# ESMWG/NoahMP

Hardware: AMD Instinct MI355X
Metric: column-steps/sec (higher is better)
Workload: dtype f32

## Files before the change

### __graft_entry__.py

```python
import os
import subprocess
import sys

ROOT = os.path.dirname(os.path.abspath(__file__))
sys.path.insert(0, ROOT)
os.environ.setdefault("GPU_PINNED_MIN_XFER_SIZE", "1048576")


def build():
    from noahmp_amd import build as b
    b.build(verbose=True)
    b.build(extra_flags=["-DNMP_EXACT_LIBM=0"], lib=os.path.join(b.CSRC, "variants", "lib_ocml.so"), jobs=4)
    b.build(extra_flags=["-DNOAHMP_NSOIL=6"], lib=os.path.join(b.CSRC, "variants", "lib_nsoil6.so"), jobs=4)
    subprocess.check_call(["make", "-s", "-C", os.path.join(ROOT, "oracle"), "port"])
    if os.path.isdir("/root/reference"):
        subprocess.check_call(["make", "-s", "-C", os.path.join(ROOT, "oracle"), "ref"])
    sys.path.insert(0, os.path.join(ROOT, "tests"))
    from host_emul import emullib
    emullib.build()
    for ns in (6, 8):
        emullib.build(ns)
    import test_libm
    test_libm.build()
    import test_divrc
    test_divrc.build()
    from fortran import build_shim
    if build_shim.available():
        build_shim.build()
    import noahmp_amd
    from noahmp_amd import abi
    abi.load_library()
    from noahmp_amd import jit_warm
    n, bad = jit_warm.warm()
    if bad:
        raise RuntimeError("jit_warm: %d of %d option sets failed to compile" % (bad, n))
    print("build ok:", b.LIB)


def smoke():
    import torch
    import numpy as np
    from noahmp_amd import synth
    from noahmp_amd.tables import load_tables
    from noahmp_amd.driver import Engine
    from oracle.portlib import PortLib
    from tools.compare import parity_check, exact_check

    T, tb = load_tables("usgs")
    s = synth.mixed_small(tb, ni=64, nj=4)
    synth.first_step_fixups(s)
    synth.diurnal_forcing(s, 12, t_offset=s.t_offset)
    port = PortLib(autobuild=not os.path.exists(os.path.join(ROOT, "oracle", "_build", "libnoahmp_oracle.so")))
    port.set_tables(T)
    eng = Engine(T, device=0)
    so, sd = s.copy(), s.to_device("cuda:0")
    port.noahmplsm(so, 1, 2000, 180.0)
    st = eng.noahmplsm(sd, 1, 2000, 180.0)
    ok, lines = exact_check(so, sd.to_host()) if eng.exact_libm else parity_check(so, sd.to_host(), steps=1)
    print("smoke: land=%d glacier=%d skipped=%d kernel_ms=%.3f" % (st.n_land, st.n_glacier, st.n_skipped, st.kernel_ms))
    if st.code or not ok:
        raise AssertionError("HIP vs oracle mismatch (code %d):\n%s" % (st.code, "\n".join(lines)))
    print("smoke ok")


if __name__ == "__main__":
    build()
    if len(sys.argv) > 1 and sys.argv[1] == "smoke":
        smoke()
```

### include/noahmp_hip.h

```cpp
#ifndef NOAHMP_HIP_H
#define NOAHMP_HIP_H
#ifndef __HIPCC_RTC__
#include <stdint.h>
#include <stddef.h>
#endif
#ifdef __cplusplus
extern "C" {
#endif

#define NOAHMP_HIP_ABI_VERSION 1
#define NOAHMP_NSNOW 3
#ifndef NOAHMP_NSOIL
#define NOAHMP_NSOIL 4
#endif

typedef struct noahmp_step_args {
  int32_t         itimestep;
  int32_t         yr;
  float           julian;
  const float*    coszin;
  const float*    xlatin;
  const float*    dz8w;
  float           dt;
  const float*    dzs;
  int32_t         nsoil;
  float           dx;
  const int32_t*  ivgtyp;
  const int32_t*  isltyp;
  const float*    vegfra;
  const float*    vegmax;
  const float*    tmn;
  const float*    xland;
  const float*    xice;
  float           xice_thres;
  int32_t         isice;
  int32_t         isurban;
  int32_t         idveg;
  int32_t         iopt_crs;
  int32_t         iopt_btr;
  int32_t         iopt_run;
  int32_t         iopt_sfc;
  int32_t         iopt_frz;
  int32_t         iopt_inf;
  int32_t         iopt_rad;
  int32_t         iopt_alb;
  int32_t         iopt_snf;
  int32_t         iopt_tbot;
  int32_t         iopt_stc;
  int32_t         iz0tlnd;
  const float*    t3d;
  const float*    qv3d;
  const float*    u_phy;
  const float*    v_phy;
  const float*    swdown;
  const float*    glw;
  const float*    p8w3d;
  const float*    rainbl;
  float*          tsk;
  float*          hfx;
  float*          qfx;
  float*          lh;
  float*          grdflx;
  float*          smstav;
  float*          smstot;
  float*          sfcrunoff;
  float*          udrunoff;
  float*          albedo;
  float*          snowc;
  float*          smois;
  float*          sh2o;
  float*          tslb;
  float*          snow;
  float*          snowh;
  float*          canwat;
  float*          acsnom;
  float*          acsnow;
  float*          emiss;
  float*          qsfc;
  int32_t*        isnowxy;
  float*          tvxy;
  float*          tgxy;
  float*          canicexy;
  float*          canliqxy;
  float*          eahxy;
  float*          tahxy;
  float*          cmxy;
  float*          chxy;
  float*          fwetxy;
  float*          sneqvoxy;
  float*          alboldxy;
  float*          qsnowxy;
  float*          wslakexy;
  float*          zwtxy;
// ... 373 lines not shown
```

### noahmp_amd/csrc/nmp_dev_common.hpp

```cpp
#pragma once
#ifndef __HIPCC_RTC__
#include <hip/hip_runtime.h>
#include <stdint.h>
#endif
#include "noahmp_hip.h"

namespace nmp {

#define NMP_DEV __host__ __device__ __forceinline__
#define L(i) ((i) + 2)
#if defined(__HIP_DEVICE_COMPILE__)
#define NMP_ASSUME(c) __builtin_assume(c)
#else
#define NMP_ASSUME(c) ((void)0)
#endif
constexpr int NSOIL = NOAHMP_NSOIL;
constexpr int NSNOW = NOAHMP_NSNOW;
constexpr int NL = NSNOW + NSOIL;
static_assert(NSNOW == 3 && NSOIL >= 2 && NSOIL <= 12, "layer slots: three snow layers, 2..12 soil layers");

constexpr float GRAV = 9.80616f, SB = 5.67E-08f, VKC = 0.40f, TFRZ = 273.16f, HSUB = 2.8440E06f,
                HVAP = 2.5104E06f, HFUS = 0.3336E06f, CWAT = 4.188E06f, CICE = 2.094E06f,
                CPAIR = 1004.64f, TKWAT = 0.6f, TKICE = 2.2f, RAIR = 287.04f, RW = 461.269f,
                DENH2O = 1000.f, DENICE = 917.f;
// ... 7 lines not shown
};

NMP_DEV float fmin2(float a, float b) { return (a < b) ? a : b; }
NMP_DEV float fmax2(float a, float b) { return (a > b) ? a : b; }

NMP_DEV float powi2(float a) { return a * a; }
NMP_DEV float powi3(float a) { return a * (a * a); }
NMP_DEV float powi4(float a) { float b = a * a; return b * b; }
NMP_DEV float powi5(float a) { float b = a * a; return a * (b * b); }

#ifndef NMP_EXACT_LIBM
#define NMP_EXACT_LIBM 1
#endif
}
#include "nmp_libm.hpp"
namespace nmp {
#if defined(NMP_LIBM_COUNT) && !defined(__HIP_DEVICE_COMPILE__)
extern "C" long nmp_libm_calls[8];
#define NMP_CNT(i) (nmp_libm_calls[i]++)
#else
#define NMP_CNT(i) ((void)0)
#endif
NMP_DEV float nmp_max(float a, float b) { return a > b ? a : b; }
NMP_DEV float nmp_min(float a, float b) { return a < b ? a : b; }

#if NMP_EXACT_LIBM
NMP_DEV float nmp_expf(float x) { NMP_CNT(0); return libm::expf_(x); }
NMP_DEV float nmp_expf_const(float x) { NMP_CNT(0); return libm::expf_k_(x); }
NMP_DEV float nmp_logf(float x) { NMP_CNT(1); return libm::logf_(x); }
template <int N> NMP_DEV void nmp_logfN(const float* x, float* out) { for (int n = 0; n < N; n++) NMP_CNT(1); libm::logfN_<N>(x, out); }
template <int N> NMP_DEV void nmp_expfN(const float* x, float* out) { for (int n = 0; n < N; n++) NMP_CNT(0); libm::expfN_<N>(x, out); }
template <int N> NMP_DEV void nmp_powfN(const float* x, const float* y, float* out) { for (int n = 0; n < N; n++) NMP_CNT(2); libm::powfN_<N>(x, y, out); }
#define NMP_LOG2K(base) libm::powf_log2_k(libm::asuint(base))
template <int N> NMP_DEV void nmp_powf_constbaseN(const float* base, const double* log2base, const float* y, float* out) {
  for (int n = 0; n < N; n++) NMP_CNT(2);
  libm::powf_constbaseN_<N>(base, log2base, y, out);
}
template <int N> NMP_DEV void nmp_powf_pairN(const float* x, float y1, float y2, float* o1, float* o2) {
  for (int n = 0; n < 2 * N; n++) NMP_CNT(2);
  libm::powf_pairN_<N>(x, y1, y2, o1, o2);
}
NMP_DEV float nmp_powf(float x, float y) { NMP_CNT(2); return libm::powf_(x, y); }
NMP_DEV float nmp_log10f(float x) { NMP_CNT(3); return libm::log10f_(x); }
NMP_DEV float nmp_atanf(float x) { NMP_CNT(4); return libm::atanf_(x); }
NMP_DEV float nmp_atanf_ge1(float x) { NMP_CNT(4); return libm::atanf_ge1_(x); }
NMP_DEV float nmp_tanhf(float x) { NMP_CNT(5); return libm::tanhf_(x); }
NMP_DEV float nmp_tanf(float x) { return libm::tanf_(x); }
NMP_DEV float nmp_acosf(float x) { return libm::acosf_(x); }
NMP_DEV float nmp_cosf(float x) { return libm::cosf_(x); }
NMP_DEV float pow_quarter(float x) { NMP_CNT(6); return libm::powf_(x, 0.25f); }
NMP_DEV void pow_quarter2(float x1, float x2, float& r1, float& r2) {
  NMP_CNT(6); NMP_CNT(6);
  const float x[2] = {x1, x2}, y[2] = {0.25f, 0.25f}; float o[2];
  libm::powfN_<2>(x, y, o);
  r1 = o[0]; r2 = o[1];
}
NMP_DEV float pow_half(float x) { NMP_CNT(6); return libm::powf_(x, 0.5f); }
NMP_DEV float pow_two(float x) { NMP_CNT(6); return libm::powf_(x, 2.0f); }
NMP_DEV float pow_neg_quarter(float x) { NMP_CNT(6); return libm::powf_(x, -0.25f); }
#else
NMP_DEV float nmp_expf(float x) { return expf(x); }
NMP_DEV float nmp_expf_const(float x) { return expf(x); }
NMP_DEV float nmp_logf(float x) { return logf(x); }
template <int N> NMP_DEV void nmp_logfN(const float* x, float* out) { for (int n = 0; n < N; n++) out[n] = logf(x[n]); }
template <int N> NMP_DEV void nmp_expfN(const float* x, float* out) { for (int n = 0; n < N; n++) out[n] = expf(x[n]); }
template <int N> NMP_DEV void nmp_powfN(const float* x, const float* y, float* out) { for (int n = 0; n < N; n++) out[n] = powf(x[n], y[n]); }
#define NMP_LOG2K(base) 0.0
template <int N> NMP_DEV void nmp_powf_constbaseN(const float* base, const double*, const float* y, float* out) { for (int n = 0; n < N; n++) out[n] = powf(base[n], y[n]); }
template <int N> NMP_DEV void nmp_powf_pairN(const float* x, float y1, float y2, float* o1, float* o2) { for (int n = 0; n < N; n++) { o1[n] = powf(x[n], y1); o2[n] = powf(x[n], y2); } }
NMP_DEV float nmp_powf(float x, float y) { return powf(x, y); }
NMP_DEV float nmp_log10f(float x) { return log10f(x); }
NMP_DEV float nmp_atanf(float x) { return atanf(x); }
NMP_DEV float nmp_atanf_ge1(float x) { return atanf(x); }
NMP_DEV float nmp_tanhf(float x) { return tanhf(x); }
NMP_DEV float nmp_tanf(float x) { return tanf(x); }
NMP_DEV float nmp_acosf(float x) { return acosf(x); }
NMP_DEV float nmp_cosf(float x) { return cosf(x); }
NMP_DEV float pow_quarter(float x) { return sqrtf(sqrtf(x)); }
NMP_DEV void pow_quarter2(float x1, float x2, float& r1, float& r2) { r1 = sqrtf(sqrtf(x1)); r2 = sqrtf(sqrtf(x2)); }
NMP_DEV float pow_half(float x) { return sqrtf(x); }
NMP_DEV float pow_two(float x) { return x * x; }
NMP_DEV float pow_neg_quarter(float x) { return 1.0f / sqrtf(sqrtf(x)); }
#endif

#if defined(NMP_PHASE_TIMERS)
constexpr int NMP_NPHASE = 32;
static __device__ unsigned long long g_nmp_prof[NMP_NPHASE * 256];
#endif
#if defined(NMP_PHASE_TIMERS) && defined(__HIP_DEVICE_COMPILE__)
static __shared__ long long s_nmp_last[8];
#define NMP_TIC(ph) do { if ((int)(threadIdx.x & 63) == __ffsll((long long)__ballot(1)) - 1) { const long long now_ = clock64(); \
    const int w_ = threadIdx.x >> 6; \
    atomicAdd(&g_nmp_prof[(ph) * 256 + (blockIdx.x & 255)], (unsigned long long)(now_ - s_nmp_last[w_])); \
    s_nmp_last[w_] = now_; } } while (0)
#define NMP_TIC0() do { if ((threadIdx.x & 63) == 0) s_nmp_last[threadIdx.x >> 6] = clock64(); } while (0)
#else
#define NMP_TIC(ph) ((void)0)
#define NMP_TIC0() ((void)0)
#endif

#ifdef NMP_FIXED_DVEG
#ifndef NMP_FIXED_RUN
#define NMP_FIXED_RUN 1
#endif
#ifndef NMP_FIXED_CRS
#define NMP_FIXED_CRS 1
#define NMP_FIXED_BTR 1
#define NMP_FIXED_SFC 1
#define NMP_FIXED_FRZ 1
#define NMP_FIXED_INF 1
#define NMP_FIXED_RAD 3
#define NMP_FIXED_ALB 2
#define NMP_FIXED_SNF 1
#define NMP_FIXED_TBOT 2
#define NMP_FIXED_STC 1
#endif
struct Opt {
  static constexpr int dveg = NMP_FIXED_DVEG, crs = NMP_FIXED_CRS, btr = NMP_FIXED_BTR, run = NMP_FIXED_RUN, sfc = NMP_FIXED_SFC,
                       frz = NMP_FIXED_FRZ, inf = NMP_FIXED_INF, rad = NMP_FIXED_RAD, alb = NMP_FIXED_ALB, snf = NMP_FIXED_SNF,
                       tbot = NMP_FIXED_TBOT, stc = NMP_FIXED_STC;
};
#else
struct Opt {
  int dveg, crs, btr, run, sfc, frz, inf, rad, alb, snf, tbot, stc;
};
#endif

constexpr int NSLT = 30, NVEGT = 27;
struct Derived {
  float thks_pow[2][NSLT], thkdry[2][NSLT], d_rsurf[2][NSLT], frzx[2][NSLT];
  float kdt[NSLT];
  float chil[NVEGT], phi1[NVEGT], phi2[NVEGT], avmu[NVEGT];
};

struct TablesDev { noahmp_tables t; Derived d; };
NMP_DEV const Derived* derived_of(const noahmp_tables* T) { return &reinterpret_cast<const TablesDev*>(T)->d; }

struct Parm {
  int nroot;
  int st, u;
  float rgl, rsmin, hs, rsmax, topt;
  float bexp, smcmax, smcref, psisat, dksat, dwsat, smcwlt, quartz;
  float slope, csoil, zbot, czil, kdt, frzx;
  float thks_pow, thkdry, d_rsurf, chil, phi1, phi2, avmu;
  float lai1, lai2, sai1, sai2, hvt, hvb, tmin, z0mvt, cwpvt, dleaf;
  float ph_wt1;
  float ch2op;
};

NMP_DEV float div_rc(float x, double r) { return (float)((double)x * r); }
#define NMP_RCC(c) (1.0 / (double)(c))
NMP_DEV double rc64(float y) {
#if defined(__HIP_DEVICE_COMPILE__)
  const double yd = (double)y;
  const double r0 = __builtin_amdgcn_rcp(yd);
  const double e = __builtin_fma(-yd, r0, 1.0);
  const double t = __builtin_fma(e, e, e);
  return __builtin_amdgcn_div_fixup(__builtin_fma(r0, t, r0), yd, 1.0);
#else
  return 1.0 / (double)y;
#endif
}

struct Urc {
  double dt;
  double dt_hfus;
  double dz[NL];
  double dz2[NL];
  double dzmm[NL];
  double zs[NL];
  double one_m_ea4;
};

struct TabScalars {
  int iswater, isbarren, issnow, eblforest, lucats, slcats;
  float csoil, zbot, czil, topt, rsmax, slope0;
  float albsat4[2], albdry4[2], omegas[2], betads, betais, eg1;
};
constexpr int NMP_TS_INTS = 6, NMP_TS_FLOATS = 15;
NMP_DEV TabScalars tab_scalars(const noahmp_tables& t) {
  TabScalars r;
  r.iswater = t.iswater; r.isbarren = t.isbarren; r.issnow = t.issnow; r.eblforest = t.eblforest; r.lucats = t.lucats; r.slcats = t.slcats;
  r.csoil = t.csoil_data; r.zbot = t.zbot_data; r.czil = t.czil_data; r.topt = t.topt_data; r.rsmax = t.rsmax_data; r.slope0 = t.slope_data[0];
  for (int ib = 0; ib < 2; ib++) { r.albsat4[ib] = t.albsat[ib][3]; r.albdry4[ib] = t.albdry[ib][3]; r.omegas[ib] = t.omegas[ib]; }
  r.betads = t.betads; r.betais = t.betais; r.eg1 = t.eg[0];
  return r;
}
NMP_DEV void tab_scalars_pack(const TabScalars& r, int* i, float* f) {
  i[0] = r.iswater; i[1] = r.isbarren; i[2] = r.issnow; i[3] = r.eblforest; i[4] = r.lucats; i[5] = r.slcats;
  f[0] = r.csoil; f[1] = r.zbot; f[2] = r.czil; f[3] = r.topt; f[4] = r.rsmax; f[5] = r.slope0;
  f[6] = r.albsat4[0]; f[7] = r.albsat4[1]; f[8] = r.albdry4[0]; f[9] = r.albdry4[1]; f[10] = r.omegas[0]; f[11] = r.omegas[1];
  f[12] = r.betads; f[13] = r.betais; f[14] = r.eg1;
}
NMP_DEV TabScalars tab_scalars_unpack(const int* i, const float* f) {
  TabScalars r;
  r.iswater = i[0]; r.isbarren = i[1]; r.issnow = i[2]; r.eblforest = i[3]; r.lucats = i[4]; r.slcats = i[5];
  r.csoil = f[0]; r.zbot = f[1]; r.czil = f[2]; r.topt = f[3]; r.rsmax = f[4]; r.slope0 = f[5];
  r.albsat4[0] = f[6]; r.albsat4[1] = f[7]; r.albdry4[0] = f[8]; r.albdry4[1] = f[9]; r.omegas[0] = f[10]; r.omegas[1] = f[11];
  r.betads = f[12]; r.betais = f[13]; r.eg1 = f[14];
  return r;
}

struct Ctx {
  const noahmp_tables* __restrict__ T;
  const Derived* __restrict__ D;
  Opt O;
  float dt;
  float zsoil[NL];
  int isurban;
  TabScalars ts;
  Urc u;
  unsigned char* cost;
};
NMP_DEV void record_cost(const Ctx& c, int which, int n) {
#if defined(__HIP_DEVICE_COMPILE__) && defined(NMP_COST_RECORD)
  if (c.cost) c.cost[2 * (size_t)(blockIdx.x * blockDim.x + threadIdx.x) + which] = (unsigned char)n;
#else
  (void)c; (void)which; (void)n;
#endif
}

#if defined(__HIP_DEVICE_COMPILE__)
NMP_DEV float uniform_value(float x) { int i; memcpy(&i, &x, 4); i = __builtin_amdgcn_readfirstlane(i); memcpy(&x, &i, 4); return x; }
NMP_DEV double uniform_value(double x) {
  int i[2]; memcpy(i, &x, 8);
  i[0] = __builtin_amdgcn_readfirstlane(i[0]); i[1] = __builtin_amdgcn_readfirstlane(i[1]);
  memcpy(&x, i, 8); return x;
}
#else
NMP_DEV float uniform_value(float x) { return x; }
NMP_DEV double uniform_value(double x) { return x; }
#endif
template <class T> NMP_DEV T pick_layer(const T* a, int k) {
  T r = uniform_value(a[L(0)]);
#pragma unroll
  for (int j = 1; j < NSOIL; j++) { const T vj = uniform_value(a[L(j)]); r = (k == j) ? vj : r; }
  const T vn = uniform_value(a[L(NSOIL)]);
  r = (k >= NSOIL) ? vn : r;
  return r;
}

template <int J, class A> NMP_DEV float pick_soil_from(const A& a, int k) {
  if constexpr (J >= NSOIL) return a[L(NSOIL)];
  else return (k == J) ? a[L(J)] : pick_soil_from<J + 1>(a, k);
}
template <class A> NMP_DEV float pick_soil(const A& a, int k) { return pick_soil_from<1>(a, k); }
template <int J, class A> NMP_DEV float pick_soil_below_from(const A& a, int k) {
  if constexpr (J >= NSOIL - 2) return a[L(NSOIL - 1)];
  else return (k == J) ? a[L(J + 1)] : pick_soil_below_from<J + 1>(a, k);
}
template <class A> NMP_DEV float pick_soil_below(const A& a, int k) { return pick_soil_below_from<1>(a, k); }
template <class A, class P> NMP_DEV bool any_of_layers_1_to_4(const A& a, P pred) {
  bool r = false;
#pragma unroll
  for (int j = 1; j <= (NSOIL < 4 ? NSOIL : 4); j++) r = r || pred(a[L(j)]);
  return r;
}

NMP_DEV float dz_soil(const Ctx& c, int k) { return k == 1 ? -c.zsoil[L(1)] : (c.zsoil[L(k - 1)] - c.zsoil[L(k)]); }

NMP_DEV void ctx_fill_uniform(Ctx& c) {
  c.u.dt = 1.0 / (double)c.dt;
  c.u.dt_hfus = 1.0 / (double)(c.dt * HFUS);
  for (int k = 1; k <= NSOIL; k++) {
    const float dz = dz_soil(c, k);
    c.u.dz[L(k)] = 1.0 / (double)dz;
    c.u.dzmm[L(k)] = 1.0 / (double)(dz * 1000.f);
    c.u.zs[L(k)] = 1.0 / (double)(-c.zsoil[L(k)]);
    if (k < NSOIL) c.u.dz2[L(k)] = 1.0 / (double)(k == 1 ? -c.zsoil[L(2)] : (c.zsoil[L(k - 1)] - c.zsoil[L(k + 1)]));
  }
  c.u.one_m_ea4 = 1.0 / (double)(1.0f - nmp_expf(-4.0f));
}

struct Col {
  float lat, julian, cosz, shdfac, shdmax, sfctmp, sfcprs, psfc, uu, vv, q2, soldn, lwdn, prcp,
        tbot, co2air, o2air, foln, zlvl;
  int yearlen, ice, ist, isc, vegtyp;
  float albold, sneqvo, tah, eah, fwet, canliq, canice, tv, tg, qsfc, qsnow;
  int isnow;
  float snowh, sneqv, zwt, wa, wt, wslake, lfmass, rtmass, stmass, wood, stblcp, fastcp, lai, sai,
        cm, ch, tauss, smcwtd, deeprech, rech;
  float acc_sfcrunoff, acc_udrunoff, acc_acsnow, acc_acsnom, acc_rech, acc_deeprech;
  float fsa, fsr, fira, fsh, ssoil, fcev, fgev, fctr, ecan, etran, edir, trad, tgb, tgv, t2mv, t2mb,
        q2v, q2b, runsrf, runsub, apar, psn, sav, sag, fsno, nee, gpp, npp, fveg, albedo, qsnbot,
        ponding, ponding1, ponding2, rssun, rssha, bgap, wgap, chv, chb, emissi, shg, shc, shb, evg,
        evb, ghv, ghb, irg, irc, irb, tr, evc, chleaf, chuc, chv2, chb2, fpice;
  float thair, qair, eair, rhoair, qprecc, qprecl, solad0, solad1, solai0, solai1, swdown;
  float elai, esai, htop, igs, btran, latheav, latheag, qmelt, fsrv, fsrg;
  int frozen_canopy, frozen_ground;
  int err;
};

template <class A>
struct Lay {
  A stc, zsnso, dzsnso;
// ... 9 lines not shown
```

### noahmp_amd/csrc/nmp_dev_energy.hpp

```cpp
#pragma once
#include "nmp_dev_common.hpp"

namespace nmp {

NMP_DEV void esat_sel(float t, float& es, float& des) {
  if (t > 0.f) {
    es = 100.f * (6.107799961f + t * (4.436518521E-01f + t * (1.428945805E-02f + t * (2.650648471E-04f +
         t * (3.031240396E-06f + t * (2.034080948E-08f + t * 6.136820929E-11f))))));
    des = 100.f * (4.438099984E-01f + t * (2.857002636E-02f + t * (7.938054040E-04f + t * (1.215215065E-05f +
          t * (1.036561403E-07f + t * (3.532421810e-10f + t * -7.090244804E-13f))))));
  } else {
    es = 100.f * (6.109177956f + t * (5.034698970E-01f + t * (1.886013408E-02f + t * (4.176223716E-04f +
         t * (5.824720280E-06f + t * (4.838803174E-08f + t * 1.838826904E-10f))))));
    des = 100.f * (5.030305237E-01f + t * (3.773255020E-02f + t * (1.267995369E-03f + t * (2.477563108E-05f +
          t * (3.005693132E-07f + t * (2.158542548E-09f + t * 7.131097725E-12f))))));
  }
}
NMP_DEV float tdc(float t) { return nmp_min(50.f, nmp_max(-50.f, (t - TFRZ))); }

NMP_DEV float tdfcnd_thks_pow(const Parm& P) {
  float thks = nmp_powf(7.7f, P.quartz) * nmp_powf(2.0f, 1.f - P.quartz);
  return nmp_powf(thks, 1.f - P.smcmax);
}
NMP_DEV float tdfcnd_thkdry(const Parm& P) {
// ... 209 lines not shown
    float fage;
    snow_age(c.dt, s.tg, s.sneqvo, s.sneqv, s.tauss, fage);
    if (c.O.alb == 1) {
      float sl = 2.0f, sl1 = 1.f / sl, sl2 = 2.f * sl;
      float cf1 = ((1.f + sl1) / (1.f + sl2 * s.cosz) - sl1);
      float fzen = nmp_max(cf1, 0.f);
      albsni[0] = 0.95f * (1.f - 0.2f * fage);
      albsni[1] = 0.65f * (1.f - 0.5f * fage);
      albsnd[0] = albsni[0] + 0.4f * fzen * (1.f - albsni[0]);
      albsnd[1] = albsni[1] + 0.4f * fzen * (1.f - albsni[1]);
    } else {
      float alb = 0.55f + (s.albold - 0.55f) * nmp_expf(-0.01f * c.dt / 3600.f);
      if (s.qsnow > 0.f) alb = alb + nmp_min(s.qsnow * c.dt, SWEMX) * (0.84f - alb) / (SWEMX);
      albsni[0] = albsni[1] = albsnd[0] = albsnd[1] = alb;
      s.albold = alb;
    }
#pragma unroll
    for (int ib = 0; ib < 2; ib++) {
      float inc = nmp_max(0.11f - 0.40f * smc1, 0.f);
      float albsod = nmp_min(c.ts.albsat4[ib] + inc, c.ts.albdry4[ib]);
      float albsoi = albsod;
      if (s.isc == 9) { albsod += 0.10f; albsoi += 0.10f; }
      albgrd[ib] = albsod * (1.f - s.fsno) + albsnd[ib] * s.fsno;
      albgri[ib] = albsoi * (1.f - s.fsno) + albsni[ib] * s.fsno;
    }
    float gdir = 0.f;
#pragma unroll 1
    for (int ib = 0; ib < 2; ib++) {
#pragma unroll
      for (int ic = 0; ic < 2; ic++) {
        TwoStreamOut o = twostream(c, P, ic, v, s.cosz, vai, s.fwet, s.tv, albgrd[ib], albgri[ib],
                                   rho[ib], tau[ib], c.ts.omegas[ib], s.fveg, gdir, s.bgap, s.wgap);
        if (ic == 0) { fabd[ib] = o.fab; albd[ib] = o.fre; ftdd[ib] = o.ftd; ftid[ib] = o.fti;
                       frevd[ib] = o.frev; fregd[ib] = o.freg; }
        else { fabi[ib] = o.fab; albi[ib] = o.fre; ftii[ib] = o.fti; frevi[ib] = o.frev;
               fregi[ib] = o.freg; }
      }
    }
    float ext = gdir / s.cosz * sqrtf(1.f - rho[0] - tau[0]);
    fsun = (1.f - nmp_expf(-ext * vai)) / nmp_max(ext * vai, MPE);
    if (fsun < 0.01f) fsun = 0.f;
  }
  RadOut r;
  r.fsun = fsun;
  float fsha = 1.f - fsun;
  r.laisun = s.elai * fsun;
  r.laisha = s.elai * fsha;
  const float solad[2] = {s.solad0, s.solad1}, solai[2] = {s.solai0, s.solai1};
  float cad[2], cai[2];
  s.sag = 0.f; s.sav = 0.f; s.fsa = 0.f;
#pragma unroll
  for (int ib = 0; ib < 2; ib++) {
    cad[ib] = solad[ib] * fabd[ib];
    cai[ib] = solai[ib] * fabi[ib];
    s.sav = s.sav + cad[ib] + cai[ib];
    s.fsa = s.fsa + cad[ib] + cai[ib];
    float trd = solad[ib] * ftdd[ib];
    float tri = solad[ib] * ftid[ib] + solai[ib] * ftii[ib];
    float abs_ = trd * (1.f - albgrd[ib]) + tri * (1.f - albgri[ib]);
    s.sag = s.sag + abs_;
    s.fsa = s.fsa + abs_;
  }
  float laifra = s.elai / nmp_max(vai, MPE);
  if (fsun > 0.f) {
    r.parsun = (cad[0] + fsun * cai[0]) * laifra / nmp_max(r.laisun, MPE);
    r.parsha = (fsha * cai[0]) * laifra / nmp_max(r.laisha, MPE);
  } else {
    r.parsun = 0.f;
    r.parsha = (cad[0] + cai[0]) * laifra / nmp_max(r.laisha, MPE);
  }
  float rvis = albd[0] * solad[0] + albi[0] * solai[0];
  float rnir = albd[1] * solad[1] + albi[1] * solai[1];
  s.fsr = rvis + rnir;
  s.fsrv = frevd[0] * solad[0] + frevi[0] * solai[0] + frevd[1] * solad[1] + frevi[1] * solai[1];
  s.fsrg = fregd[0] * solad[0] + fregi[0] * solai[0] + fregd[1] * solad[1] + fregi[1] * solai[1];
  return r;
}

struct MoState {
  float moz, fm, fh, fh2, fv; int mozsgn;
  float tmpcm, tmpcm2;
};

NMP_DEV void sfcdif1(int& err, int iter, float sfctmp, double r_rhocp, float h, float qair, float zlvl,
                     float zpd, float z0m, float ur, float mpe, MoState& m, float& cm,
                     float& ch) {
  const float z0h = z0m;
  float mozold = m.moz;
  float moz2, fmnew, fhnew, fh2new;
  if (zlvl <= zpd) { if (!err) err = NOAHMP_ERR_STABILITY_STOP; }
  if (iter == 1) {
    m.tmpcm = nmp_logf((zlvl - zpd) / z0m);
    m.tmpcm2 = nmp_logf((2.0f + z0m) / z0m);
  }
  const float tmpcm = m.tmpcm, tmpch = m.tmpcm, tmpch2 = m.tmpcm2;
  if (iter == 1) {
    m.fv = 0.0f; m.moz = 0.0f; moz2 = 0.0f;
  } else {
    float tvir = (1.f + 0.61f * qair) * sfctmp;
    float tmp1 = div_rc(VKC * (GRAV / tvir) * h, r_rhocp);
    if (fabsf(tmp1) <= mpe) tmp1 = mpe;
    float mol = -1.f * powi3(m.fv) / tmp1;
    const double r_mol = rc64(mol);
    m.moz = nmp_min(div_rc(zlvl - zpd, r_mol), 1.f);
    moz2 = nmp_min(div_rc(2.0f + z0h, r_mol), 1.f);
  }
  if (mozold * m.moz < 0.f) m.mozsgn = m.mozsgn + 1;
  if (m.mozsgn >= 2) { m.moz = 0.f; m.fm = 0.f; m.fh = 0.f; moz2 = 0.f; m.fh2 = 0.f; }
  if (m.moz < 0.f) {
    float tmp1, tmp12;
    pow_quarter2(1.f - 16.f * m.moz, 1.f - 16.f * moz2, tmp1, tmp12);
    const float la[3] = {(1.f + tmp1 * tmp1) / 2.f, (1.f + tmp1) / 2.f, (1.f + tmp12 * tmp12) / 2.f};
    float lg[3];
    nmp_logfN<3>(la, lg);
    const float tmp2 = lg[0], tmp3 = lg[1];
    fmnew = 2.f * tmp3 + tmp2 - 2.f * nmp_atanf_ge1(tmp1) + 1.5707963f;
    fhnew = 2 * tmp2;
    const float tmp22 = lg[2];
    fh2new = 2 * tmp22;
  } else {
    fmnew = -5.f * m.moz; fhnew = fmnew;
    fh2new = -5.f * moz2;
  }
  if (iter == 1) {
    m.fm = fmnew; m.fh = fhnew; m.fh2 = fh2new;
  } else {
    m.fm = 0.5f * (m.fm + fmnew);
    m.fh = 0.5f * (m.fh + fhnew);
    m.fh2 = 0.5f * (m.fh2 + fh2new);
  }
  m.fh = nmp_min(m.fh, 0.9f * tmpch);
  m.fm = nmp_min(m.fm, 0.9f * tmpcm);
  m.fh2 = nmp_min(m.fh2, 0.9f * tmpch2);
  float cmfm = tmpcm - m.fm, chfh = tmpch - m.fh;
  if (fabsf(cmfm) <= mpe) cmfm = mpe;
  if (fabsf(chfh) <= mpe) chfh = mpe;
  cm = VKC * VKC / (cmfm * cmfm);
  ch = VKC * VKC / (cmfm * chfh);
  m.fv = ur * sqrtf(cm);
}

NMP_DEV float pspmu(float xx) {
  return -2.f * nmp_logf((xx + 1.f) * 0.5f) - nmp_logf((xx * xx + 1.f) * 0.5f) + 2.f * nmp_atanf(xx) -
         (3.14159265f / 2.f);
}
NMP_DEV float psphu(float xx) { return -2.f * nmp_logf((xx * xx + 1.f) * 0.5f); }

NMP_DEV float sfcdif2_rlogu(float z0, float zlm) { return nmp_logf((zlm + z0) / z0); }
NMP_DEV void sfcdif2(int iter, float z0, float thz0, float thlm, float sfcspd, float czil, float zlm,
                     float& akms, float& akhs, float& rlmo, float& wstar2, float& ustar, const float rlogu_in) {
  const float WWST2 = 1.2f * 1.2f, VKRM = 0.40f, EXCM = 0.001f, BTG = (1.0f / 270.0f) * GRAV,
              ELFC = VKRM * BTG, WOLD = 0.15f, WNEW = 1.0f - WOLD, EPSU2 = 1.E-4f, EPSUST = 0.07f,
              ZTMIN = -5.0f, ZTMAX = 1.0f, HPBL = 1000.0f, SQVISC = 258.2f;
  float zilfc = -czil * VKRM * SQVISC;
  float zu = z0;
  float rdz = 1.f / zlm;
  float cxch = EXCM * rdz;
  float dthv = thlm - thz0;
  float du2 = nmp_max(sfcspd * sfcspd, EPSU2);
  float btgh = BTG * HPBL;
  if (iter == 1) {
    if (btgh * akhs * dthv != 0.0f) wstar2 = WWST2 * nmp_powf(fabsf(btgh * akhs * dthv), 2.f / 3.f);
    else wstar2 = 0.0f;
    ustar = nmp_max(sqrtf(akms * sqrtf(du2 + wstar2)), EPSUST);
    rlmo = ELFC * akhs * dthv / powi3(ustar);
  }
  float zt = nmp_max(1.E-6f, nmp_expf(zilfc * sqrtf(ustar * z0)) * z0);
  float zslu = zlm + zu;
  float zslt = zlm + zt;
  const float rlt_arg = zslt / zt;
  const float rlogu = rlogu_in;
  float rlogt;
  float zetalt = nmp_max(zslt * rlmo, ZTMIN);
  rlmo = zetalt / zslt;
  float zetalu = zslu * rlmo;
  float zetau = zu * rlmo;
  float zetat = zt * rlmo;
  float psmz, simm, pshz, simh;
  if (rlmo < 0.f) {
    float xlu = sqrtf(sqrtf(1.f - 16.f * zetalu)), xlt = sqrtf(sqrtf(1.f - 16.f * zetalt)),
          xu = sqrtf(sqrtf(1.f - 16.f * zetau)), xt = sqrtf(sqrtf(1.f - 16.f * zetat));
    const float la[7] = {(xu + 1.f) * 0.5f, (xu * xu + 1.f) * 0.5f, (xlu + 1.f) * 0.5f, (xlu * xlu + 1.f) * 0.5f,
                         (xt * xt + 1.f) * 0.5f, (xlt * xlt + 1.f) * 0.5f, rlt_arg};
    float lg[7];
    nmp_logfN<7>(la, lg);
    rlogt = lg[6];
    psmz = -2.f * lg[0] - lg[1] + 2.f * nmp_atanf(xu) - (3.14159265f / 2.f);
    const float pspmu_xlu = -2.f * lg[2] - lg[3] + 2.f * nmp_atanf(xlu) - (3.14159265f / 2.f);
    simm = pspmu_xlu - psmz + rlogu;
    pshz = -2.f * lg[4];
    simh = -2.f * lg[5] - pshz + rlogt;
  } else {
    rlogt = nmp_logf(rlt_arg);
    zetalu = nmp_min(zetalu, ZTMAX);
    zetalt = nmp_min(zetalt, ZTMAX);
    psmz = 5.f * zetau;
    simm = 5.f * zetalu - psmz + rlogu;
    pshz = 5.f * zetat;
    simh = 5.f * zetalt - pshz + rlogt;
  }
  ustar = nmp_max(sqrtf(akms * sqrtf(du2 + wstar2)), EPSUST);
  float ustark = ustar * VKRM;
  akms = nmp_max(ustark / simm, cxch);
  akhs = nmp_max(ustark / simh, cxch);
  if (btgh * akhs * dthv != 0.0f) wstar2 = WWST2 * nmp_powf(fabsf(btgh * akhs * dthv), 2.f / 3.f);
  else wstar2 = 0.0f;
  float rlmn = ELFC * akhs * dthv / powi3(ustar);
  rlmo = rlmo * WOLD + rlmn * WNEW;
}

struct StomataT { float awc, cp, vcmx_t; };
struct StomataP { float bp, c3psn, mp, folnmx, qe25, vcmx25, kc25, akc, ko25, ako, avcmx; };
NMP_DEV StomataP stomata_rows(const noahmp_tables* T, int v) {
  return StomataP{T->bp[v], T->c3psn[v], T->mp[v], T->folnmx[v], T->qe25[v], T->vcmx25[v], T->kc25[v], T->akc[v], T->ko25[v], T->ako[v], T->avcmx[v]};
}
NMP_DEV StomataT stomata_temperature(const StomataP& T, float tv, float o2) {
  StomataT r;
  float tc = tv - TFRZ;
  const float ex = div_rc(tc - 25.0f, NMP_RCC(10.0f));
  float pk[2];
  { const float pb[2] = {T.akc, T.ako}, py[2] = {ex, ex}; nmp_powfN<2>(pb, py, pk); }
  float kc = T.kc25 * pk[0];
// ... 12 lines not shown
  rs = 1.0f / bpv * cf;
  psn = 0.0f;
  if (apar <= 0.0f) return;
  const float c3 = T.c3psn, mpv = T.mp;
  float fnf = nmp_min(foln / nmp_max(mpe, T.folnmx), 1.0f);
  float ppf = 4.6f * apar;
  float j = ppf * T.qe25;
  const float awc = st.awc, cp = st.cp;
  float vcmx = T.vcmx25 / (1.0f + st.vcmx_t) * fnf * btran * avcmx_pow;
  float rlb = rb / cf;
  float cihi = 1.5f * co2, cilow = 0.0f;
  const double r_sfcprs = rc64(sfcprs);
#pragma unroll 1
  for (int iter = 1; iter <= 20; iter++) {
    float ci = 0.5f * (cihi + cilow);
    float wj = nmp_max(ci - cp, 0.0f) * j / (ci + 2.0f * cp) * c3 + j * (1.f - c3);
    float wc = nmp_max(ci - cp, 0.0f) * vcmx / (ci + awc) * c3 + vcmx * (1.f - c3);
    float we = 0.5f * vcmx * c3 + div_rc(4000.0f * vcmx * ci, r_sfcprs) * (1.f - c3);
    psn = nmp_min(nmp_min(wj, wc), we) * igs;
    float cs = nmp_max(co2 - 1.37f * rlb * sfcprs * psn, mpe);
    float a = mpv * psn * sfcprs * ea / (cs * ei) + bpv;
    float b = (mpv * psn * sfcprs / cs + bpv) * rlb - 1.f;
    float cq = -rlb;
    float q;
    if (b >= 0.0f) q = -0.5f * (b + sqrtf(b * b - 4.0f * a * cq));
    else q = -0.5f * (b - sqrtf(b * b - 4.0f * a * cq));
    float r1 = q / a, r2 = cq / q;
    rs = nmp_max(r1, r2);
    float fci = nmp_max(cs - psn * sfcprs * 1.65f * rs, 0.0f);
    steps++;
    if (((cihi - cilow) <= 5e-2f) || fabsf(fci - ci) <= mpe) break;
    else if (fci > ci) cilow = ci;
    else cihi = ci;
  }
  rs = rs * cf;
}

NMP_DEV void canres(const Parm& P, float par, float sfctmp, float rcsoil, float eah, float sfcprs,
                    float& rc, float& psn) {
  float q2 = 0.622f * eah / (sfcprs - 0.378f * eah);
  q2 = q2 / (1.0f + q2);
  float es = 0.611f * nmp_expf(2.501E6f / 461.0f * (1.f / 273.15f - 1.f / sfctmp));
  float sfcprsx = sfcprs * 1.E-3f;
  float q2sat = 0.622f * es / (sfcprsx - es);
  q2sat = q2sat * 1.E3f;
  q2sat = q2sat / 1.E3f;
  float ff = 2.0f * par / P.rgl;
  float rcs = (ff + P.rsmin / P.rsmax) / (1.0f + ff);
  rcs = nmp_max(rcs, 0.0001f);
  float dt_ = P.topt - sfctmp;
  float rct = 1.0f - 0.0016f * pow_two(dt_);
  rct = nmp_max(rct, 0.0001f);
  float rcq = 1.0f / (1.0f + P.hs * nmp_max(0.f, q2sat - q2));
  rcq = nmp_max(rcq, 0.01f);
  rc = P.rsmin / (rcs * rct * rcq * rcsoil);
  psn = -999.99f;
}

struct VegIn {
  float ur, vai, gammav, gammag, laisun, laisha, cwp, zlvl, zpd, z0m, z0mg, emv, emg, rsurf, rhsur,
        parsun, parsha, df_top, dz_top, stc_top;
  double r_rhocp, r_gammav, r_gammag;
};

struct VegLoop {
  float sfctmp, rhoair, qair, zlvl, zpd, z0m, ur, z0mg, hcan, cwp, vaie, sqrt_dleaf_uc, fveg, tg, laisune,
        laishae, rssun, rssha, rsurf, eair, estg, gammav, air, cir, canliq, canice, latheav, sav, fwet, sfcprs,
        thair, czil, rlogu;
  double r_rhocp, r_hcan, r_gammav;
  double r_ur;
  MoState mo;
  float cm, ch, tv, tah, eah, h, hg, fhg, dtv, rahc, rahg, rb, cah, cvh, estv, destv, irc, shc, evc, tr, wstar,
        tv_in, csh, cev, ctr;
  int liter, err, iter, done;
};
constexpr int VEGLOOP_WORDS = sizeof(VegLoop) / 4;

struct VegFirst {
  const Parm* P; int v; float parsun, parsha, foln, o2air, co2air, igs, btran; float psnsun, psnsha;
  StomataP sp;
  int bisections;
};

template <bool FIRST>
NMP_DEV void vege_iter(const Ctx& c, VegLoop& L, const int iter, VegFirst* f) {
  const float MPE = 1E-6f;
  const float sfctmp = L.sfctmp, rhoair = L.rhoair, ur = L.ur, fveg = L.fveg, tg = L.tg;
  const float z0h = L.z0m, z0hg = L.z0mg, hcan = L.hcan;
  if (c.O.sfc == 1) {
    sfcdif1(L.err, iter, sfctmp, L.r_rhocp, L.h, L.qair, L.zlvl, L.zpd, L.z0m, ur, MPE, L.mo, L.cm, L.ch);
  } else {
    sfcdif2(iter, L.z0m, L.tah, L.thair, ur, L.czil, L.zlvl, L.cm, L.ch, L.mo.moz, L.wstar, L.mo.fv, L.rlogu);
    L.ch = div_rc(L.ch, L.r_ur);
    L.cm = div_rc(L.cm, L.r_ur);
  }
  NMP_TIC(16);
  L.rahc = nmp_max(1.f, 1.f / (L.ch * ur));
  const float rawc = L.rahc;
  {
    float mozg = 0.f, fhgnew;
    if (!FIRST) {
      float tmp1 = div_rc(VKC * (GRAV / L.tah) * L.hg, L.r_rhocp);
      if (fabsf(tmp1) <= MPE) tmp1 = MPE;
      float molg = -1.f * powi3(L.mo.fv) / tmp1;
      mozg = nmp_min((L.zpd - L.z0mg) / molg, 1.f);
    }
    if (mozg < 0.f) fhgnew = pow_neg_quarter(1.f - 15.f * mozg);
    else fhgnew = 1.f + 4.7f * mozg;
    if (FIRST) L.fhg = fhgnew;
    else L.fhg = 0.5f * (L.fhg + fhgnew);
    float cwpc = pow_half(L.cwp * L.vaie * hcan * L.fhg);
    const float ea[4] = {div_rc(-cwpc * z0hg, L.r_hcan), div_rc(-cwpc * (z0h + L.zpd), L.r_hcan), cwpc, -cwpc / 2.f};
    float ex[4];
    nmp_expfN<4>(ea, ex);
    float tmp1 = ex[0];
    float tmp2 = ex[1];
    float tmprah2 = hcan * ex[2] / cwpc * (tmp1 - tmp2);
    float kh = nmp_max(VKC * L.mo.fv * (hcan - L.zpd), MPE);
    L.rahg = tmprah2 / kh;
    float tmprb = cwpc * 50.f / (1.f - ex[3]);
    L.rb = tmprb * L.sqrt_dleaf_uc;
  }
  const float rawg = L.rahg, rb = L.rb;
  NMP_TIC(17);
  float t = tdc(L.tv);
  esat_sel(t, L.estv, L.destv);
  const float estv = L.estv, destv = L.destv;
  NMP_TIC(18);
  if (FIRST) {
    StomataT st = {0.f, 0.f, 0.f};
    float avcmx_pow = 0.f;
    if (c.O.crs == 1 && (!(f->parsun <= 0.0f) || !(f->parsha <= 0.0f))) {
      st = stomata_temperature(f->sp, L.tv, f->o2air);
      avcmx_pow = nmp_powf(f->sp.avcmx, div_rc((L.tv - TFRZ) - 25.0f, NMP_RCC(10.0f)));
    }
#pragma unroll 1
    for (int leaf = 0; leaf < 2; leaf++) {
      float par = leaf ? f->parsha : f->parsun, rs_, psn_;
      if (c.O.crs == 1)
        stomata(f->sp, MPE, par, f->foln, L.tv, estv, L.eah, sfctmp, L.sfcprs, f->o2air, f->co2air, f->igs,
                f->btran, rb, st, avcmx_pow, rs_, psn_, f->bisections);
      else
        canres(*f->P, par, L.tv, f->btran, L.eah, L.sfcprs, rs_, psn_);
      if (leaf) { L.rssha = rs_; f->psnsha = psn_; } else { L.rssun = rs_; f->psnsun = psn_; }
    }
  }
  NMP_TIC(19);
  const double r_rahc = rc64(L.rahc), r_rb = rc64(rb), r_rahg = rc64(L.rahg);
  L.cah = div_rc(1.f, r_rahc);
  L.cvh = div_rc(2.f * L.vaie, r_rb);
  const float cah = L.cah, cvh = L.cvh;
  float cgh = div_rc(1.f, r_rahg);
  float cond = cah + cvh + cgh;
  const double r_cond = rc64(cond);
  float ata = div_rc(sfctmp * cah + tg * cgh, r_cond);
  float bta = div_rc(cvh, r_cond);
  float csh = (1.f - bta) * rhoair * CPAIR * cvh;
  float caw = cah;
  float cew = div_rc(L.fwet * L.vaie, r_rb);
  float ctw = (1.f - L.fwet) * (L.laisune / (rb + L.rssun) + L.laishae / (rb + L.rssha));
  float cgw = 1.f / (rawg + L.rsurf);
  cond = caw + cew + ctw + cgw;
  const double r_cond2 = rc64(cond);
  float aea = div_rc(L.eair * caw + L.estg * cgw, r_cond2);
  float bea = div_rc(cew + ctw, r_cond2);
  float cev = div_rc((1.f - bea) * cew * rhoair * CPAIR, L.r_gammav);
  float ctr = div_rc((1.f - bea) * ctw * rhoair * CPAIR, L.r_gammav);
  L.tah = ata + bta * L.tv;
  L.eah = aea + bea * estv;
  L.irc = fveg * (L.air + L.cir * powi4(L.tv));
  L.shc = fveg * rhoair * CPAIR * cvh * (L.tv - L.tah);
  L.evc = div_rc(fveg * rhoair * CPAIR * cew * (estv - L.eah), L.r_gammav);
  L.tr = div_rc(fveg * rhoair * CPAIR * ctw * (estv - L.eah), L.r_gammav);
  if (L.tv > TFRZ) L.evc = nmp_min(div_rc(L.canliq * L.latheav, c.u.dt), L.evc);
  else L.evc = nmp_min(div_rc(L.canice * L.latheav, c.u.dt), L.evc);
  float b = L.sav - L.irc - L.shc - L.evc - L.tr;
  float a = fveg * (4.f * L.cir * powi3(L.tv) + csh + (cev + ctr) * destv);
  L.dtv = b / a;
  L.tv_in = L.tv; L.csh = csh; L.cev = cev; L.ctr = ctr;
  L.tv = L.tv + L.dtv;
  L.h = div_rc(rhoair * CPAIR * (L.tah - sfctmp), r_rahc);
  L.hg = div_rc(rhoair * CPAIR * (tg - L.tah), r_rahg);
  NMP_TIC(20);
  NMP_CNT(7);
  if (L.liter == 1) L.done = 1;
  else if (iter >= 5 && fabsf(L.dtv) <= 0.01f && L.liter == 0) L.liter = 1;
  L.iter = iter + 1;
  if (L.iter > 20) L.done = 1;
}

NMP_DEV void vege_run_until(const Ctx& c, VegLoop& L, int last) {
#pragma unroll 1
  while (!L.done && L.iter <= last) vege_iter<false>(c, L, L.iter, nullptr);
}

struct SimpleLoop {
  NMP_DEV void run(const Ctx& c, VegLoop& L, bool active) const {
    if (active) vege_run_until(c, L, 20);
  }
};

template <class Runner>
NMP_DEV void vege_flux(const Ctx& c, const Parm& P, Col& s, const VegIn& q, float& cmv, float& psnsun,
                       float& psnsha, const bool canopy, Runner& runner) {
  const noahmp_tables* T = c.T;
  const float MPE = 1E-6f;
  VegLoop L = {};
  L.done = 1;
  if (canopy) {
    const int v = s.vegtyp - 1;
    VegFirst f = {};
    f.P = &P; f.v = v;
    if (c.O.crs == 1) f.sp = stomata_rows(T, v);
    const float fveg = s.fveg, ur = q.ur;
    L.sfctmp = s.sfctmp; L.rhoair = s.rhoair; L.qair = s.qair; L.zlvl = q.zlvl; L.zpd = q.zpd; L.z0m = q.z0m;
    L.ur = ur; L.z0mg = q.z0mg; L.cwp = q.cwp; L.fveg = fveg; L.rsurf = q.rsurf; L.eair = s.eair;
    L.gammav = q.gammav; L.canliq = s.canliq; L.canice = s.canice; L.latheav = s.latheav; L.sav = s.sav;
    L.fwet = s.fwet; L.sfcprs = s.sfcprs; L.thair = s.thair; L.czil = P.czil;
    L.mo = MoState{0.f, 0.f, 0.f, 0.f, 0.1f, 0, 0.f, 0.f};
    L.tv = s.tv; L.tg = s.tgv; L.tah = s.tah; L.eah = s.eah; L.ch = s.chv; L.cm = cmv;
    L.r_rhocp = q.r_rhocp; L.r_gammav = q.r_gammav;
    if (c.O.sfc != 1) { L.r_ur = rc64(ur); L.rlogu = sfcdif2_rlogu(L.z0m, L.zlvl); }
    const double r_fveg = rc64(fveg);
    L.vaie = nmp_min(6.f, div_rc(q.vai, r_fveg));
    L.laisune = nmp_min(6.f, div_rc(q.laisun, r_fveg));
    L.laishae = nmp_min(6.f, div_rc(q.laisha, r_fveg));
    float t = tdc(L.tg), destg_unused;
    esat_sel(t, L.estg, destg_unused);
    L.hcan = s.htop;
    L.r_hcan = rc64(L.hcan);
    float uc = ur * nmp_logf(L.hcan / q.z0m) / nmp_logf(q.zlvl / q.z0m);
    if ((L.hcan - q.zpd) <= 0.f) raise(s, NOAHMP_ERR_HCAN_LE_ZPD);
    L.air = -q.emv * (1.f + (1.f - q.emv) * (1.f - q.emg)) * s.lwdn - q.emv * q.emg * SB * powi4(L.tg);
    L.cir = (2.f - q.emv * (1.f - q.emg)) * q.emv * SB;
    L.sqrt_dleaf_uc = sqrtf(P.dleaf / uc);
    L.irc = s.irc; L.shc = s.shc; L.evc = s.evc; L.tr = s.tr;
    L.done = 0; L.iter = 1;
    f.parsun = q.parsun; f.parsha = q.parsha; f.foln = s.foln; f.o2air = s.o2air; f.co2air = s.co2air; f.igs = s.igs; f.btran = s.btran;
    vege_iter<true>(c, L, 1, &f);
    psnsun = f.psnsun; psnsha = f.psnsha;
    record_cost(c, 1, f.bisections);
  } else {
    record_cost(c, 1, 0);
  }
  runner.run(c, L, canopy);
  record_cost(c, 0, canopy ? L.iter - 1 : 0);
  NMP_TIC(21);
  if (!canopy) return;
  if (L.err) raise(s, L.err);
  {
    const float fveg = L.fveg, destv = L.destv;
    L.irc = L.irc + fveg * 4.f * L.cir * powi3(L.tv_in) * L.dtv;
    L.shc = L.shc + fveg * L.csh * L.dtv;
    L.evc = L.evc + fveg * L.cev * destv * L.dtv;
    L.tr = L.tr + fveg * L.ctr * destv * L.dtv;
  }
  float& tv = s.tv; float& tg = s.tgv; float& tah = s.tah; float& eah = s.eah;
  const float rhoair = s.rhoair;
  tv = L.tv; tah = L.tah; eah = L.eah; cmv = L.cm;
  s.rssun = L.rssun; s.rssha = L.rssha;
  s.irc = L.irc; s.shc = L.shc; s.evc = L.evc; s.tr = L.tr;
  s.qsfc = (0.622f * L.eah) / (L.sfcprs - 0.378f * L.eah);
  const float rahg = L.rahg, rawg = L.rahg, cah = L.cah, cvh = L.cvh, z0h = q.z0m, fveg = s.fveg;
  float t, estg = L.estg, destg = 0.f;
  float air = -q.emg * (1.f - q.emv) * s.lwdn - q.emg * q.emv * SB * powi4(tv);
  float cir = q.emg * SB;
  float csh = rhoair * CPAIR / rahg;
  float cev = rhoair * CPAIR / (q.gammag * (rawg + q.rsurf));
  float cgh = 2.f * q.df_top / q.dz_top;
#pragma unroll 1
  for (int iter = 1; iter <= 5; iter++) {
    t = tdc(tg);
    esat_sel(t, estg, destg);
    s.irg = cir * powi4(tg) + air;
    s.shg = csh * (tg - tah);
    s.evg = cev * (estg * q.rhsur - eah);
    s.ghv = cgh * (tg - q.stc_top);
    float b = s.sag - s.irg - s.shg - s.evg - s.ghv;
    float a = 4.f * cir * powi3(tg) + csh + cev * destg + cgh;
    float dtg = b / a;
    s.irg = s.irg + 4.f * cir * powi3(tg) * dtg;
    s.shg = s.shg + csh * dtg;
    s.evg = s.evg + cev * destg * dtg;
    s.ghv = s.ghv + cgh * dtg;
    tg = tg + dtg;
  }
  if (c.O.stc == 1) {
    if (s.snowh > 0.05f && tg > TFRZ) {
      tg = TFRZ;
      s.irg = cir * powi4(tg) - q.emg * (1.f - q.emv) * s.lwdn - q.emg * q.emv * SB * powi4(tv);
      s.shg = csh * (tg - tah);
      s.evg = cev * (estg * q.rhsur - eah);
      s.ghv = s.sag - (s.irg + s.shg + s.evg);
    }
  }
  float cah2 = L.mo.fv * VKC / ((c.O.sfc == 1 ? L.mo.tmpcm2 : nmp_logf((2.f + z0h) / z0h)) - L.mo.fh2);
  s.chv2 = cah2;
  if (cah2 < 1.E-5f) {
    s.t2mv = tah;
    s.q2v = s.qsfc;
  } else {
    const double r_fveg = rc64(fveg), r_cah2 = rc64(cah2);
    s.t2mv = tah - div_rc(div_rc(s.shg + div_rc(s.shc, r_fveg), q.r_rhocp) * 1.f, r_cah2);
    s.q2v = s.qsfc - div_rc(((div_rc(s.evc + s.tr, r_fveg) + s.evg) / (s.latheav * rhoair)) * 1.f, r_cah2);
  }
  s.chv = cah;
  s.chleaf = cvh;
  s.chuc = 1.f / rahg;
}

NMP_DEV void bare_flux(const Ctx& c, const Parm& P, Col& s, const VegIn& q, float zpdg, float& cmb) {
  const float MPE = 1E-6f;
  const float rhoair = s.rhoair, sfctmp = s.sfctmp, ur = q.ur, z0m = q.z0mg;
  MoState mo = {0.f, 0.f, 0.f, 0.f, 0.1f, 0, 0.f, 0.f};
  float h = 0.f, wstar = 0.f;
  float t, estg = 0.f, destg, csh = 0.f, cev = 0.f, ehb = 0.f;
  float& tgb = s.tgb; float& ch = s.chb; float& cm = cmb;
  const float z0h = z0m;
  const float cir = q.emg * SB;
  const float cgh = 2.f * q.df_top / q.dz_top;
  const float gamma = q.gammag, lathea = s.latheag;
  t = tdc(tgb);
  esat_sel(t, estg, destg);
  const double r_ur = (c.O.sfc != 1) ? rc64(ur) : 0.0;
  const float rlogu2 = (c.O.sfc != 1) ? sfcdif2_rlogu(z0m, q.zlvl) : 0.f;
#pragma unroll 1
  for (int iter = 1; iter <= 5; iter++) {
    if (c.O.sfc == 1) {
      sfcdif1(s.err, iter, sfctmp, q.r_rhocp, h, s.qair, q.zlvl, zpdg, z0m, ur, MPE, mo, cm, ch);
    } else {
      sfcdif2(iter, z0m, tgb, s.thair, ur, P.czil, q.zlvl, cm, ch, mo.moz, wstar, mo.fv, rlogu2);
      ch = div_rc(ch, r_ur);
      cm = div_rc(cm, r_ur);
      if (s.snowh > 0.f) { cm = nmp_min(0.01f, cm); ch = nmp_min(0.01f, ch); }
    }
    float rahb = nmp_max(1.f, 1.f / (ch * ur));
    float rawb = rahb;
    const double r_rahb = rc64(rahb);
    ehb = div_rc(1.f, r_rahb);
    csh = div_rc(rhoair * CPAIR, r_rahb);
    cev = div_rc(rhoair * CPAIR, q.r_gammag) / (q.rsurf + rawb);
    s.irb = cir * powi4(tgb) - q.emg * s.lwdn;
    s.shb = csh * (tgb - sfctmp);
    s.evb = cev * (estg * q.rhsur - s.eair);
    s.ghb = cgh * (tgb - q.stc_top);
    float b = s.sag - s.irb - s.shb - s.evb - s.ghb;
    float a = 4.f * cir * powi3(tgb) + csh + cev * destg + cgh;
    float dtg = b / a;
    if (iter == 5) {
      s.irb = s.irb + 4.f * cir * powi3(tgb) * dtg;
      s.shb = s.shb + csh * dtg;
      s.evb = s.evb + cev * destg * dtg;
      s.ghb = s.ghb + cgh * dtg;
    }
    tgb = tgb + dtg;
    h = csh * (tgb - sfctmp);
    t = tdc(tgb);
    esat_sel(t, estg, destg);
    if (iter == 5) s.qsfc = 0.622f * (estg * q.rhsur) / (s.psfc - 0.378f * (estg * q.rhsur));
  }
  if (c.O.stc == 1) {
    if (s.snowh > 0.05f && tgb > TFRZ) {
      tgb = TFRZ;
      s.irb = cir * powi4(tgb) - q.emg * s.lwdn;
      s.shb = csh * (tgb - sfctmp);
      s.evb = cev * (estg * q.rhsur - s.eair);
      s.ghb = s.sag - (s.irb + s.shb + s.evb);
    }
  }
  float ehb2 = mo.fv * VKC / ((c.O.sfc == 1 ? mo.tmpcm2 : nmp_logf((2.f + z0h) / z0h)) - mo.fh2);
  s.chb2 = ehb2;
  if (ehb2 < 1.E-5f) {
    s.t2mb = tgb;
    s.q2b = s.qsfc;
  } else {
    s.t2mb = tgb - div_rc(s.shb, q.r_rhocp) * 1.f / ehb2;
    s.q2b = s.qsfc - s.evb / (lathea * rhoair) * (1.f / ehb2 + q.rsurf);
  }
  if (s.vegtyp == c.isurban) s.q2b = s.qsfc;
  ch = ehb;
}

template <class A>
NMP_DEV void tsnosoi(const Ctx& c, const Parm& P, const Col& s, const Lay<A>& y, const float* df,
                     const float* hcpct) {
  const int isnow = s.isnow, ntop = isnow + 1;
  const float dt = c.dt;
  const float zbotsno = P.zbot - s.snowh;
  float ai[NL], bi[NL], ci[NL], rhsts[NL], ddz[NL], dtsdz[NL], zs[NL], tt[NL];
#pragma unroll
  for (int k = -2; k <= NSOIL; k++) { zs[L(k)] = y.zsnso[L(k)]; tt[L(k)] = y.stc[L(k)]; }
#pragma unroll
  for (int k = -2; k <= NSOIL; k++) {
    const int km = (k > -2) ? k - 1 : -2;
    const int kp = (k < NSOIL) ? k + 1 : NSOIL;
    ai[L(k)] = 0.f; bi[L(k)] = 1.f; ci[L(k)] = 0.f; rhsts[L(k)] = 0.f; ddz[L(k)] = 0.f; dtsdz[L(k)] = 0.f;
    if (k >= ntop) {
      float denom, eflux;
      if (k == ntop) {
        denom = -zs[L(k)] * hcpct[L(k)];
        float temp1 = -zs[L(kp)];
        const double r_temp1 = rc64(temp1);
        ddz[L(k)] = div_rc(2.0f, r_temp1);
        dtsdz[L(k)] = div_rc(2.0f * (tt[L(k)] - tt[L(kp)]), r_temp1);
        eflux = df[L(k)] * dtsdz[L(k)] - s.ssoil - 0.f;
      } else if (k < NSOIL) {
        denom = (zs[L(km)] - zs[L(k)]) * hcpct[L(k)];
        float temp1 = zs[L(km)] - zs[L(kp)];
        const double r_temp1 = rc64(temp1);
        ddz[L(k)] = div_rc(2.0f, r_temp1);
        dtsdz[L(k)] = div_rc(2.0f * (tt[L(k)] - tt[L(kp)]), r_temp1);
        eflux = (df[L(k)] * dtsdz[L(k)] - df[L(km)] * dtsdz[L(km)]) - 0.f;
      } else {
        denom = (zs[L(km)] - zs[L(k)]) * hcpct[L(k)];
        float botflx = 0.f;
        if (c.O.tbot == 2) {
          dtsdz[L(k)] = (tt[L(k)] - s.tbot) / (0.5f * (zs[L(km)] + zs[L(k)]) - zbotsno);
          botflx = -df[L(k)] * dtsdz[L(k)];
        }
        eflux = (-botflx - df[L(km)] * dtsdz[L(km)]) - 0.f;
      }
      const double r_denom = rc64(denom);
      if (k == ntop) {
        ai[L(k)] = 0.0f;
        ci[L(k)] = div_rc(-df[L(k)] * ddz[L(k)], r_denom);
        if (c.O.stc == 1) bi[L(k)] = -ci[L(k)];
        else bi[L(k)] = -ci[L(k)] + df[L(k)] / (0.5f * zs[L(k)] * zs[L(k)] * hcpct[L(k)]);
      } else if (k < NSOIL) {
        ai[L(k)] = div_rc(-df[L(km)] * ddz[L(km)], r_denom);
        ci[L(k)] = div_rc(-df[L(k)] * ddz[L(k)], r_denom);
        bi[L(k)] = -(ai[L(k)] + ci[L(k)]);
      } else {
        ai[L(k)] = div_rc(-df[L(km)] * ddz[L(km)], r_denom);
        ci[L(k)] = 0.0f;
        bi[L(k)] = -(ai[L(k)] + ci[L(k)]);
      }
      rhsts[L(k)] = div_rc(eflux, -r_denom);
      rhsts[L(k)] = rhsts[L(k)] * dt;
      ai[L(k)] = ai[L(k)] * dt;
      bi[L(k)] = 1.f + bi[L(k)] * dt;
      ci[L(k)] = ci[L(k)] * dt;
    }
  }
// ... 351 lines not shown
```

### noahmp_amd/csrc/nmp_dev_water.hpp

```cpp
#pragma once
#include "nmp_dev_common.hpp"

namespace nmp {

NMP_DEV void canwater(const Ctx& c, const Parm& P, Col& s, float& qrain, float& snowhin) {
  const float dt = c.dt, sfctmp = s.sfctmp, fveg = s.fveg;
  const double rdt = c.u.dt;
  float fp = 0.0f, qintr, qdripr, qthror, qints, qdrips, qthros, qevac, qdewc, qsubc, qfroc;
  float fpice = 0.f;
  if (c.O.snf == 1) {
    if (sfctmp > TFRZ + 2.5f) fpice = 0.f;
    else if (sfctmp <= TFRZ + 0.5f) fpice = 1.0f;
    else if (sfctmp <= TFRZ + 2.f) fpice = 1.f - (-54.632f + 0.2f * sfctmp);
    else fpice = 0.6f;
  } else if (c.O.snf == 2) {
    fpice = (sfctmp >= TFRZ + 2.2f) ? 0.f : 1.0f;
  } else {
    fpice = (sfctmp >= TFRZ) ? 0.f : 1.0f;
  }
  s.fpice = fpice;
  float bdfall = nmp_min(120.f, 67.92f + 51.25f * nmp_expf(div_rc(sfctmp - TFRZ, NMP_RCC(2.59f))));
  float rain = (s.qprecc + s.qprecl) * (1.f - fpice);
  float snow = (s.qprecc + s.qprecl) * fpice;
  if (s.qprecc + s.qprecl > 0.f) fp = (s.qprecc + s.qprecl) / (10.f * s.qprecc + s.qprecl);
  const float vai = s.elai + s.esai;
  float maxliq = P.ch2op * vai;
  if (vai > 0.f) {
    qintr = fveg * rain * fp;
    qintr = nmp_min(qintr, div_rc(maxliq - s.canliq, rdt) * (1.f - nmp_expf(-rain * dt / maxliq)));
    qintr = nmp_max(qintr, 0.f);
    qdripr = fveg * rain - qintr;
    qthror = (1.f - fveg) * rain;
  } else {
    qintr = 0.f; qdripr = 0.f; qthror = rain;
  }
  if (!s.frozen_canopy) {
    const float fcev_hvap = div_rc(s.fcev, NMP_RCC(HVAP));
    s.etran = nmp_max(div_rc(s.fctr, NMP_RCC(HVAP)), 0.f);
    qevac = nmp_max(fcev_hvap, 0.f);
    qdewc = fabsf(nmp_min(fcev_hvap, 0.f));
    qsubc = 0.f; qfroc = 0.f;
  } else {
    const float fcev_hsub = div_rc(s.fcev, NMP_RCC(HSUB));
    s.etran = nmp_max(div_rc(s.fctr, NMP_RCC(HSUB)), 0.f);
    qevac = 0.f; qdewc = 0.f;
    qsubc = nmp_max(fcev_hsub, 0.f);
    qfroc = fabsf(nmp_min(fcev_hsub, 0.f));
  }
  qevac = nmp_min(div_rc(s.canliq, rdt), qevac);
  s.canliq = nmp_max(0.f, s.canliq + (qintr + qdewc - qevac) * dt);
  if (s.canliq <= 1.E-06f) s.canliq = 0.0f;
  float maxsno = 6.6f * (0.27f + 46.f / bdfall) * vai;
  if (vai > 0.f) {
    qints = fveg * snow * fp;
    qints = nmp_min(qints, div_rc(maxsno - s.canice, rdt) * (1.f - nmp_expf(-snow * dt / maxsno)));
    qints = nmp_max(qints, 0.f);
    float ft = nmp_max(0.0f, div_rc(s.tv - 270.15f, NMP_RCC(1.87E5f)));
    float fv = div_rc(sqrtf(s.uu * s.uu + s.vv * s.vv), NMP_RCC(1.56E5f));
    qdrips = nmp_max(0.f, s.canice) * (fv + ft);
    qthros = (1.0f - fveg) * snow + (fveg * snow - qints);
  } else {
    qints = 0.f; qdrips = 0.f; qthros = snow;
  }
  qsubc = nmp_min(div_rc(s.canice, rdt), qsubc);
  s.canice = nmp_max(0.f, s.canice + (qints - qdrips) * dt + (qfroc - qsubc) * dt);
  if (s.canice <= 1.E-6f) s.canice = 0.f;
  if (s.canice > 0.f) s.fwet = nmp_max(0.f, s.canice) / nmp_max(maxsno, 1.E-06f);
  else s.fwet = nmp_max(0.f, s.canliq) / nmp_max(maxliq, 1.E-06f);
  s.fwet = nmp_powf(nmp_min(s.fwet, 1.f), 0.667f);
  if (s.canice > 1.E-6f && s.tv > TFRZ) {
    float qmeltc = nmp_min(div_rc(s.canice, rdt), div_rc(div_rc((s.tv - TFRZ) * CICE * s.canice, NMP_RCC(DENICE)), c.u.dt_hfus));
    s.canice = nmp_max(0.f, s.canice - qmeltc * dt);
    s.canliq = nmp_max(0.f, s.canliq + qmeltc * dt);
    s.tv = s.fwet * TFRZ + (1.f - s.fwet) * s.tv;
  }
  if (s.canliq > 1.E-6f && s.tv < TFRZ) {
    float qfrzc = nmp_min(div_rc(s.canliq, rdt), div_rc(div_rc((TFRZ - s.tv) * CWAT * s.canliq, NMP_RCC(DENH2O)), c.u.dt_hfus));
    s.canliq = nmp_max(0.f, s.canliq - qfrzc * dt);
    s.canice = nmp_max(0.f, s.canice + qfrzc * dt);
    s.tv = s.fwet * TFRZ + (1.f - s.fwet) * s.tv;
  }
  s.ecan = qevac + qsubc - qdewc - qfroc;
  qrain = qdripr + qthror;
  s.qsnow = qdrips + qthros;
  snowhin = s.qsnow / bdfall;
}

NMP_DEV void combo(float& dz, float& wliq, float& wice, float& t, float dz2, float wliq2, float wice2,
                   float t2) {
  float dzc = dz + dz2;
  float wicec = (wice + wice2);
  float wliqc = (wliq + wliq2);
  float h = (CICE * wice + CWAT * wliq) * (t - TFRZ) + HFUS * wliq;
  float h2 = (CICE * wice2 + CWAT * wliq2) * (t2 - TFRZ) + HFUS * wliq2;
  float hc = h + h2, tc;
  if (hc < 0.f) tc = TFRZ + hc / (CICE * wicec + CWAT * wliqc);
  else if (hc <= HFUS * wliqc) tc = TFRZ;
  else tc = TFRZ + (hc - HFUS * wliqc) / (CICE * wicec + CWAT * wliqc);
  dz = dzc; wice = wicec; wliq = wliqc; t = tc;
}

template <bool GLAC, class A>
NMP_DEV void combine(Col& s, const Lay<A>& y) {
  int& isnow = s.isnow;
  int isnow_old = isnow;
#pragma unroll 1
  for (int j = isnow_old + 1; j <= 0; j++) {
    if (y.snice[L(j)] <= .1f) {
      if (j != 0) {
        y.snliq[L(j + 1)] = y.snliq[L(j + 1)] + y.snliq[L(j)];
        y.snice[L(j + 1)] = y.snice[L(j + 1)] + y.snice[L(j)];
      } else {
        if (isnow_old < -1) {
          y.snliq[L(j - 1)] = y.snliq[L(j - 1)] + y.snliq[L(j)];
          y.snice[L(j - 1)] = y.snice[L(j - 1)] + y.snice[L(j)];
        } else {
          if (GLAC) {
            s.ponding1 = s.ponding1 + y.snliq[L(j)];
            s.sneqv = y.snice[L(j)];
            s.snowh = y.dzsnso[L(j)];
          } else if (y.snice[L(j)] >= 0.f) {
            s.ponding1 = y.snliq[L(j)];
            s.sneqv = y.snice[L(j)];
            s.snowh = y.dzsnso[L(j)];
          } else {
            s.ponding1 = y.snliq[L(j)] + y.snice[L(j)];
            if (s.ponding1 < 0.f) {
              y.sice[L(1)] = nmp_max(0.0f, y.sice[L(1)] + s.ponding1 / (y.dzsnso[L(1)] * 1000.f));
              s.ponding1 = 0.0f;
            }
            s.sneqv = 0.0f;
            s.snowh = 0.0f;
          }
          y.snliq[L(j)] = 0.0f; y.snice[L(j)] = 0.0f; y.dzsnso[L(j)] = 0.0f;
        }
      }
      if (j > isnow + 1 && isnow < -1) {
#pragma unroll 1
        for (int i = j; i >= isnow + 2; i--) {
          y.stc[L(i)] = y.stc[L(i - 1)];
          y.snliq[L(i)] = y.snliq[L(i - 1)];
          y.snice[L(i)] = y.snice[L(i - 1)];
          y.dzsnso[L(i)] = y.dzsnso[L(i - 1)];
        }
      }
      isnow = isnow + 1;
    }
  }
  if (y.sice[L(1)] < 0.f) { y.sh2o[L(1)] = y.sh2o[L(1)] + y.sice[L(1)]; y.sice[L(1)] = 0.f; }
  if (isnow == 0) return;
  s.sneqv = 0.f; s.snowh = 0.f;
  float zwice = 0.f, zwliq = 0.f;
// ... 206 lines not shown
    }
  }
  s.qsnbot = div_rc(qout, c.u.dt);
}

template <class A>
NMP_DEV void rebuild_layers(const Ctx& c, const Col& s, const Lay<A>& y) {
  float run = 0.f;
#pragma unroll
  for (int iz = -2; iz <= NSOIL; iz++) {
    if (iz > s.isnow) {
      float d;
      if (iz <= 0) d = -y.dzsnso[L(iz)];
      else if (iz == 1) d = c.zsoil[L(1)];
      else d = (c.zsoil[L(iz)] - c.zsoil[L(iz > 1 ? iz - 1 : 1)]);
      run = (iz == s.isnow + 1) ? d : (run + d);
      y.zsnso[L(iz)] = run;
      y.dzsnso[L(iz)] = -d;
    }
  }
}

template <class A>
NMP_DEV void snowwater(const Ctx& c, Col& s, const Lay<A>& y, float snowhin, float qsnfro,
                       float qsnsub, float qrain, float& snoflow) {
  const float dt = c.dt;
  snoflow = 0.0f; s.ponding1 = 0.0f; s.ponding2 = 0.0f;
  {
    int newnode = 0;
    if (s.isnow == 0 && s.qsnow > 0.f) {
      s.snowh = s.snowh + snowhin * dt;
      s.sneqv = s.sneqv + s.qsnow * dt;
    }
    if (s.isnow == 0 && s.qsnow > 0.f && s.snowh >= 0.025f) {
      s.isnow = -1;
      newnode = 1;
      y.dzsnso[L(0)] = s.snowh;
      s.snowh = 0.f;
      y.stc[L(0)] = nmp_min(273.16f, s.sfctmp);
      y.snice[L(0)] = s.sneqv;
      y.snliq[L(0)] = 0.f;
    }
    if (s.isnow < 0 && newnode == 0 && s.qsnow > 0.f) {
      y.snice[L(s.isnow + 1)] = y.snice[L(s.isnow + 1)] + s.qsnow * dt;
      y.dzsnso[L(s.isnow + 1)] = y.dzsnso[L(s.isnow + 1)] + snowhin * dt;
    }
  }
  if (s.isnow < 0) compact(c, s, y);
  if (s.isnow < 0) combine<false>(s, y);
  if (s.isnow < 0) divide<false>(s, y);
  snowh2o<false>(c, s, y, qsnfro, qsnsub, qrain);
  NMP_ASSUME(s.isnow >= -NSNOW && s.isnow <= 0);
#pragma unroll
  for (int iz = -2; iz <= 0; iz++) {
    if (iz <= s.isnow) {
      y.snice[L(iz)] = 0.f; y.snliq[L(iz)] = 0.f; y.stc[L(iz)] = 0.f; y.dzsnso[L(iz)] = 0.f;
      y.zsnso[L(iz)] = 0.f;
    }
  }
  if (s.sneqv > 2000.f) {
    float bdsnow = y.snice[L(0)] / y.dzsnso[L(0)];
    snoflow = (s.sneqv - 2000.f);
    y.snice[L(0)] = y.snice[L(0)] - snoflow;
    y.dzsnso[L(0)] = y.dzsnso[L(0)] - snoflow / bdsnow;
    snoflow = div_rc(snoflow, c.u.dt);
  }
  if (s.isnow < 0) {
    float sw = 0.f;
#pragma unroll
    for (int iz = -2; iz <= 0; iz++)
      if (iz > s.isnow) sw = sw + y.snice[L(iz)] + y.snliq[L(iz)];
    s.sneqv = sw;
  }
  rebuild_layers(c, s, y);
}

NMP_DEV void wdfcnd1(const Parm& P, double r_smcmax, float& wdf, float& wcnd, float smc, float fcr) {
  float factr = nmp_max(0.01f, div_rc(smc, r_smcmax));
  wdf = P.dwsat * nmp_powf(factr, P.bexp + 2.0f);
  wdf = wdf * (1.0f - fcr);
  wcnd = P.dksat * nmp_powf(factr, 2.0f * P.bexp + 3.0f);
  wcnd = wcnd * (1.0f - fcr);
}
NMP_DEV void wdfcnd2(const Parm& P, double r_smcmax, float& wdf, float& wcnd, float smc, float sice) {
  float factr = nmp_max(0.01f, div_rc(smc, r_smcmax));
  float expon = P.bexp + 2.0f;
  wdf = P.dwsat * nmp_powf(factr, expon);
  if (sice > 0.0f) {
    float x = 500.f * sice;
    float vkwgt = 1.f / (1.f + nmp_powf(x, 3.f));
    wdf = vkwgt * wdf + (1.f - vkwgt) * P.dwsat * nmp_powf(div_rc(0.2f, r_smcmax), expon);
  }
  wcnd = P.dksat * nmp_powf(factr, 2.0f * P.bexp + 3.0f);
}

template <class A>
NMP_DEV void soilwater(const Ctx& c, const Parm& P, Col& s, const Lay<A>& y, float qinsur, float qseva,
                       const float* etrani, float& qdrain, float* wcnd, float& fcrmax) {
  const float dt = c.dt;
  const double r_smcmax = rc64(P.smcmax);
  float sh2o[NL], smc[NL], sice[NL], dz[NL], fcr[NL];
  float pddum = 0.0f, rsat = 0.0f, sicemax = 0.0f;
  s.runsrf = 0.0f;
  fcrmax = 0.0f;
#pragma unroll
  for (int k = 1; k <= NSOIL; k++) {
    sh2o[L(k)] = y.sh2o[L(k)]; smc[L(k)] = y.smc[L(k)]; sice[L(k)] = y.sice[L(k)];
    dz[L(k)] = dz_soil(c, k);
  }
#pragma unroll
  for (int k = 1; k <= NSOIL; k++) {
    float epore = nmp_max(1.E-4f, (P.smcmax - sice[L(k)]));
    rsat = rsat + nmp_max(0.f, sh2o[L(k)] - epore) * dz[L(k)];
    sh2o[L(k)] = nmp_min(epore, sh2o[L(k)]);
  }
  const float ea4 = nmp_expf_const(-4.0f);
  float fcr_arg[NSOIL], fcr_exp[NSOIL];
#pragma unroll
  for (int k = 1; k <= NSOIL; k++) fcr_arg[k - 1] = -4.0f * (1.f - nmp_min(1.0f, div_rc(sice[L(k)], r_smcmax)));
  nmp_expfN<NSOIL>(fcr_arg, fcr_exp);
#pragma unroll
  for (int k = 1; k <= NSOIL; k++) {
    fcr[L(k)] = div_rc(nmp_max(0.0f, fcr_exp[k - 1] - ea4), c.u.one_m_ea4);
    if (sice[L(k)] > sicemax) sicemax = sice[L(k)];
    if (fcr[L(k)] > fcrmax) fcrmax = fcr[L(k)];
  }
  if (c.O.run == 2) {
    float wd1 = 0.f, wd2 = 0.f;
#pragma unroll
    for (int k = 1; k <= NSOIL; k++) wd1 = wd1 + (P.smcmax - sh2o[L(k)]) * dz[L(k)];
    float dzfine = 3.0f * (-c.zsoil[L(NSOIL)]) / 100;
    s.zwt = -3.f * c.zsoil[L(NSOIL)] - 0.001f;
    const float zwt0 = s.zwt;
#pragma unroll 1
    for (int k = 1; k <= 100; k++) {
      float zfine = (float)k * dzfine;
      float temp = 1.f + (zwt0 - zfine) / P.psisat;
      wd2 = wd2 + P.smcmax * (1.f - nmp_powf(temp, -1.f / P.bexp)) * dzfine;
      if (fabsf(wd2 - wd1) <= 0.01f) { s.zwt = zfine; break; }
    }
    s.runsub = (1.0f - fcrmax) * 4.0f * nmp_expf_const(-TIMEAN) * nmp_expf(-2.0f * s.zwt);
  }
  if (s.vegtyp == c.isurban) fcr[L(1)] = 0.95f;
  if (c.O.run == 1 || c.O.run == 2 || c.O.run == 4 || c.O.run == 5) {
    float fsat;
    if (c.O.run == 1) fsat = FSATMX * nmp_expf(-0.5f * 6.0f * (s.zwt - 2.0f));
    else if (c.O.run == 5) fsat = FSATMX * nmp_expf(-0.5f * 6.0f * nmp_max(-2.0f - s.zwt, 0.f));
    else if (c.O.run == 2) fsat = FSATMX * nmp_expf(-0.5f * 2.0f * s.zwt);
    else {
      float smctot = 0.f, dztot = 0.f;
      bool done = false;
#pragma unroll
      for (int k = 1; k <= NSOIL; k++) {
        if (!done) {
          dztot = dztot + dz[L(k)];
          smctot = smctot + smc[L(k)] * dz[L(k)];
          if (dztot >= 2.0f) done = true;
        }
      }
      smctot = smctot / dztot;
      fsat = nmp_powf(nmp_max(0.01f, smctot / P.smcmax), 4.f);
    }
    if (qinsur > 0.f) {
      s.runsrf = qinsur * ((1.0f - fcr[L(1)]) * fsat + fcr[L(1)]);
      pddum = qinsur - s.runsrf;
    }
  }
  if (c.O.run == 3) {
    if (qinsur > 0.0f) {
      float dt1 = dt / 86400.f;
      float smcav = P.smcmax - P.smcwlt;
      float dmax = -c.zsoil[L(1)] * smcav;
      float dice = -c.zsoil[L(1)] * sice[L(1)];
      dmax = dmax * (1.0f - (sh2o[L(1)] + sice[L(1)] - P.smcwlt) / smcav);
      float dd = dmax;
#pragma unroll
      for (int k = 2; k <= NSOIL; k++) {
        float th = (c.zsoil[L(k - 1)] - c.zsoil[L(k)]);
        dice = dice + th * sice[L(k)];
        dmax = th * smcav;
        dmax = dmax * (1.0f - (sh2o[L(k)] + sice[L(k)] - P.smcwlt) / smcav);
        dd = dd + dmax;
      }
      float val = (1.f - nmp_expf(-P.kdt * dt1));
      float ddt = dd * val;
      float px = nmp_max(0.f, qinsur * dt);
      float infmax = (px * (ddt / (px + ddt))) / dt;
      float fcr_ = 1.f;
      if (dice > 1.E-2f) {
        float acrt = 3 * P.frzx / dice;
        float sum = 1.f;
        sum = sum + (acrt * acrt) / 2.f;
        sum = sum + acrt / 1.f;
        fcr_ = 1.f - nmp_expf(-acrt) * sum;
      }
      infmax = infmax * fcr_;
      float wdf_, wcnd_;
      wdfcnd2(P, r_smcmax, wdf_, wcnd_, sh2o[L(1)], sicemax);
      infmax = nmp_max(infmax, wcnd_);
      infmax = nmp_min(infmax, px);
      s.runsrf = nmp_max(0.f, qinsur - infmax);
      pddum = qinsur - s.runsrf;
    }
  }
  int niter = 1;
  if (c.O.inf == 1) {
    niter = 3;
    if (pddum * dt > dz[L(1)] * P.smcmax) niter = niter * 2;
  }
  const float dtf = dt / niter;
  float qdrain_save = 0.0f;
  qdrain = 0.f;
#pragma unroll 1
  for (int iter = 1; iter <= niter; iter++) {
    float wdf[NL], smx[NL], ddz[NL], dsmdz[NL], ai[NL], bi[NL], ci[NL], rhstt[NL];
    float smxwtd = 0.f;
    if (c.O.inf == 1) {
      float factr[NSOIL], pw1[NSOIL], pw2[NSOIL];
#pragma unroll
      for (int k = 1; k <= NSOIL; k++) factr[k - 1] = nmp_max(0.01f, div_rc(smc[L(k)], r_smcmax));
      nmp_powf_pairN<NSOIL>(factr, P.bexp + 2.0f, 2.0f * P.bexp + 3.0f, pw1, pw2);
#pragma unroll
      for (int k = 1; k <= NSOIL; k++) {
        wdf[L(k)] = P.dwsat * pw1[k - 1];
        wdf[L(k)] = wdf[L(k)] * (1.0f - fcr[L(k)]);
        wcnd[L(k)] = P.dksat * pw2[k - 1];
        wcnd[L(k)] = wcnd[L(k)] * (1.0f - fcr[L(k)]);
        smx[L(k)] = smc[L(k)];
      }
    } else {
#pragma unroll
      for (int k = 1; k <= NSOIL; k++) { wdfcnd2(P, r_smcmax, wdf[L(k)], wcnd[L(k)], sh2o[L(k)], sicemax); smx[L(k)] = sh2o[L(k)]; }
    }
    if (c.O.run == 5) smxwtd = (c.O.inf == 1) ? s.smcwtd : s.smcwtd * sh2o[L(NSOIL)] / smc[L(NSOIL)];
#pragma unroll
    for (int k = 1; k <= NSOIL; k++) {
      float denom, wflux;
      if (k == 1) {
        denom = -c.zsoil[L(k)];
        ddz[L(k)] = div_rc(2.0f, c.u.dz2[L(k)]);
        dsmdz[L(k)] = div_rc(2.0f * (smx[L(k)] - smx[L(k + 1)]), c.u.dz2[L(k)]);
        wflux = wdf[L(k)] * dsmdz[L(k)] + wcnd[L(k)] - pddum + etrani[L(k)] + qseva;
      } else if (k < NSOIL) {
        denom = (c.zsoil[L(k - 1)] - c.zsoil[L(k)]);
        ddz[L(k)] = div_rc(2.0f, c.u.dz2[L(k)]);
        dsmdz[L(k)] = div_rc(2.0f * (smx[L(k)] - smx[L(k + 1)]), c.u.dz2[L(k)]);
        wflux = wdf[L(k)] * dsmdz[L(k)] + wcnd[L(k)] - wdf[L(k - 1)] * dsmdz[L(k - 1)] - wcnd[L(k - 1)] +
                etrani[L(k)];
      } else {
        denom = (c.zsoil[L(k - 1)] - c.zsoil[L(k)]);
        if (c.O.run == 1 || c.O.run == 2) qdrain = 0.f;
        if (c.O.run == 3) qdrain = P.slope * wcnd[L(k)];
        if (c.O.run == 4) qdrain = (1.0f - fcrmax) * wcnd[L(k)];
        if (c.O.run == 5) {
          float smxbot;
          if (s.zwt < c.zsoil[L(NSOIL)] - denom)
            smxbot = smx[L(k)] - (smx[L(k)] - smxwtd) * denom * 2.f / (denom + c.zsoil[L(k)] - s.zwt);
          else
            smxbot = smxwtd;
          dsmdz[L(k)] = div_rc(2.0f * (smx[L(k)] - smxbot), 0.5 * c.u.dz[L(k)]);
          qdrain = wdf[L(k)] * dsmdz[L(k)] + wcnd[L(k)];
        }
        wflux = -(wdf[L(k - 1)] * dsmdz[L(k - 1)]) - wcnd[L(k - 1)] + etrani[L(k)] + qdrain;
      }
      if (k == 1) {
        ai[L(k)] = 0.0f;
        bi[L(k)] = div_rc(wdf[L(k)] * ddz[L(k)], c.u.dz[L(k)]);
        ci[L(k)] = -bi[L(k)];
      } else if (k < NSOIL) {
        ai[L(k)] = div_rc(-wdf[L(k - 1)] * ddz[L(k - 1)], c.u.dz[L(k)]);
        ci[L(k)] = div_rc(-wdf[L(k)] * ddz[L(k)], c.u.dz[L(k)]);
        bi[L(k)] = -(ai[L(k)] + ci[L(k)]);
      } else {
        ai[L(k)] = div_rc(-wdf[L(k - 1)] * ddz[L(k - 1)], c.u.dz[L(k)]);
        ci[L(k)] = 0.0f;
        bi[L(k)] = -(ai[L(k)] + ci[L(k)]);
      }
      rhstt[L(k)] = div_rc(wflux, -c.u.dz[L(k)]);
    }
    float wplus = 0.0f;
#pragma unroll
    for (int k = 1; k <= NSOIL; k++) {
      rhstt[L(k)] = rhstt[L(k)] * dtf;
      ai[L(k)] = ai[L(k)] * dtf;
      bi[L(k)] = 1.f + bi[L(k)] * dtf;
      ci[L(k)] = ci[L(k)] * dtf;
    }
    {
      float p[NL], dl[NL];
      ci[L(NSOIL)] = 0.0f;
      p[L(1)] = -ci[L(1)] / bi[L(1)];
      dl[L(1)] = rhstt[L(1)] / bi[L(1)];
#pragma unroll
      for (int k = 2; k <= NSOIL; k++) {
        float inv = 1.0f / (bi[L(k)] + ai[L(k)] * p[L(k - 1)]);
        p[L(k)] = -ci[L(k)] * inv;
        dl[L(k)] = (rhstt[L(k)] - ai[L(k)] * dl[L(k - 1)]) * inv;
      }
      p[L(NSOIL)] = dl[L(NSOIL)];
#pragma unroll
      for (int kk = NSOIL - 1; kk >= 1; kk--) p[L(kk)] = p[L(kk)] * p[L(kk + 1)] + dl[L(kk)];
#pragma unroll
      for (int k = 1; k <= NSOIL; k++) sh2o[L(k)] = sh2o[L(k)] + p[L(k)];
    }
    if (c.O.run == 5) {
      if (s.zwt < c.zsoil[L(NSOIL)] - dz[L(NSOIL)]) {
        s.deeprech = s.deeprech + dtf * qdrain;
      } else {
        s.smcwtd = s.smcwtd + div_rc(dtf * qdrain, c.u.dz[L(NSOIL)]);
        wplus = nmp_max((s.smcwtd - P.smcmax), 0.0f) * dz[L(NSOIL)];
        float wminus = nmp_max((1.E-4f - s.smcwtd), 0.0f) * dz[L(NSOIL)];
        s.smcwtd = nmp_max(nmp_min(s.smcwtd, P.smcmax), 1.E-4f);
        sh2o[L(NSOIL)] = sh2o[L(NSOIL)] + div_rc(wplus, c.u.dz[L(NSOIL)]);
        qdrain = qdrain - wplus / dtf;
        s.deeprech = s.deeprech - wminus;
      }
    }
#pragma unroll
    for (int k = NSOIL; k >= 2; k--) {
      float epore = nmp_max(1.E-4f, (P.smcmax - sice[L(k)]));
      wplus = nmp_max((sh2o[L(k)] - epore), 0.0f) * dz[L(k)];
      sh2o[L(k)] = nmp_min(epore, sh2o[L(k)]);
      sh2o[L(k - 1)] = sh2o[L(k - 1)] + div_rc(wplus, c.u.dz[L(k - 1)]);
    }
    {
      float epore = nmp_max(1.E-4f, (P.smcmax - sice[L(1)]));
      wplus = nmp_max((sh2o[L(1)] - epore), 0.0f) * dz[L(1)];
      sh2o[L(1)] = nmp_min(epore, sh2o[L(1)]);
    }
#pragma unroll
    for (int k = 1; k <= NSOIL; k++) smc[L(k)] = sh2o[L(k)] + sice[L(k)];
    rsat = rsat + wplus;
    qdrain_save = qdrain_save + qdrain;
  }
  qdrain = (niter == 3) ? div_rc(qdrain_save, NMP_RCC(3.f)) : (niter == 6) ? div_rc(qdrain_save, NMP_RCC(6.f)) : qdrain_save;
  s.runsrf = s.runsrf * 1000.f + div_rc(rsat * 1000.f, c.u.dt);
  qdrain = qdrain * 1000.f;
  if (c.O.run == 2) {
    float wtsub = 0.f;
#pragma unroll
    for (int k = 1; k <= NSOIL; k++) wtsub = wtsub + wcnd[L(k)] * dz[L(k)];
#pragma unroll
    for (int k = 1; k <= NSOIL; k++) {
      float mh2o = s.runsub * dt * (wcnd[L(k)] * dz[L(k)]) / wtsub;
      sh2o[L(k)] = sh2o[L(k)] - div_rc(mh2o, c.u.dzmm[L(k)]);
    }
  }
  if (c.O.run != 1) {
    float mliq[NL], xs;
    const float watmin = 0.01f;
#pragma unroll
    for (int iz = 1; iz <= NSOIL; iz++) mliq[L(iz)] = sh2o[L(iz)] * dz[L(iz)] * 1000.f;
#pragma unroll
    for (int iz = 1; iz <= NSOIL - 1; iz++) {
      xs = (mliq[L(iz)] < 0.f) ? (watmin - mliq[L(iz)]) : 0.f;
      mliq[L(iz)] = mliq[L(iz)] + xs;
      mliq[L(iz + 1)] = mliq[L(iz + 1)] - xs;
    }
    xs = (mliq[L(NSOIL)] < watmin) ? (watmin - mliq[L(NSOIL)]) : 0.f;
    mliq[L(NSOIL)] = mliq[L(NSOIL)] + xs;
    s.runsub = s.runsub - div_rc(xs, c.u.dt);
    if (c.O.run == 5) s.deeprech = s.deeprech - xs * 1.E-3f;
#pragma unroll
    for (int iz = 1; iz <= NSOIL; iz++) sh2o[L(iz)] = div_rc(mliq[L(iz)], c.u.dzmm[L(iz)]);
  }
#pragma unroll
  for (int k = 1; k <= NSOIL; k++) { y.sh2o[L(k)] = sh2o[L(k)]; y.smc[L(k)] = smc[L(k)]; }
}

template <class A>
NMP_DEV void groundwater(const Ctx& c, const Parm& P, Col& s, const Lay<A>& y, const float* wcnd,
                         float fcrmax, float& qdis) {
  const float ROUS = 0.2f, CMIC = 0.20f, dt = c.dt;
  float dzmm[NL], znode[NL], mliq[NL], epore[NL], hk[NL], smc[NL];
  dzmm[L(1)] = -c.zsoil[L(1)] * 1.E3f;
  znode[L(1)] = -c.zsoil[L(1)] / 2.f;
#pragma unroll
  for (int iz = 2; iz <= NSOIL; iz++) {
    dzmm[L(iz)] = 1.E3f * (c.zsoil[L(iz - 1)] - c.zsoil[L(iz)]);
    znode[L(iz)] = -c.zsoil[L(iz - 1)] + 0.5f * (c.zsoil[L(iz - 1)] - c.zsoil[L(iz)]);
  }
#pragma unroll
  for (int iz = 1; iz <= NSOIL; iz++) {
    float sh = y.sh2o[L(iz)], si = y.sice[L(iz)];
    smc[L(iz)] = sh + si;
    mliq[L(iz)] = sh * dzmm[L(iz)];
    epore[L(iz)] = nmp_max(0.01f, P.smcmax - si);
    hk[L(iz)] = 1.E3f * wcnd[L(iz)];
  }
  int iwt = NSOIL;
  {
    bool found = false;
#pragma unroll
    for (int iz = 2; iz <= NSOIL; iz++)
      if (!found && s.zwt <= -c.zsoil[L(iz)]) { iwt = iz - 1; found = true; }
  }
  qdis = (1.0f - fcrmax) * 5.0f * nmp_expf_const(-TIMEAN) * nmp_expf(-6.0f * (s.zwt - 2.0f));
  float smc_iwt = pick_soil(smc, iwt), hk_iwt = pick_soil(hk, iwt), zn_iwt = pick_soil(znode, iwt);
  double s_node = nmp_min(1.0f, smc_iwt / P.smcmax);
  s_node = (s_node > (double)0.01f) ? s_node : (double)0.01f;
  float smpfz = (float)(-((double)(P.psisat * 1000.f) * pow(s_node, (double)(-P.bexp))));
  smpfz = nmp_max(-120000.0f, CMIC * smpfz);
  float wh_zwt = -s.zwt * 1.E3f;
  float wh = smpfz - zn_iwt * 1.E3f;
  float qin = -hk_iwt * (wh_zwt - wh) / ((s.zwt - zn_iwt) * 1.E3f);
  qin = nmp_max(div_rc(-10.0f, c.u.dt), nmp_min(div_rc(10.f, c.u.dt), qin));
  s.wt = s.wt + (qin - qdis) * dt;
  if (iwt == NSOIL) {
    s.wa = s.wa + (qin - qdis) * dt;
    s.wt = s.wa;
    s.zwt = (-c.zsoil[L(NSOIL)] + 25.f) - div_rc(div_rc(s.wa, NMP_RCC(1000.f)), NMP_RCC(ROUS));
    mliq[L(NSOIL)] = mliq[L(NSOIL)] - qin * dt;
    mliq[L(NSOIL)] = mliq[L(NSOIL)] + nmp_max(0.f, (s.wa - 5000.f));
    s.wa = nmp_min(s.wa, 5000.f);
  } else {
    if (iwt == NSOIL - 1) {
      s.zwt = -c.zsoil[L(NSOIL)] - div_rc((s.wt - ROUS * 1000 * 25.f) / (epore[L(NSOIL)]), NMP_RCC(1000.f));
    } else {
      float ws = 0.f;
#pragma unroll
      for (int iz = 3; iz <= NSOIL; iz++)
        if (iz >= iwt + 2) ws = ws + epore[L(iz)] * dzmm[L(iz)];
      const float ep = pick_soil_below(epore, iwt), zs = pick_soil_below(c.zsoil, iwt);
      s.zwt = -zs - div_rc((s.wt - ROUS * 1000.f * 25.f - ws) / (ep), NMP_RCC(1000.f));
    }
    float wtsub = 0.f;
#pragma unroll
    for (int iz = 1; iz <= NSOIL; iz++) wtsub = wtsub + hk[L(iz)] * dzmm[L(iz)];
    const double r_wtsub = rc64(wtsub);
#pragma unroll
    for (int iz = 1; iz <= NSOIL; iz++) mliq[L(iz)] = mliq[L(iz)] - div_rc(qdis * dt * hk[L(iz)] * dzmm[L(iz)], r_wtsub);
  }
  s.zwt = nmp_max(1.5f, s.zwt);
  float xs;
  const float watmin = 0.01f;
#pragma unroll
  for (int iz = 1; iz <= NSOIL - 1; iz++) {
    xs = (mliq[L(iz)] < 0.f) ? (watmin - mliq[L(iz)]) : 0.f;
    mliq[L(iz)] = mliq[L(iz)] + xs;
    mliq[L(iz + 1)] = mliq[L(iz + 1)] - xs;
  }
  xs = (mliq[L(NSOIL)] < watmin) ? (watmin - mliq[L(NSOIL)]) : 0.f;
  mliq[L(NSOIL)] = mliq[L(NSOIL)] + xs;
  s.wa = s.wa - xs;
  s.wt = s.wt - xs;
#pragma unroll
  for (int iz = 1; iz <= NSOIL; iz++) y.sh2o[L(iz)] = div_rc(mliq[L(iz)], c.u.dzmm[L(iz)]);
}
// ... 132 lines not shown
```

### noahmp_amd/csrc/nmp_engine_fixed.inc

```
#define NMP_CAT2(a, b) a##b
#define NMP_CAT(a, b) NMP_CAT2(a, b)
#define NMP_FIXED_TAG NMP_CAT(NMP_CAT(d, NMP_FIXED_DVEG), NMP_CAT(_r, NMP_FIXED_RUN))
#define nmp NMP_CAT(nmp_fixed_, NMP_FIXED_TAG)
#include "nmp_kernel.hpp"

namespace nmp_host {

static void NMP_CAT(fill_fixed_, NMP_FIXED_TAG)(KArgs& k, const LaunchDesc& d) {
  memset(&k, 0, sizeof(k));
  k.a = d.a;
  k.c.T = d.tables; k.c.D = derived_of(d.tables); k.c.dt = d.dt; k.c.isurban = d.isurban;
  k.c.ts = tab_scalars_unpack(d.ts_i, d.ts_f);
  for (int l = 0; l < NL; l++) k.c.zsoil[l] = d.zsoil[l];
  ctx_fill_uniform(k.c);
  k.ni = d.ni; k.nka = d.nka; k.nti = d.nti; k.ntj = d.ntj; k.k1 = d.k1; k.kp_lo = d.kp_lo; k.kp_hi = d.kp_hi; k.yearlen = d.yearlen;
  k.c.cost = d.cost;
  k.r_land = d.r_land; k.r_ice = d.r_ice; k.r_skip = d.r_skip;
  k.err = d.err; k.counts = d.counts; k.err_base = d.err_base; k.t_offset = d.t_offset; k.t_first = d.t_first; k.t_count = d.t_count;
}

#ifdef NMP_FIXED_EXPORT_PACK
size_t pack_fixed_kargs(const LaunchDesc& d, void* buf, size_t cap) {
  if (cap < sizeof(KArgs)) return 0;
  NMP_CAT(fill_fixed_, NMP_FIXED_TAG)(*reinterpret_cast<KArgs*>(buf), d);
  return sizeof(KArgs);
}
#endif

void NMP_CAT(launch_fixed_, NMP_FIXED_TAG)(const LaunchDesc& d, int mode, hipStream_t s, hipEvent_t ev0, hipEvent_t ev1) {
  KArgs k;
  NMP_CAT(fill_fixed_, NMP_FIXED_TAG)(k, d);
#ifndef NMP_FIXED_USE_LDS
#define NMP_FIXED_USE_LDS true
#endif
  constexpr long B = NMP_FIXED_BLOCK;
  if (mode == 4) {
    const long nb = (k.r_ice + B - 1) / B + (k.r_land + B - 1) / B + (k.r_skip + B - 1) / B;
    if (nb <= 0) return;
    hipExtLaunchKernelGGL((noahmp_ranges_kernel<NMP_FIXED_BLOCK>), dim3((unsigned)nb), dim3(NMP_FIXED_BLOCK), 0, s, ev0, ev1, 0, k);
    return;
  }
  const long n = (long)k.nti * k.ntj;
  if (n <= 0) return;
  hipExtLaunchKernelGGL((noahmp_column_kernel<NMP_FIXED_BLOCK, NMP_FIXED_USE_LDS, 0>), dim3((unsigned)((n + B - 1) / B)), dim3(NMP_FIXED_BLOCK), 0, s, ev0, ev1, 0, k);
}

#ifdef NMP_PHASE_TIMERS
void NMP_CAT(prof_fixed_, NMP_FIXED_TAG)(unsigned long long* acc, int n) {
  std::vector<unsigned long long> h(nmp::NMP_NPHASE * 256);
  if (hipMemcpyFromSymbol(h.data(), HIP_SYMBOL(nmp::g_nmp_prof), h.size() * 8) != hipSuccess) return;
  for (int p = 0; p < n && p < nmp::NMP_NPHASE; p++)
    for (int s2 = 0; s2 < 256; s2++) acc[p] += h[p * 256 + s2];
  std::fill(h.begin(), h.end(), 0ull);
  (void)hipMemcpyToSymbol(HIP_SYMBOL(nmp::g_nmp_prof), h.data(), h.size() * 8);
}
#endif

}
```

### noahmp_amd/csrc/nmp_engine_host.hpp

```cpp
#pragma once
#include <hip/hip_runtime.h>
#include <hip/hip_ext.h>
#include <stdio.h>
#include <string>
#include <unordered_map>
#include <vector>
#include "noahmp_hip.h"

#ifndef NMP_FIXED_BLOCK
#define NMP_FIXED_BLOCK 64
#endif

namespace nmp_host {

constexpr int kCountSlots = 256;
constexpr int kCountStride = 16;

struct Engine {
  int device = -1;
  bool have_tables = false;
  noahmp_tables* d_tables = nullptr;
  int ts_i[6] = {0, 0, 0, 0, 0, 0}; float ts_f[15] = {};
  unsigned long long* d_err = nullptr;
  int* d_counts = nullptr;
  int* d_gw_counts = nullptr;
  unsigned long long* h_err = nullptr;
  int* h_counts = nullptr;
  hipEvent_t ev0 = nullptr, ev1 = nullptr;
  bool ev_timed = false;
  hipStream_t own_stream = nullptr;
  std::vector<void*> mirror;
  std::vector<size_t> mirror_bytes;
  std::vector<void*> gw_mirror;
  std::vector<size_t> gw_mirror_bytes;
  std::vector<void*> init_mirror;
  std::vector<size_t> init_mirror_bytes;
  float* gw_kcell = nullptr;
  float* gw_head = nullptr;
  size_t gw_plane_bytes = 0;
  int async_pending = 0;
  hipStream_t async_stream = nullptr;
  std::vector<hipStream_t> async_streams;
  std::vector<hipEvent_t> async_events;
  int async_nti = 1, async_its = 1, async_jts = 1;
  float sync_class_ms[3] = {0.f, 0.f, 0.f};
  int sync_steps = 0;
  std::vector<float> sync_step_ms;
  std::vector<signed char> async_kind;
  int last_launch_kind = 0;
  unsigned char* d_cost = nullptr; size_t d_cost_bytes = 0; long cost_cols = 0; int record_cost = 0;
  bool cost_fresh = false;
  long long last_counts[3] = {0, 0, 0};
  int deferred_code = 0;
  hipStream_t s_up = nullptr, s_dn = nullptr;
  std::vector<hipEvent_t> pipe_events;
  struct HostReg { size_t bytes; int seen; int state; };
  std::unordered_map<const void*, HostReg> host_regs;
  int host_chunks = 3;
  bool host_chunks_auto = true;
  int pin_host_arrays = 0;
  int trust_out_mirror = 0;
  bool out_mirror_valid = false;
  std::vector<const void*> pipe_host;
  int pipe_extents[9] = {0, 0, 0, 0, 0, 0, 0, 0, 0};
  int resident_state = 0, lazy_download = 0;
  int static_inputs = 0;
  int deferred_status = 0;
  bool deferred_pending = false;
  unsigned resident_calls = 0;
  std::vector<void*> mirror_b;
  std::vector<size_t> mirror_b_bytes;
  int resident_sorted = 0;
  std::vector<void*> smirror; std::vector<size_t> smirror_bytes;
  int* s_perm = nullptr; unsigned* s_keys = nullptr; unsigned short* s_order = nullptr; int* s_dpos = nullptr; size_t s_cols = 0;
  long s_land = -1, s_glacier = -1;
  bool sorted_ok = false;
  bool sorted_newer = false;
  bool last_step_sorted = false;
  unsigned calls_since_sort = 0;
  hipEvent_t ev_up = nullptr, ev_kdone = nullptr;
  bool resident_valid = false, resident_dirty = false;
  std::vector<const void*> mirror_host;
  noahmp_step_args resident_args;
  int jit_kernels = 1;
  int jit_compile_only = 0;
  int fixed_kernels = 1;
  long sorted_land = -1, sorted_glacier = -1;
  int block = 256;
  int use_lds = 1;
  std::string last_error;
};
extern Engine g;

struct LaunchDesc {
  noahmp_step_args a;
  const noahmp_tables* tables;
  int ts_i[6]; float ts_f[15];
  float dt, zsoil[NOAHMP_NSNOW + NOAHMP_NSOIL + 1];
  int isurban, ni, nka, nti, ntj, k1, kp_lo, kp_hi, yearlen;
  unsigned long long* err;
  int* counts;
  unsigned long long err_base;
  long t_offset, t_first, t_count;
  unsigned char* cost;
  long r_land, r_ice, r_skip;
};
void launch_fixed_d1_r1(const LaunchDesc& d, int mode, hipStream_t s, hipEvent_t ev0, hipEvent_t ev1);
#ifdef NMP_PHASE_TIMERS
void prof_fixed_d1_r1(unsigned long long*, int); void prof_fixed_d3_r1(unsigned long long*, int); void prof_fixed_d3_r5(unsigned long long*, int);
void prof_fixed_d4_r1(unsigned long long*, int); void prof_fixed_d4_r3(unsigned long long*, int);
#endif
void launch_fixed_d3_r1(const LaunchDesc& d, int mode, hipStream_t s, hipEvent_t ev0, hipEvent_t ev1);
void launch_fixed_d3_r5(const LaunchDesc& d, int mode, hipStream_t s, hipEvent_t ev0, hipEvent_t ev1);
void launch_fixed_d4_r1(const LaunchDesc& d, int mode, hipStream_t s, hipEvent_t ev0, hipEvent_t ev1);
void launch_fixed_d4_r3(const LaunchDesc& d, int mode, hipStream_t s, hipEvent_t ev0, hipEvent_t ev1);
bool launch_jit(const int* o, const LaunchDesc& d, int mode, hipStream_t s, hipEvent_t ev0, hipEvent_t ev1);
void jit_finalize();
void jit_stats(int* out);
std::string cache_dir_public();
unsigned long long source_hash_public();
void sort_finalize();

#define HIPCHK(x) do { hipError_t e_ = (x); if (e_ != hipSuccess) { \
  char b_[256]; snprintf(b_, sizeof b_, "%s failed: %s (%s:%d)", #x, hipGetErrorString(e_), __FILE__, __LINE__); \
  nmp_host::g.last_error = b_; return -100; } } while (0)

int ensure_init();
void sum_counts(long long* out);
void status_counts(noahmp_status* st);
int ensure_bytes(void** p, size_t* have, size_t need);

}
```

### noahmp_amd/csrc/nmp_libm.hpp

```cpp
#pragma once
#ifndef __HIPCC_RTC__
#include <hip/hip_runtime.h>
#include <stdint.h>
#include <string.h>
#endif

namespace nmp {
namespace libm {

#ifndef NMP_LIBM_DEV
#define NMP_LIBM_DEV __host__ __device__ __forceinline__
#endif
#ifndef NMP_LIBM_FN
#define NMP_LIBM_FN NMP_LIBM_DEV
#endif
#ifndef NMP_LIBM_FN_POW
#define NMP_LIBM_FN_POW NMP_LIBM_FN
#endif

#if defined(__HIP_DEVICE_COMPILE__)
#define NMP_LIBM_TABLE static __device__ const
#else
#define NMP_LIBM_TABLE static const
#endif
#include "nmp_libm_tables.inc"
#ifndef NMP_LIBM_LDS
#define NMP_LIBM_LDS 1
#endif
#if defined(__HIP_DEVICE_COMPILE__) && NMP_LIBM_LDS
static __shared__ uint64_t sExp2fTab[32];
static __shared__ double sLogfTab[32];
static __shared__ double sPowfLog2Tab[32];
#define NMP_T_EXP2F sExp2fTab
#define NMP_T_LOGF sLogfTab
#define NMP_T_POWLOG2 sPowfLog2Tab
__device__ __forceinline__ void libm_stage_tables() {
  const int t = threadIdx.y * blockDim.x + threadIdx.x;
  if (t < 32) {
    sExp2fTab[t] = kExp2fTab[t];
    sLogfTab[t] = kLogfTab[t];
    sPowfLog2Tab[t] = kPowfLog2Tab[t];
  }
  __syncthreads();
}
#else
#define NMP_T_EXP2F kExp2fTab
#define NMP_T_LOGF kLogfTab
#define NMP_T_POWLOG2 kPowfLog2Tab
__host__ __device__ __forceinline__ void libm_stage_tables() {}
#endif

NMP_LIBM_DEV double mad(double a, double b, double c) { return __builtin_fma(a, b, c); }

NMP_LIBM_DEV uint32_t asuint(float f) { uint32_t u; memcpy(&u, &f, 4); return u; }
NMP_LIBM_DEV float asfloat(uint32_t u) { float f; memcpy(&f, &u, 4); return f; }
NMP_LIBM_DEV uint64_t asuint64(double f) { uint64_t u; memcpy(&u, &f, 8); return u; }
NMP_LIBM_DEV double asdouble(uint64_t u) { double f; memcpy(&f, &u, 8); return f; }
NMP_LIBM_DEV uint64_t exp2_tab_scale_(uint64_t tab, uint64_t k) {
#if defined(__HIP_DEVICE_COMPILE__)
  if (!__builtin_constant_p(k)) {
    typedef uint32_t u32x2 __attribute__((ext_vector_type(2)));
    u32x2 w = __builtin_bit_cast(u32x2, tab);
    w.y += (uint32_t)k << (52 - 5 - 32);
    return __builtin_bit_cast(uint64_t, w);
  }
#endif
  return tab + (k << (52 - 5));
}

NMP_LIBM_DEV bool expf_is_special_(float x) { return !(__builtin_fabsf(x) <= 88.0f); }
NMP_LIBM_DEV float expf_special_(float x, float res) {
  res = (x > 0x1.62e42ep6f) ? asfloat(0x7f800000u) : res;
  res = (x < -0x1.9fe368p6f) ? 0.0f : res;
  res = (x != x) ? x + x : res;
  return res;
}
NMP_LIBM_FN float expf_(float x) {
  const double xd = (double)x;
  double z = kExpfInvLn2Scaled * xd;
  double kd = z + kExp2fShift;
  const uint64_t ki = asuint64(kd);
  kd -= kExp2fShift;
  const double r = mad(kExpfInvLn2Scaled, xd, -kd);
  const uint64_t t = exp2_tab_scale_(NMP_T_EXP2F[ki % 32], ki);
  const double s = asdouble(t);
  z = mad(kExp2fPolyScaled[0], r, kExp2fPolyScaled[1]);
  const double r2 = r * r;
  double y = mad(kExp2fPolyScaled[2], r, 1.0);
  y = mad(z, r2, y);
  y = y * s;
  float res = (float)y;
  if (__builtin_expect(expf_is_special_(x), 0)) res = expf_special_(x, res);
  return res;
}

NMP_LIBM_DEV float expf_k_(float x) {
  const double xd = (double)x;
  double z = kExpfInvLn2Scaled * xd;
  double kd = z + kExp2fShift;
  const uint64_t ki = asuint64(kd);
  kd -= kExp2fShift;
  const double r = mad(kExpfInvLn2Scaled, xd, -kd);
  const uint64_t t = exp2_tab_scale_(kExp2fTab[ki % 32], ki);
  const double s = asdouble(t);
  z = mad(kExp2fPolyScaled[0], r, kExp2fPolyScaled[1]);
  const double r2 = r * r;
  double y = mad(kExp2fPolyScaled[2], r, 1.0);
  y = mad(z, r2, y);
  y = y * s;
  float res = (float)y;
  res = (x > 0x1.62e42ep6f) ? asfloat(0x7f800000u) : res;
  res = (x < -0x1.9fe368p6f) ? 0.0f : res;
  res = (x != x) ? x + x : res;
  return res;
}

NMP_LIBM_DEV bool logf_is_special_(uint32_t ix) { return ix - 0x00800000u >= 0x7f800000u - 0x00800000u; }
NMP_LIBM_DEV uint32_t logf_normalise_(float x, uint32_t ix) {
  return (ix - 1u < 0x007fffffu) ? asuint(x * 0x1p23f) - (23u << 23) : ix;
}
NMP_LIBM_DEV float logf_fix_special_(uint32_t ix0, float x, float res) {
  res = (ix0 == 0x7f800000u) ? x : res;
  res = ((ix0 & 0x80000000u) || ix0 * 2 > 0xff000000u) ? asfloat(0x7fc00000u) : res;
  res = (ix0 * 2 == 0) ? -asfloat(0x7f800000u) : res;
  return res;
}
NMP_LIBM_FN float logf_(float x) {
  const uint32_t ix0 = asuint(x);
  uint32_t ix = ix0;
  if (__builtin_expect(logf_is_special_(ix0), 0)) ix = logf_normalise_(x, ix0);
  const uint32_t tmp = ix - 0x3f330000u;
  const int i = (tmp >> (23 - 4)) % 16;
  const int k = (int32_t)tmp >> 23;
  const uint32_t iz = ix - (tmp & 0xff800000u);
  const double invc = NMP_T_LOGF[2 * i], logc = NMP_T_LOGF[2 * i + 1];
  const double z = (double)asfloat(iz);
  const double r = mad(z, invc, -1.0);
  const double y0 = mad((double)k, kLogfLn2, logc);
  const double r2 = r * r;
  double y = mad(kLogfPoly[1], r, kLogfPoly[2]);
  y = mad(kLogfPoly[0], r2, y);
  y = mad(y, r2, y0 + r);
  float res = (float)y;
  if (__builtin_expect(logf_is_special_(ix0), 0)) res = logf_fix_special_(ix0, x, res);
  return res;
}

#if defined(__HIP_DEVICE_COMPILE__)
#define NMP_LIBM_PIN() __builtin_amdgcn_sched_barrier(0)
#else
#define NMP_LIBM_PIN() ((void)0)
#endif
template <int N>
NMP_LIBM_DEV void logfN_(const float* x, float* out) {
  uint32_t ix0[N], ixn[N], iz[N]; int k[N]; double invc[N], logc[N];
  bool special = false;
#pragma unroll
  for (int n = 0; n < N; n++) {
    ix0[n] = asuint(x[n]);
    ixn[n] = ix0[n];
    special = special || logf_is_special_(ix0[n]);
  }
  if (__builtin_expect(special, 0)) {
#pragma unroll
    for (int n = 0; n < N; n++) ixn[n] = logf_normalise_(x[n], ix0[n]);
  }
#pragma unroll
  for (int n = 0; n < N; n++) {
    const uint32_t ix = ixn[n];
    const uint32_t tmp = ix - 0x3f330000u;
    const int i = (tmp >> (23 - 4)) % 16;
    k[n] = (int32_t)tmp >> 23;
    iz[n] = ix - (tmp & 0xff800000u);
    invc[n] = NMP_T_LOGF[2 * i]; logc[n] = NMP_T_LOGF[2 * i + 1];
  }
  NMP_LIBM_PIN();
#pragma unroll
  for (int n = 0; n < N; n++) {
    const double z = (double)asfloat(iz[n]);
    const double r = mad(z, invc[n], -1.0);
    const double y0 = mad((double)k[n], kLogfLn2, logc[n]);
    const double r2 = r * r;
    double y = mad(kLogfPoly[1], r, kLogfPoly[2]);
    y = mad(kLogfPoly[0], r2, y);
    y = mad(y, r2, y0 + r);
    out[n] = (float)y;
  }
  if (__builtin_expect(special, 0)) {
#pragma unroll
    for (int n = 0; n < N; n++) out[n] = logf_fix_special_(ix0[n], x[n], out[n]);
  }
}
template <int N>
NMP_LIBM_DEV void expfN_(const float* x, float* out) {
  double r[N]; uint64_t t[N];
#pragma unroll
  for (int n = 0; n < N; n++) {
    const double xd = (double)x[n];
    const double z = kExpfInvLn2Scaled * xd;
    double kd = z + kExp2fShift;
    const uint64_t ki = asuint64(kd);
    kd -= kExp2fShift;
    r[n] = mad(kExpfInvLn2Scaled, xd, -kd);
    t[n] = exp2_tab_scale_(NMP_T_EXP2F[ki % 32], ki);
  }
  NMP_LIBM_PIN();
  bool special = false;
#pragma unroll
  for (int n = 0; n < N; n++) {
    const double s = asdouble(t[n]);
    const double z = mad(kExp2fPolyScaled[0], r[n], kExp2fPolyScaled[1]);
    const double r2 = r[n] * r[n];
    double y = mad(kExp2fPolyScaled[2], r[n], 1.0);
    y = mad(z, r2, y);
    y = y * s;
    out[n] = (float)y;
    special = special || expf_is_special_(x[n]);
  }
  if (__builtin_expect(special, 0)) {
#pragma unroll
    for (int n = 0; n < N; n++) out[n] = expf_special_(x[n], out[n]);
  }
}

NMP_LIBM_DEV double powf_log2_inline(uint32_t ix) {
  const uint32_t tmp = ix - 0x3f330000u;
  const int i = (tmp >> (23 - 4)) % 16;
  const uint32_t top = tmp & 0xff800000u;
  const uint32_t iz = ix - top;
  const int k = (int32_t)top >> 23;
  const double invc = NMP_T_POWLOG2[2 * i], logc = NMP_T_POWLOG2[2 * i + 1];
  const double z = (double)asfloat(iz);
  const double r = mad(z, invc, -1.0);
  const double y0 = logc + (double)k;
  const double r2 = r * r;
  double y = mad(kPowfLog2Poly[0], r, kPowfLog2Poly[1]);
  const double p = mad(kPowfLog2Poly[2], r, kPowfLog2Poly[3]);
  const double r4 = r2 * r2;
  double q = mad(kPowfLog2Poly[4], r, y0);
  q = mad(p, r2, q);
  y = mad(y, r4, q);
  return y;
}

NMP_LIBM_DEV double powf_exp2_inline(double xd, uint32_t sign_bias) {
  double kd = xd + kExp2fShiftScaled;
  const uint64_t ki = asuint64(kd);
  kd -= kExp2fShiftScaled;
  const double r = xd - kd;
  const uint64_t t = exp2_tab_scale_(NMP_T_EXP2F[ki % 32], ki + sign_bias);
  const double s = asdouble(t);
  const double z = mad(kExp2fPoly[0], r, kExp2fPoly[1]);
  const double r2 = r * r;
  double y = mad(kExp2fPoly[2], r, 1.0);
  y = mad(z, r2, y);
  y = y * s;
  return y;
}

NMP_LIBM_DEV int powf_checkint(uint32_t iy) {
  const int e = iy >> 23 & 0xff;
  if (e < 0x7f) return 0;
  if (e > 0x7f + 23) return 2;
  if (iy & ((1u << (0x7f + 23 - e)) - 1)) return 0;
  if (iy & (1u << (0x7f + 23 - e))) return 1;
  return 2;
}
NMP_LIBM_DEV bool powf_zeroinfnan(uint32_t ix) { return 2 * ix - 1 >= 2u * 0x7f800000u - 1; }

NMP_LIBM_DEV bool powf_range_special_(double ylogx) { return !(__builtin_fabs(ylogx) < 126.0); }
NMP_LIBM_DEV bool powf_x_special_(uint32_t ix) { return ix - 0x00800000u >= 0x7f800000u - 0x00800000u; }
NMP_LIBM_DEV bool powf_is_special_(uint32_t ix, uint32_t iy) { return powf_x_special_(ix) || powf_zeroinfnan(iy); }
NMP_LIBM_DEV uint32_t powf_pre_special_(float x, uint32_t ix0) {
  uint32_t ix = ix0 & 0x7fffffffu;
  if (ix < 0x00800000u) ix = (asuint(x * 0x1p23f) & 0x7fffffffu) - (23u << 23);
  return ix;
}
NMP_LIBM_DEV float powf_post_special_(float x, float y, double ylogx, float res) {
  const uint32_t ix = asuint(x), iy = asuint(y);
  if (powf_zeroinfnan(iy)) {
    if (2 * iy == 0) return (2 * (ix ^ 0x00400000u) > 2u * 0x7fc00000u) ? x + y : 1.0f;
    if (ix == 0x3f800000u) return (2 * (iy ^ 0x00400000u) > 2u * 0x7fc00000u) ? x + y : 1.0f;
    if (2 * ix > 2u * 0x7f800000u || 2 * iy > 2u * 0x7f800000u) return x + y;
    if (2 * ix == 2 * 0x3f800000u) return 1.0f;
    if ((2 * ix < 2 * 0x3f800000u) == !(iy & 0x80000000u)) return 0.0f;
    return y * y;
  }
  if (powf_zeroinfnan(ix)) {
    float x2 = x * x;
    if ((ix & 0x80000000u) && powf_checkint(iy) == 1) x2 = -x2;
    return (iy & 0x80000000u) ? (1.0f / x2) : x2;
  }
  bool neg = false;
  if (ix & 0x80000000u) {
    const int yint = powf_checkint(iy);
    if (yint == 0) return asfloat(0x7fc00000u);
    neg = yint == 1;
  }
  res = (ylogx > 0x1.fffffffd1d571p+6) ? asfloat(0x7f800000u) : res;
  res = (ylogx <= -150.0) ? 0.0f : res;
  return neg ? -res : res;
}

NMP_LIBM_FN_POW float powf_(float x, float y) {
  const uint32_t ix0 = asuint(x), iy = asuint(y);
  const bool special = powf_is_special_(ix0, iy);
  uint32_t ix = ix0;
  if (__builtin_expect(special, 0)) ix = powf_pre_special_(x, ix0);
  const double logx = powf_log2_inline(ix);
  const double ylogx = (double)y * logx;
  float res = (float)powf_exp2_inline(ylogx, 0);
  if (__builtin_expect(special || powf_range_special_(ylogx), 0)) res = powf_post_special_(x, y, ylogx, res);
  return res;
}

template <int N>
NMP_LIBM_DEV void powfN_(const float* x, const float* y, float* out) {
  uint32_t ix[N]; double invc[N], logc[N];
  bool special = false;
#pragma unroll
  for (int n = 0; n < N; n++) {
    ix[n] = asuint(x[n]);
    special = special || powf_is_special_(ix[n], asuint(y[n]));
  }
  if (__builtin_expect(special, 0)) {
#pragma unroll
    for (int n = 0; n < N; n++) if (powf_x_special_(ix[n])) ix[n] = powf_pre_special_(x[n], ix[n]);
  }
#pragma unroll
  for (int n = 0; n < N; n++) {
    const int i = ((ix[n] - 0x3f330000u) >> (23 - 4)) % 16;
    invc[n] = NMP_T_POWLOG2[2 * i]; logc[n] = NMP_T_POWLOG2[2 * i + 1];
  }
  NMP_LIBM_PIN();
  double ylogx[N], r[N]; uint64_t t[N];
#pragma unroll
  for (int n = 0; n < N; n++) {
    const uint32_t tmp = ix[n] - 0x3f330000u;
    const uint32_t top = tmp & 0xff800000u;
    const int k = (int32_t)top >> 23;
    const double z = (double)asfloat(ix[n] - top);
    const double rr = mad(z, invc[n], -1.0);
    const double y0 = logc[n] + (double)k;
    const double r2 = rr * rr;
    double yy = mad(kPowfLog2Poly[0], rr, kPowfLog2Poly[1]);
    const double p = mad(kPowfLog2Poly[2], rr, kPowfLog2Poly[3]);
    const double r4 = r2 * r2;
    double q = mad(kPowfLog2Poly[4], rr, y0);
    q = mad(p, r2, q);
    yy = mad(yy, r4, q);
    ylogx[n] = (double)y[n] * yy;
    double kd = ylogx[n] + kExp2fShiftScaled;
    const uint64_t ki = asuint64(kd);
    kd -= kExp2fShiftScaled;
    r[n] = ylogx[n] - kd;
    t[n] = exp2_tab_scale_(NMP_T_EXP2F[ki % 32], ki);
  }
  NMP_LIBM_PIN();
#pragma unroll
  for (int n = 0; n < N; n++) {
    const double s = asdouble(t[n]);
    const double z = mad(kExp2fPoly[0], r[n], kExp2fPoly[1]);
    const double r2 = r[n] * r[n];
    double yy = mad(kExp2fPoly[2], r[n], 1.0);
    yy = mad(z, r2, yy);
    yy = yy * s;
    out[n] = (float)yy;
    special = special || powf_range_special_(ylogx[n]);
  }
  if (__builtin_expect(special, 0)) {
#pragma unroll
    for (int n = 0; n < N; n++)
      if (powf_is_special_(asuint(x[n]), asuint(y[n])) || powf_range_special_(ylogx[n])) out[n] = powf_post_special_(x[n], y[n], ylogx[n], out[n]);
  }
}

template <int N>
NMP_LIBM_DEV void powf_exp2N_(const double* ylogx, float* out) {
  double r[N]; uint64_t t[N];
#pragma unroll
  for (int n = 0; n < N; n++) {
    double kd = ylogx[n] + kExp2fShiftScaled;
    const uint64_t ki = asuint64(kd);
    kd -= kExp2fShiftScaled;
    r[n] = ylogx[n] - kd;
    t[n] = exp2_tab_scale_(NMP_T_EXP2F[ki % 32], ki);
  }
  NMP_LIBM_PIN();
#pragma unroll
  for (int n = 0; n < N; n++) {
    const double s = asdouble(t[n]);
    const double z = mad(kExp2fPoly[0], r[n], kExp2fPoly[1]);
    const double r2 = r[n] * r[n];
    double yy = mad(kExp2fPoly[2], r[n], 1.0);
    yy = mad(z, r2, yy);
    yy = yy * s;
    out[n] = (float)yy;
  }
}
NMP_LIBM_DEV double powf_log2_k(uint32_t ix) {
  const uint32_t tmp = ix - 0x3f330000u;
  const int i = (tmp >> (23 - 4)) % 16;
  const uint32_t top = tmp & 0xff800000u;
  const int k = (int32_t)top >> 23;
  const double invc = kPowfLog2Tab[2 * i], logc = kPowfLog2Tab[2 * i + 1];
  const double z = (double)asfloat(ix - top);
  const double r = mad(z, invc, -1.0);
  const double y0 = logc + (double)k;
  const double r2 = r * r;
  double y = mad(kPowfLog2Poly[0], r, kPowfLog2Poly[1]);
  const double p = mad(kPowfLog2Poly[2], r, kPowfLog2Poly[3]);
  const double r4 = r2 * r2;
  double q = mad(kPowfLog2Poly[4], r, y0);
  q = mad(p, r2, q);
  y = mad(y, r4, q);
  return y;
}
template <int N>
NMP_LIBM_DEV void powf_constbaseN_(const float* base, const double* log2base, const float* y, float* out) {
  double ylogx[N];
  bool special = false;
#pragma unroll
  for (int n = 0; n < N; n++) {
    ylogx[n] = (double)y[n] * log2base[n];
    special = special || powf_zeroinfnan(asuint(y[n])) || powf_range_special_(ylogx[n]);
  }
  powf_exp2N_<N>(ylogx, out);
  if (__builtin_expect(special, 0)) {
#pragma unroll
    for (int n = 0; n < N; n++)
      if (powf_zeroinfnan(asuint(y[n])) || powf_range_special_(ylogx[n])) out[n] = powf_post_special_(base[n], y[n], ylogx[n], out[n]);
  }
}
template <int N>
NMP_LIBM_DEV void powf_pairN_(const float* x, float y1, float y2, float* out1, float* out2) {
  uint32_t ix[N]; double invc[N], logc[N];
  bool special = powf_zeroinfnan(asuint(y1)) || powf_zeroinfnan(asuint(y2));
#pragma unroll
  for (int n = 0; n < N; n++) {
    ix[n] = asuint(x[n]);
    special = special || powf_x_special_(ix[n]);
  }
  if (__builtin_expect(special, 0)) {
#pragma unroll
    for (int n = 0; n < N; n++) if (powf_x_special_(ix[n])) ix[n] = powf_pre_special_(x[n], ix[n]);
  }
#pragma unroll
  for (int n = 0; n < N; n++) {
    const int i = ((ix[n] - 0x3f330000u) >> (23 - 4)) % 16;
    invc[n] = NMP_T_POWLOG2[2 * i]; logc[n] = NMP_T_POWLOG2[2 * i + 1];
  }
  NMP_LIBM_PIN();
  double ylogx[2 * N];
#pragma unroll
  for (int n = 0; n < N; n++) {
    const uint32_t tmp = ix[n] - 0x3f330000u;
    const uint32_t top = tmp & 0xff800000u;
    const int k = (int32_t)top >> 23;
    const double z = (double)asfloat(ix[n] - top);
    const double rr = mad(z, invc[n], -1.0);
    const double y0 = logc[n] + (double)k;
    const double r2 = rr * rr;
    double yy = mad(kPowfLog2Poly[0], rr, kPowfLog2Poly[1]);
    const double p = mad(kPowfLog2Poly[2], rr, kPowfLog2Poly[3]);
    const double r4 = r2 * r2;
    double q = mad(kPowfLog2Poly[4], rr, y0);
    q = mad(p, r2, q);
    yy = mad(yy, r4, q);
    ylogx[2 * n] = (double)y1 * yy;
    ylogx[2 * n + 1] = (double)y2 * yy;
    special = special || powf_range_special_(ylogx[2 * n]) || powf_range_special_(ylogx[2 * n + 1]);
  }
  float o[2 * N];
  powf_exp2N_<2 * N>(ylogx, o);
#pragma unroll
  for (int n = 0; n < N; n++) { out1[n] = o[2 * n]; out2[n] = o[2 * n + 1]; }
  if (__builtin_expect(special, 0)) {
#pragma unroll
    for (int n = 0; n < N; n++) {
      const uint32_t ixn = asuint(x[n]);
      if (powf_is_special_(ixn, asuint(y1)) || powf_range_special_(ylogx[2 * n])) out1[n] = powf_post_special_(x[n], y1, ylogx[2 * n], out1[n]);
      if (powf_is_special_(ixn, asuint(y2)) || powf_range_special_(ylogx[2 * n + 1])) out2[n] = powf_post_special_(x[n], y2, ylogx[2 * n + 1], out2[n]);
    }
  }
}

NMP_LIBM_FN float log10f_(float x) {
  const float two25 = 3.3554432000e+07f, ivln10 = 4.3429449201e-01f, log10_2hi = 3.0102920532e-01f,
              log10_2lo = 7.9034151668e-07f;
  int32_t hx = (int32_t)asuint(x);
  int32_t k = 0;
  if (hx < 0x00800000) {
    if ((hx & 0x7fffffff) == 0) return -asfloat(0x7f800000u);
    if (hx < 0) return asfloat(0x7fc00000u);
    k -= 25;
    x *= two25;
    hx = (int32_t)asuint(x);
  }
  if (hx >= 0x7f800000) return x + x;
  k += (hx >> 23) - 127;
  const int32_t i = (int32_t)(((uint32_t)k & 0x80000000u) >> 31);
  hx = (hx & 0x007fffff) | ((0x7f - i) << 23);
  const float y = (float)(k + i);
  x = asfloat((uint32_t)hx);
  const float z = y * log10_2lo + ivln10 * logf_(x);
  return z + y * log10_2hi;
}

NMP_LIBM_FN float atanf_(float x) {
  const float aT[11] = {3.3333334327e-01f, -2.0000000298e-01f, 1.4285714924e-01f, -1.1111110449e-01f,
                        9.0908870101e-02f, -7.6918758452e-02f, 6.6610731184e-02f, -5.8335702866e-02f,
                        4.9768779427e-02f, -3.6531571299e-02f, 1.6285819933e-02f};
  const int32_t hx = (int32_t)asuint(x);
  const int32_t ix = hx & 0x7fffffff;
  const float ax = fabsf(x);
  const bool small = ix < 0x3ee00000;
  const bool r0 = ix < 0x3f300000, r1 = ix < 0x3f980000, r2 = ix < 0x401c0000;
  const float num = small ? x : (r0 ? 2.0f * ax - 1.0f : (r1 ? ax - 1.0f : (r2 ? ax - 1.5f : -1.0f)));
  const float den = small ? 1.0f : (r0 ? 2.0f + ax : (r1 ? ax + 1.0f : (r2 ? 1.0f + 1.5f * ax : ax)));
  const float hi = r0 ? 4.6364760399e-01f : (r1 ? 7.8539812565e-01f : (r2 ? 9.8279368877e-01f : 1.5707962513e+00f));
  const float lo = r0 ? 5.0121582440e-09f : (r1 ? 3.7748947079e-08f : (r2 ? 3.4473217170e-08f : 7.5497894159e-08f));
  const float xr = num / den;
  float z = xr * xr;
  const float w = z * z;
  const float s1 = z * (aT[0] + w * (aT[2] + w * (aT[4] + w * (aT[6] + w * (aT[8] + w * aT[10])))));
  const float s2 = w * (aT[1] + w * (aT[3] + w * (aT[5] + w * (aT[7] + w * aT[9]))));
  const float red = hi - ((xr * (s1 + s2) - lo) - xr);
  float res = small ? xr - xr * (s1 + s2) : ((hx < 0) ? -red : red);
  res = (ix < 0x31000000) ? x : res;
  const float big = (hx > 0) ? 1.5707962513e+00f + 7.5497894159e-08f : -1.5707962513e+00f - 7.5497894159e-08f;
  res = (ix >= 0x4c000000) ? big : res;
  res = (ix > 0x7f800000) ? x + x : res;
  return res;
}

NMP_LIBM_FN float atanf_ge1_(float x) {
  if (__builtin_expect(!(x >= 1.0f), 0)) return atanf_(x);
  const float aT[11] = {3.3333334327e-01f, -2.0000000298e-01f, 1.4285714924e-01f, -1.1111110449e-01f,
                        9.0908870101e-02f, -7.6918758452e-02f, 6.6610731184e-02f, -5.8335702866e-02f,
                        4.9768779427e-02f, -3.6531571299e-02f, 1.6285819933e-02f};
  const int32_t ix = (int32_t)asuint(x);
  const bool r1 = ix < 0x3f980000, r2 = ix < 0x401c0000;
  const float num = r1 ? x - 1.0f : (r2 ? x - 1.5f : -1.0f);
  const float den = r1 ? x + 1.0f : (r2 ? 1.0f + 1.5f * x : x);
  const float hi = r1 ? 7.8539812565e-01f : (r2 ? 9.8279368877e-01f : 1.5707962513e+00f);
  const float lo = r1 ? 3.7748947079e-08f : (r2 ? 3.4473217170e-08f : 7.5497894159e-08f);
  const float xr = num / den;
  const float z = xr * xr;
  const float w = z * z;
  const float s1 = z * (aT[0] + w * (aT[2] + w * (aT[4] + w * (aT[6] + w * (aT[8] + w * aT[10])))));
  const float s2 = w * (aT[1] + w * (aT[3] + w * (aT[5] + w * (aT[7] + w * aT[9]))));
  const float red = hi - ((xr * (s1 + s2) - lo) - xr);
  return (ix >= 0x4c000000) ? 1.5707962513e+00f + 7.5497894159e-08f : red;
}

NMP_LIBM_FN float expm1f_(float x) {
  const float one = 1.0f, huge = 1.0e+30f, tiny = 1.0e-30f, o_threshold = 8.8721679688e+01f,
              ln2_hi = 6.9313812256e-01f, ln2_lo = 9.0580006145e-06f, invln2 = 1.4426950216e+00f,
              Q1 = -3.3333335072e-02f, Q2 = 1.5873016091e-03f, Q3 = -7.9365076090e-05f,
              Q4 = 4.0082177293e-06f, Q5 = -2.0109921195e-07f;
  float y, hi, lo, c = 0.f, t, e, hxs, hfx, r1;
  int32_t k;
  uint32_t hx = asuint(x);
  const uint32_t xsb = hx & 0x80000000u;
  hx &= 0x7fffffffu;
  if (hx >= 0x4195b844u) {
    if (hx >= 0x42b17218u) {
// ... 227 lines not shown
```

### noahmp_amd/csrc/noahmp_engine.hip

```cpp
#include <hip/hip_runtime.h>
#include <stdio.h>
#include <stdlib.h>
#include <string.h>
#include <string>
#include <vector>
#include "noahmp_hip.h"
#define NMP_WIDE_INDEX 1
#include "nmp_kernel.hpp"
#include "nmp_stage.hpp"

using namespace nmp;

namespace {

struct FieldDesc { const char* name; size_t off; int kind; int lev; int io; };
#define FD(n, kind, lev, io) {#n, offsetof(noahmp_step_args, n), kind, lev, io}
const FieldDesc kFields[] = {
#include "nmp_fields.inc"
};
constexpr int kNumFields = sizeof(kFields) / sizeof(kFields[0]);

}

namespace nmp_host {
// ... 80 lines not shown
int noahmp_hip_device_count(void) {
  int n = 0;
  if (hipGetDeviceCount(&n) != hipSuccess) return 0;
  return n;
}

int noahmp_hip_set_device(int device) {
  HIPCHK(hipSetDevice(device));
  g.device = device;
  return 0;
}

void* noahmp_hip_malloc(size_t bytes) {
  if (ensure_init()) return nullptr;
  void* p = nullptr;
  if (hipMalloc(&p, bytes ? bytes : 1) != hipSuccess) { g.last_error = "noahmp_hip_malloc: hipMalloc failed"; return nullptr; }
  return p;
}
int noahmp_hip_memcpy(void* dst, const void* src, size_t bytes, int kind) {
  int rc = ensure_init();
  if (rc) return rc;
  if (!bytes) return 0;
  if (kind == 2) { HIPCHK(hipMemcpy(dst, src, bytes, hipMemcpyDeviceToDevice)); return 0; }
  rc = kind == 0 ? nmp_host::copy_h2d(dst, src, bytes, g.own_stream) : nmp_host::copy_d2h(dst, src, bytes, g.own_stream);
  if (rc) return rc;
  HIPCHK(hipStreamSynchronize(g.own_stream));
  return 0;
}
void noahmp_hip_free(void* p) { if (p) hipFree(p); }

static void drop_host_regs();

int noahmp_hip_debug_live_host_registrations(void) {
  int n = 0;
  for (auto& kv : g.host_regs) n += kv.second.state == 1;
  return n;
}

int noahmp_hip_set_tables(const noahmp_tables* t) {
  int rc = ensure_init();
  if (rc) return rc;
  drop_host_regs();
  g.out_mirror_valid = false;
  static nmp::TablesDev img;
  img.t = *t;
  nmp::derive_tables(img.t, img.d);
  if (!g.d_tables) HIPCHK(hipMalloc((void**)&g.d_tables, sizeof(nmp::TablesDev)));
  HIPCHK(hipMemcpy(g.d_tables, &img, sizeof(nmp::TablesDev), hipMemcpyHostToDevice));
  nmp::tab_scalars_pack(nmp::tab_scalars(img.t), g.ts_i, g.ts_f);
  g.have_tables = true;
  return 0;
}

static void note_fetch(int rc) {
  if (rc > 0) {
    g.deferred_code = rc;
    g.last_error = std::string("a fatal column of the previous (deferred) step is pending: ") + noahmp_hip_error_string(rc);
  }
}

int noahmp_hip_set_option(const char* key, int value) {
  int prev = -1;
  if (!strcmp(key, "block")) { prev = g.block; if (value == 64 || value == 128 || value == 256) g.block = value; }
  else if (!strcmp(key, "lds")) { prev = g.use_lds; g.use_lds = value ? 1 : 0; }
  else if (!strcmp(key, "host_chunks")) {
    prev = g.host_chunks_auto ? -2 : g.host_chunks;
    if (value == -1 || value == -2) g.host_chunks_auto = true;
    else if (value >= 0 && value <= 32) { g.host_chunks = value; g.host_chunks_auto = false; }
  }
  else if (!strcmp(key, "pin_host_arrays")) {
    prev = g.pin_host_arrays;
    if (value == 0 || value == 1) {
      g.pin_host_arrays = value;
      if (!value) drop_host_regs();
    }
  }
  else if (!strcmp(key, "trust_out_mirror")) {
    prev = g.trust_out_mirror;
    if (value == 0 || value == 1) { g.trust_out_mirror = value; g.out_mirror_valid = false; }
  }
  else if (!strcmp(key, "jit_option_kernels")) { prev = g.jit_kernels; if (value == 0 || value == 1) g.jit_kernels = value; }
  else if (!strcmp(key, "jit_compile_only")) { prev = g.jit_compile_only; if (value == 0 || value == 1) g.jit_compile_only = value; }
  else if (!strcmp(key, "fixed_option_kernels")) { prev = g.fixed_kernels; if (value == 0 || value == 1) g.fixed_kernels = value; }
  else if (!strcmp(key, "sorted_land_columns")) { prev = (int)g.sorted_land; g.sorted_land = value; }
  else if (!strcmp(key, "sorted_glacier_columns")) { prev = (int)g.sorted_glacier; g.sorted_glacier = value; }
  else if (!strcmp(key, "resident_state")) {
    prev = g.resident_state;
    if (value == 0 || value == 1) {
      if (!value && (g.resident_dirty || g.deferred_pending)) note_fetch(noahmp_hip_fetch(nullptr));
      g.resident_state = value; g.resident_valid = false;
    }
  }
  else if (!strcmp(key, "resident_sorted")) {
    prev = g.resident_sorted;
    if (value == 0 || value == 1) {
      if (value != g.resident_sorted && (g.resident_dirty || g.deferred_pending)) note_fetch(noahmp_hip_fetch(nullptr));
      if (value != g.resident_sorted) { g.resident_sorted = value; g.sorted_ok = false; g.resident_valid = false; }
    }
  }
  else if (!strcmp(key, "lazy_download")) {
    prev = g.lazy_download;
    if (value == 0 || value == 1) {
      if (!value && (g.resident_dirty || g.deferred_pending)) note_fetch(noahmp_hip_fetch(nullptr));
      g.lazy_download = value;
    }
  }
  else if (!strcmp(key, "overlap_class_kernels")) prev = 1;
  else if (!strcmp(key, "static_inputs")) {
    prev = g.static_inputs;
    if ((value == 0 || value == 1) && value != g.static_inputs) {
      if (g.resident_dirty || g.deferred_pending) note_fetch(noahmp_hip_fetch(nullptr));
      g.static_inputs = value; g.sorted_ok = false; g.sorted_newer = false; g.resident_valid = false;
    }
  }
  else if (!strcmp(key, "deferred_status")) {
    prev = g.deferred_status;
    if (value == 0 || value == 1) {
      if (g.deferred_pending || g.resident_dirty) note_fetch(noahmp_hip_fetch(nullptr));
      g.deferred_status = value; g.resident_valid = false;
    }
  }
  else if (!strcmp(key, "record_cost")) {
#ifdef NMP_COST_RECORD
    prev = g.record_cost;
    if (value == 0 || value == 1) { g.record_cost = value; if (!value) g.cost_fresh = false; }
#endif
  }
  else if (!strcmp(key, "exact_libm")) prev = NMP_EXACT_LIBM;
  return prev;
}

}

static void fill_kargs(KArgs& k, const noahmp_step_args* a) {
  memset(&k, 0, sizeof(k));
  k.a = *a;
  k.ni = a->ime - a->ims + 1;
  k.nka = a->kme - a->kms + 1;
  k.nti = a->ite - a->its + 1;
  k.ntj = a->jte - a->jts + 1;
  k.k1 = 1 - a->kms;
  k.kp_lo = a->kts - a->kms;
  k.kp_hi = a->kts + 1 - a->kms;
  k.yearlen = 365;
  if (a->yr % 4 == 0) { k.yearlen = 366; if (a->yr % 100 == 0) { k.yearlen = 365; if (a->yr % 400 == 0) k.yearlen = 366; } }
  k.c.T = g.d_tables;
  k.c.D = derived_of(g.d_tables);
  k.c.O = Opt{a->idveg, a->iopt_crs, a->iopt_btr, a->iopt_run, a->iopt_sfc, a->iopt_frz, a->iopt_inf,
              a->iopt_rad, a->iopt_alb, a->iopt_snf, a->iopt_tbot, a->iopt_stc};
  k.c.dt = a->dt;
  k.c.isurban = a->isurban;
  k.c.ts = tab_scalars_unpack(g.ts_i, g.ts_f);
  k.c.zsoil[L(1)] = -a->dzs[0];
  for (int l = 2; l <= NOAHMP_NSOIL; l++) k.c.zsoil[L(l)] = -a->dzs[l - 1] + k.c.zsoil[L(l - 1)];
  ctx_fill_uniform(k.c);
  k.err = g.d_err;
  k.counts = g.d_counts;
  k.a.dzs = nullptr;
}

#ifndef NMP_NO_FIXED_KERNELS
struct FixedKernel { int dveg, run; void (*launch)(const nmp_host::LaunchDesc&, int, hipStream_t, hipEvent_t, hipEvent_t); };
static const FixedKernel kFixed[] = {{1, 1, nmp_host::launch_fixed_d1_r1}, {3, 1, nmp_host::launch_fixed_d3_r1},
                                     {3, 5, nmp_host::launch_fixed_d3_r5}, {4, 1, nmp_host::launch_fixed_d4_r1},
                                     {4, 3, nmp_host::launch_fixed_d4_r3}};
#endif
static int fixed_level(const KArgs& k) {
#ifdef NMP_NO_FIXED_KERNELS
  return 0;
#else
  const Opt& o = k.c.O;
  if (!g.fixed_kernels) return 0;
  if (noahmp_hip_index_width(k.ni, k.a.jme - k.a.jms + 1, k.nka) != 32) return 0;
  if (!(o.crs == 1 && o.btr == 1 && o.sfc == 1 && o.frz == 1 && o.inf == 1 && o.rad == 3 && o.alb == 2 &&
        o.snf == 1 && o.tbot == 2 && o.stc == 1)) return g.jit_kernels ? -1 : 0;
  for (int n = 0; n < (int)(sizeof(kFixed) / sizeof(kFixed[0])); n++)
    if (kFixed[n].dveg == o.dveg && kFixed[n].run == o.run) return n + 1;
  return g.jit_kernels ? -1 : 0;
#endif
}

static bool launch_fixed(const KArgs& k, int level, int mode, hipStream_t s, hipEvent_t ev0 = nullptr, hipEvent_t ev1 = nullptr) {
#ifdef NMP_NO_FIXED_KERNELS
  return false;
#else
  nmp_host::LaunchDesc d;
  memset(&d, 0, sizeof(d));
  d.a = k.a; d.tables = k.c.T; d.dt = k.c.dt; d.isurban = k.c.isurban;
  for (int n = 0; n < 6; n++) d.ts_i[n] = g.ts_i[n];
  for (int n = 0; n < 15; n++) d.ts_f[n] = g.ts_f[n];
  for (int l = 0; l < NL; l++) d.zsoil[l] = k.c.zsoil[l];
  d.ni = k.ni; d.nka = k.nka; d.nti = k.nti; d.ntj = k.ntj; d.k1 = k.k1; d.kp_lo = k.kp_lo; d.kp_hi = k.kp_hi; d.yearlen = k.yearlen;
  d.err = k.err; d.counts = k.counts; d.err_base = k.err_base; d.t_offset = k.t_offset; d.t_first = k.t_first; d.t_count = k.t_count;
  d.cost = k.c.cost;
  d.r_land = k.r_land; d.r_ice = k.r_ice; d.r_skip = k.r_skip;
  if (level > 0) { kFixed[level - 1].launch(d, mode, s, ev0, ev1); return true; }
  const Opt& o = k.c.O;
  const int opts[12] = {o.dveg, o.crs, o.btr, o.run, o.sfc, o.frz, o.inf, o.rad, o.alb, o.snf, o.tbot, o.stc};
  return nmp_host::launch_jit(opts, d, mode, s, ev0, ev1);
#endif
}

static void launch_ranges(KArgs k, long n_land, long n_ice, long n_skip, hipStream_t s, hipEvent_t ev0, hipEvent_t ev1) {
  constexpr long B = NMP_FIXED_BLOCK;
  k.r_land = n_land; k.r_ice = n_ice; k.r_skip = n_skip;
  k.t_first = 0; k.t_count = n_land + n_ice + n_skip;
  const long nb_ice = (n_ice + B - 1) / B, nb = nb_ice + (n_land + B - 1) / B + (n_skip + B - 1) / B;
  if (nb <= 0) return;
  if (k.c.cost) k.c.cost -= 2 * nb_ice * B;
  const int fx = fixed_level(k);
  if (fx && launch_fixed(k, fx, 4, s, ev0, ev1)) return;
  hipExtLaunchKernelGGL((noahmp_ranges_kernel<NMP_FIXED_BLOCK>), dim3((unsigned)nb), dim3(NMP_FIXED_BLOCK), 0, s, ev0, ev1, 0, k);
}

static void launch_any(const KArgs& k_in, hipStream_t s, bool class_ranges = false, hipEvent_t* ev = nullptr) {
  KArgs k = k_in;
  const long ncol = (long)k.nti * k.ntj;
  g.last_launch_kind = 0;
  if (ncol <= 0) { g.last_launch_kind = -1; return; }
  k.c.cost = nullptr;
  if (g.record_cost && class_ranges && k.t_offset == 0) {
    if (nmp_host::ensure_bytes((void**)&g.d_cost, &g.d_cost_bytes, (size_t)ncol * 2) == 0) {
      if (g.cost_cols != ncol) (void)hipMemsetAsync(g.d_cost, 0, (size_t)ncol * 2, s);
      k.c.cost = g.d_cost; g.cost_cols = ncol; g.cost_fresh = true;
    }
  }
  if (class_ranges && g.sorted_land >= 0 && g.sorted_glacier >= 0 && g.sorted_land + g.sorted_glacier <= ncol && k.t_offset == 0 &&
      g.block == 256 && g.use_lds) {
    g.last_launch_kind = 1;
    launch_ranges(k, g.sorted_land, g.sorted_glacier, ncol - g.sorted_land - g.sorted_glacier, s, ev ? ev[0] : nullptr, ev ? ev[1] : nullptr);
    return;
  }
  if (ev) hipEventRecord(ev[0], s);
  struct EndEvent { hipEvent_t* e; hipStream_t s; ~EndEvent() { if (e) hipEventRecord(e[1], s); } } at_end{ev, s};
  if (g.block == 256 && g.use_lds) {
    const int fx = fixed_level(k);
    if (fx) { k.t_first = 0; k.t_count = ncol; if (launch_fixed(k, fx, 0, s)) return; }
  }
  if (g.block == 256) launch<256>(k, ncol, g.use_lds, s);
  else if (g.block == 128) launch<128>(k, ncol, g.use_lds, s);
  else launch<64>(k, ncol, g.use_lds, s);
}

static int check_step_args(const noahmp_step_args* a, noahmp_status* st) {
  if (!g.have_tables) { g.last_error = "noahmp_hip_set_tables() has not been called"; return -102; }
  if (a->nsoil != NOAHMP_NSOIL) { if (st) st->code = NOAHMP_ERR_NSOIL_UNSUPPORTED; return NOAHMP_ERR_NSOIL_UNSUPPORTED; }
  if (a->iopt_sfc != 1 && a->iopt_sfc != 2) {
    if (st) st->code = NOAHMP_ERR_OPT_SFC_UNSUPPORTED;
    return NOAHMP_ERR_OPT_SFC_UNSUPPORTED;
  }
  return 0;
}

static void drop_host_regs() {
  bool any = false;
  for (auto& kv : g.host_regs) any = any || kv.second.state == 1;
  if (any) hipDeviceSynchronize();
  for (auto& kv : g.host_regs) if (kv.second.state == 1) hipHostUnregister(const_cast<void*>(kv.first));
  g.host_regs.clear();
  (void)hipGetLastError();
}
static void maybe_pin(const void* host, size_t bytes) {
  if (!g.pin_host_arrays || !host || !bytes) return;
  const char* lo = (const char*)host; const char* hi = lo + bytes;
  for (auto it = g.host_regs.begin(); it != g.host_regs.end();) {
    const char* olo = (const char*)it->first; const char* ohi = olo + it->second.bytes;
    if (it->first != host && olo < hi && lo < ohi) {
      if (it->second.state == 1) { hipDeviceSynchronize(); hipHostUnregister(const_cast<void*>(it->first)); }
      it = g.host_regs.erase(it);
    } else ++it;
  }
  auto it = g.host_regs.find(host);
  if (it == g.host_regs.end()) { g.host_regs[host] = nmp_host::Engine::HostReg{bytes, 1, 0}; (void)hipGetLastError(); return; }
  nmp_host::Engine::HostReg& r = it->second;
  if (r.bytes != bytes) {
    if (r.state == 1) { hipDeviceSynchronize(); hipHostUnregister(const_cast<void*>(host)); }
    r = nmp_host::Engine::HostReg{bytes, 1, 0};
// ... 719 lines not shown
```

### noahmp_amd/csrc/noahmp_jit.hip

```cpp
#include <hip/hip_runtime.h>
#include <hip/hiprtc.h>
#include <dirent.h>
#include <dlfcn.h>
#include <stdio.h>
#include <stdlib.h>
#include <string.h>
#include <sys/stat.h>
#include <unistd.h>
#include <algorithm>
#include <map>
#include <string>
#include <vector>
#include "noahmp_hip.h"
#include "nmp_engine_host.hpp"

namespace nmp_host {

size_t pack_fixed_kargs(const LaunchDesc& d, void* buf, size_t cap);

namespace {

struct JitKernels { hipModule_t mod = nullptr; hipFunction_t fn[3] = {nullptr, nullptr, nullptr}; bool failed = false; };
std::map<std::string, JitKernels> cache;
struct JitStats { int compiled = 0, disk_hits = 0, fallbacks = 0; } stats;

std::string source_dir() {
  Dl_info info;
  if (!dladdr((const void*)&pack_fixed_kargs, &info) || !info.dli_fname) return ".";
  std::string p(info.dli_fname);
  const size_t cut = p.rfind('/');
  return cut == std::string::npos ? "." : p.substr(0, cut);
}

const char* kNames[12] = {"DVEG", "CRS", "BTR", "RUN", "SFC", "FRZ", "INF", "RAD", "ALB", "SNF", "TBOT", "STC"};

#define NMP_STR2(x) #x
#define NMP_STR(x) NMP_STR2(x)
#ifndef NMP_EXACT_LIBM
#define NMP_EXACT_LIBM 1
#endif
#ifndef NMP_WAVES_PER_EU
#define NMP_WAVES_PER_EU 2
#endif
#ifndef NMP_LIBM_LDS
#define NMP_LIBM_LDS 1
#endif
const char* kBuildMacros =
    "#define NMP_EXACT_LIBM " NMP_STR(NMP_EXACT_LIBM) "\n"
    "#define NMP_WAVES_PER_EU " NMP_STR(NMP_WAVES_PER_EU) "\n"
    "#define NMP_LIBM_LDS " NMP_STR(NMP_LIBM_LDS) "\n"
    "#define NMP_FIXED_BLOCK " NMP_STR(NMP_FIXED_BLOCK) "\n"
    "#define NOAHMP_NSOIL " NMP_STR(NOAHMP_NSOIL) "\n"
#ifdef NMP_PHASE_TIMERS
    "#define NMP_PHASE_TIMERS 1\n"
#endif
    ;
const char* kWrapper =
    "#include \"nmp_kernel.hpp\"\n"
    "extern \"C\" __global__ void __launch_bounds__(NMP_FIXED_BLOCK, NMP_WAVES_PER_EU) nmp_jit_m0(const nmp::KArgs k) {\n"
    "  __shared__ float lds[nmp::LAY_SLOTS * NMP_FIXED_BLOCK];\n"
    "  column_kernel_body<NMP_FIXED_BLOCK, true, 0>(k, lds, (long)blockIdx.x, k.t_first, k.t_count); }\n"
    "extern \"C\" __global__ void __launch_bounds__(NMP_FIXED_BLOCK, NMP_WAVES_PER_EU) nmp_jit_m4(const nmp::KArgs k) {\n"
    "  __shared__ float lds[nmp::LAY_SLOTS * NMP_FIXED_BLOCK];\n"
    "  const long nb_ice = (k.r_ice + NMP_FIXED_BLOCK - 1) / NMP_FIXED_BLOCK, nb_land = (k.r_land + NMP_FIXED_BLOCK - 1) / NMP_FIXED_BLOCK;\n"
    "  const long b = (long)blockIdx.x;\n"
    "  if (b < nb_ice) column_kernel_body<NMP_FIXED_BLOCK, true, 2>(k, lds, b, k.r_land, k.r_ice);\n"
    "  else if (b < nb_ice + nb_land) column_kernel_body<NMP_FIXED_BLOCK, true, 1>(k, lds, b - nb_ice, 0L, k.r_land);\n"
    "  else column_kernel_body<NMP_FIXED_BLOCK, true, 3>(k, lds, b - nb_ice - nb_land, k.r_land + k.r_ice, k.r_skip); }\n";
const char* kCompileFlags[] = {"--offload-arch=gfx950", "-O3", "-std=c++17", "-ffp-contract=off", "-fno-slp-vectorize", "-mllvm", "-amdgpu-sched-strategy=max-ilp",
                               "-mllvm", "-instcombine-max-copied-from-constant-users=100000"};
constexpr int kNumCompileFlags = sizeof(kCompileFlags) / sizeof(kCompileFlags[0]);

uint64_t fnv1a(const void* p, size_t n, uint64_t h = 1469598103934665603ull) {
  const unsigned char* c = (const unsigned char*)p;
  for (size_t i = 0; i < n; i++) { h ^= c[i]; h *= 1099511628211ull; }
  return h;
}

bool read_file(const std::string& path, std::vector<char>& out) {
  FILE* f = fopen(path.c_str(), "rb");
  if (!f) return false;
  fseek(f, 0, SEEK_END);
  const long n = ftell(f);
  fseek(f, 0, SEEK_SET);
  out.resize(n > 0 ? n : 0);
  const bool ok = n > 0 && fread(out.data(), 1, n, f) == (size_t)n;
  fclose(f);
  return ok;
}

uint64_t source_hash() {
  static uint64_t h = 0;
  static bool done = false;
  if (done) return h;
  done = true;
  const std::string dir = source_dir();
  std::vector<std::string> files;
  if (DIR* d = opendir(dir.c_str())) {
    while (dirent* e = readdir(d)) {
      const std::string n = e->d_name;
      if ((n.size() > 4 && n.substr(n.size() - 4) == ".hpp") || (n.size() > 4 && n.substr(n.size() - 4) == ".inc")) files.push_back(dir + "/" + n);
    }
    closedir(d);
  }
  std::sort(files.begin(), files.end());
  files.push_back(dir + "/../../include/noahmp_hip.h");
  uint64_t acc = fnv1a(kBuildMacros, strlen(kBuildMacros));
  acc = fnv1a(kWrapper, strlen(kWrapper), acc);
  for (const char* f : kCompileFlags) acc = fnv1a(f, strlen(f), acc);
  int major = 0, minor = 0;
  hiprtcVersion(&major, &minor);
  acc = fnv1a(&major, sizeof major, acc);
  acc = fnv1a(&minor, sizeof minor, acc);
  bool kernel_seen = false;
  std::vector<char> buf;
  for (const std::string& f : files) {
    if (!read_file(f, buf)) { if (f.find("noahmp_hip.h") != std::string::npos) return h = 0; continue; }
    if (f.find("nmp_kernel.hpp") != std::string::npos) kernel_seen = true;
    acc = fnv1a(buf.data(), buf.size(), acc);
  }
  return h = kernel_seen ? (acc ? acc : 1) : 0;
}

bool writable_dir(const std::string& d) {
  mkdir(d.c_str(), 0755);
  return access(d.c_str(), W_OK | X_OK) == 0;
}

std::string cache_dir() {
  static std::string dir;
  static bool done = false;
  if (done) return dir;
  done = true;
  if (const char* e = getenv("NOAHMP_HIP_CACHE_DIR")) { if (*e && writable_dir(e)) return dir = e; }
  const std::string local = source_dir() + "/jit_cache";
  if (writable_dir(local)) return dir = local;
  if (const char* home = getenv("HOME")) {
// ... 150 lines not shown
```

Baseline: 2.142 billion.

## Run iterative flux loops with unchecked libm and redo wave on special inputs

Adds unchecked expf/logf/powf variants that only accumulate a 'suspect' flag instead of branching into special-case handling. The vegetation and bare-ground flux iterations now run first with these fast variants. If any lane in the wave flagged a special input, or a force_checked_regions knob is set, the state is restored and the region is recomputed with the fully checked libm. This removes per-call special-case branches from the hot iterative loops, at the cost of duplicated code, extra register pressure for the saved state, and a full redo when a rare case appears. It is enabled by default only for fixed-dveg kernels built with exact libm.

```diff
diff --git a/__graft_entry__.py b/__graft_entry__.py
--- a/__graft_entry__.py
+++ b/__graft_entry__.py
@@ -24,6 +24,12 @@
     test_libm.build()
     import test_divrc
     test_divrc.build()
+    import test_libm_rare_sites
+    test_libm_rare_sites.build()
+    import test_libm_unchecked
+    test_libm_unchecked.build()
+    import test_optimistic_regions
+    test_optimistic_regions.build()
     from fortran import build_shim
     if build_shim.available():
         build_shim.build()
diff --git a/include/noahmp_hip.h b/include/noahmp_hip.h
--- a/include/noahmp_hip.h
+++ b/include/noahmp_hip.h
@@ -9,6 +9,7 @@
 #endif
 
 #define NOAHMP_HIP_ABI_VERSION 1
+#define NOAHMP_HIP_ABI_MINOR 1
 #define NOAHMP_NSNOW 3
 #ifndef NOAHMP_NSOIL
 #define NOAHMP_NSOIL 4
diff --git a/noahmp_amd/csrc/nmp_dev_common.hpp b/noahmp_amd/csrc/nmp_dev_common.hpp
--- a/noahmp_amd/csrc/nmp_dev_common.hpp
+++ b/noahmp_amd/csrc/nmp_dev_common.hpp
@@ -113,6 +113,68 @@
 NMP_DEV float pow_two(float x) { return x * x; }
 NMP_DEV float pow_neg_quarter(float x) { return 1.0f / sqrtf(sqrtf(x)); }
 #endif
+NMP_DEV float nmp_powf_zero_base(float x, float y) {
+  const bool zero = x == 0.f;
+  const float r = nmp_powf(zero ? 1.f : x, y);
+  return zero ? 0.f : r;
+}
+
+#ifndef NMP_OPTIMISTIC_REGIONS
+#if defined(NMP_FIXED_DVEG) && NMP_EXACT_LIBM
+#define NMP_OPTIMISTIC_REGIONS 1
+#else
+#define NMP_OPTIMISTIC_REGIONS 0
+#endif
+#endif
+template <bool CHK> struct Libm;
+template <> struct Libm<true> {
+  NMP_DEV float expf(float x) { return nmp_expf(x); }
+  NMP_DEV float logf(float x) { return nmp_logf(x); }
+  NMP_DEV float powf(float x, float y) { return nmp_powf(x, y); }
+  template <int N> NMP_DEV void expfN(const float* x, float* out) { nmp_expfN<N>(x, out); }
+  template <int N> NMP_DEV void logfN(const float* x, float* out) { nmp_logfN<N>(x, out); }
+  template <int N> NMP_DEV void powfN(const float* x, const float* y, float* out) { nmp_powfN<N>(x, y, out); }
+  template <int N> NMP_DEV void powf_pairN(const float* x, float y1, float y2, float* o1, float* o2) { nmp_powf_pairN<N>(x, y1, y2, o1, o2); }
+  NMP_DEV void pow_quarter2(float x1, float x2, float& r1, float& r2) { nmp::pow_quarter2(x1, x2, r1, r2); }
+  NMP_DEV float pow_half(float x) { return nmp::pow_half(x); }
+  NMP_DEV float pow_neg_quarter(float x) { return nmp::pow_neg_quarter(x); }
+};
+#if NMP_EXACT_LIBM
+template <> struct Libm<false> {
+  unsigned suspect = 0;
+  NMP_DEV float expf(float x) { NMP_CNT(0); return libm::expf_u_(x, suspect); }
+  NMP_DEV float logf(float x) { NMP_CNT(1); return libm::logf_u_(x, suspect); }
+  NMP_DEV float powf(float x, float y) { NMP_CNT(2); return libm::powf_u_(x, y, suspect); }
+  template <int N> NMP_DEV void expfN(const float* x, float* out) { for (int n = 0; n < N; n++) NMP_CNT(0); libm::expfN_u_<N>(x, out, suspect); }
+  template <int N> NMP_DEV void logfN(const float* x, float* out) { for (int n = 0; n < N; n++) NMP_CNT(1); libm::logfN_u_<N>(x, out, suspect); }
+  template <int N> NMP_DEV void powfN(const float* x, const float* y, float* out) { for (int n = 0; n < N; n++) NMP_CNT(2); libm::powfN_u_<N>(x, y, out, suspect); }
+  template <int N> NMP_DEV void powf_pairN(const float* x, float y1, float y2, float* o1, float* o2) {
+    for (int n = 0; n < 2 * N; n++) NMP_CNT(2);
+    libm::powf_pairN_u_<N>(x, y1, y2, o1, o2, suspect);
+  }
+  NMP_DEV void pow_quarter2(float x1, float x2, float& r1, float& r2) {
+    NMP_CNT(6); NMP_CNT(6);
+    const float x[2] = {x1, x2}, y[2] = {0.25f, 0.25f}; float o[2];
+    libm::powfN_u_<2>(x, y, o, suspect);
+    r1 = o[0]; r2 = o[1];
+  }
+  NMP_DEV float pow_half(float x) { NMP_CNT(6); return libm::powf_u_(x, 0.5f, suspect); }
+  NMP_DEV float pow_neg_quarter(float x) { NMP_CNT(6); return libm::powf_u_(x, -0.25f, suspect); }
+};
+#endif
+#if defined(NMP_REGION_COUNT) && !defined(__HIP_DEVICE_COMPILE__)
+extern "C" { __attribute__((used, visibility("default"))) inline long nmp_region_redos[3] = {0, 0, 0}; }
+#define NMP_REDO(i) (nmp_region_redos[i]++)
+#else
+#define NMP_REDO(i) ((void)0)
+#endif
+NMP_DEV bool wave_any(bool flag) {
+#if defined(__HIP_DEVICE_COMPILE__)
+  return __ballot(flag) != 0;
+#else
+  return flag;
+#endif
+}
 
 #if defined(NMP_PHASE_TIMERS)
 constexpr int NMP_NPHASE = 32;
@@ -242,6 +304,7 @@
   TabScalars ts;
   Urc u;
   unsigned char* cost;
+  int force_checked;
 };
 NMP_DEV void record_cost(const Ctx& c, int which, int n) {
 #if defined(__HIP_DEVICE_COMPILE__) && defined(NMP_COST_RECORD)
diff --git a/noahmp_amd/csrc/nmp_dev_energy.hpp b/noahmp_amd/csrc/nmp_dev_energy.hpp
--- a/noahmp_amd/csrc/nmp_dev_energy.hpp
+++ b/noahmp_amd/csrc/nmp_dev_energy.hpp
@@ -315,7 +315,8 @@
   float tmpcm, tmpcm2;
 };
 
-NMP_DEV void sfcdif1(int& err, int iter, float sfctmp, double r_rhocp, float h, float qair, float zlvl,
+template <class LM>
+NMP_DEV void sfcdif1(LM& lm, int& err, int iter, float sfctmp, double r_rhocp, float h, float qair, float zlvl,
                      float zpd, float z0m, float ur, float mpe, MoState& m, float& cm,
                      float& ch) {
   const float z0h = z0m;
@@ -323,8 +324,8 @@
   float moz2, fmnew, fhnew, fh2new;
   if (zlvl <= zpd) { if (!err) err = NOAHMP_ERR_STABILITY_STOP; }
   if (iter == 1) {
-    m.tmpcm = nmp_logf((zlvl - zpd) / z0m);
-    m.tmpcm2 = nmp_logf((2.0f + z0m) / z0m);
+    m.tmpcm = lm.logf((zlvl - zpd) / z0m);
+    m.tmpcm2 = lm.logf((2.0f + z0m) / z0m);
   }
   const float tmpcm = m.tmpcm, tmpch = m.tmpcm, tmpch2 = m.tmpcm2;
   if (iter == 1) {
@@ -342,10 +343,10 @@
   if (m.mozsgn >= 2) { m.moz = 0.f; m.fm = 0.f; m.fh = 0.f; moz2 = 0.f; m.fh2 = 0.f; }
   if (m.moz < 0.f) {
     float tmp1, tmp12;
-    pow_quarter2(1.f - 16.f * m.moz, 1.f - 16.f * moz2, tmp1, tmp12);
+    lm.pow_quarter2(1.f - 16.f * m.moz, 1.f - 16.f * moz2, tmp1, tmp12);
     const float la[3] = {(1.f + tmp1 * tmp1) / 2.f, (1.f + tmp1) / 2.f, (1.f + tmp12 * tmp12) / 2.f};
     float lg[3];
-    nmp_logfN<3>(la, lg);
+    lm.template logfN<3>(la, lg);
     const float tmp2 = lg[0], tmp3 = lg[1];
     fmnew = 2.f * tmp3 + tmp2 - 2.f * nmp_atanf_ge1(tmp1) + 1.5707963f;
     fhnew = 2 * tmp2;
@@ -371,6 +372,12 @@
   cm = VKC * VKC / (cmfm * cmfm);
   ch = VKC * VKC / (cmfm * chfh);
   m.fv = ur * sqrtf(cm);
+}
+NMP_DEV void sfcdif1(int& err, int iter, float sfctmp, double r_rhocp, float h, float qair, float zlvl,
+                     float zpd, float z0m, float ur, float mpe, MoState& m, float& cm,
+                     float& ch) {
+  Libm<true> lm;
+  sfcdif1(lm, err, iter, sfctmp, r_rhocp, h, qair, zlvl, zpd, z0m, ur, mpe, m, cm, ch);
 }
 
 NMP_DEV float pspmu(float xx) {
@@ -549,13 +556,13 @@
   int bisections;
 };
 
-template <bool FIRST>
-NMP_DEV void vege_iter(const Ctx& c, VegLoop& L, const int iter, VegFirst* f) {
+template <bool FIRST, bool CHK>
+NMP_DEV void vege_iter(Libm<CHK>& lm, const Ctx& c, VegLoop& L, const int iter, VegFirst* f) {
   const float MPE = 1E-6f;
   const float sfctmp = L.sfctmp, rhoair = L.rhoair, ur = L.ur, fveg = L.fveg, tg = L.tg;
   const float z0h = L.z0m, z0hg = L.z0mg, hcan = L.hcan;
   if (c.O.sfc == 1) {
-    sfcdif1(L.err, iter, sfctmp, L.r_rhocp, L.h, L.qair, L.zlvl, L.zpd, L.z0m, ur, MPE, L.mo, L.cm, L.ch);
+    sfcdif1(lm, L.err, iter, sfctmp, L.r_rhocp, L.h, L.qair, L.zlvl, L.zpd, L.z0m, ur, MPE, L.mo, L.cm, L.ch);
   } else {
     sfcdif2(iter, L.z0m, L.tah, L.thair, ur, L.czil, L.zlvl, L.cm, L.ch, L.mo.moz, L.wstar, L.mo.fv, L.rlogu);
     L.ch = div_rc(L.ch, L.r_ur);
@@ -572,14 +579,14 @@
       float molg = -1.f * powi3(L.mo.fv) / tmp1;
       mozg = nmp_min((L.zpd - L.z0mg) / molg, 1.f);
     }
-    if (mozg < 0.f) fhgnew = pow_neg_quarter(1.f - 15.f * mozg);
+    if (mozg < 0.f) fhgnew = lm.pow_neg_quarter(1.f - 15.f * mozg);
     else fhgnew = 1.f + 4.7f * mozg;
     if (FIRST) L.fhg = fhgnew;
     else L.fhg = 0.5f * (L.fhg + fhgnew);
-    float cwpc = pow_half(L.cwp * L.vaie * hcan * L.fhg);
+    float cwpc = lm.pow_half(L.cwp * L.vaie * hcan * L.fhg);
     const float ea[4] = {div_rc(-cwpc * z0hg, L.r_hcan), div_rc(-cwpc * (z0h + L.zpd), L.r_hcan), cwpc, -cwpc / 2.f};
     float ex[4];
-    nmp_expfN<4>(ea, ex);
+    lm.template expfN<4>(ea, ex);
     float tmp1 = ex[0];
     float tmp2 = ex[1];
     float tmprah2 = hcan * ex[2] / cwpc * (tmp1 - tmp2);
@@ -656,61 +663,87 @@
   if (L.iter > 20) L.done = 1;
 }
 
-NMP_DEV void vege_run_until(const Ctx& c, VegLoop& L, int last) {
+template <bool CHK>
+NMP_DEV void vege_run_until(Libm<CHK>& lm, const Ctx& c, VegLoop& L, int last) {
 #pragma unroll 1
-  while (!L.done && L.iter <= last) vege_iter<false>(c, L, L.iter, nullptr);
+  while (!L.done && L.iter <= last) vege_iter<false>(lm, c, L, L.iter, nullptr);
 }
 
 struct SimpleLoop {
-  NMP_DEV void run(const Ctx& c, VegLoop& L, bool active) const {
-    if (active) vege_run_until(c, L, 20);
+  template <bool CHK>
+  NMP_DEV void run(Libm<CHK>& lm, const Ctx& c, VegLoop& L, bool active) const {
+    if (active) vege_run_until(lm, c, L, 20);
   }
 };
+
+NMP_DEV void vege_setup(const Ctx& c, const Parm& P, Col& s, const VegIn& q, float cmv, VegLoop& L, VegFirst& f) {
+  const noahmp_tables* T = c.T;
+  const int v = s.vegtyp - 1;
+  L = VegLoop{};
+  f = VegFirst{};
+  f.P = &P; f.v = v;
+  if (c.O.crs == 1) f.sp = stomata_rows(T, v);
+  const float fveg = s.fveg, ur = q.ur;
+  L.sfctmp = s.sfctmp; L.rhoair = s.rhoair; L.qair = s.qair; L.zlvl = q.zlvl; L.zpd = q.zpd; L.z0m = q.z0m;
+  L.ur = ur; L.z0mg = q.z0mg; L.cwp = q.cwp; L.fveg = fveg; L.rsurf = q.rsurf; L.eair = s.eair;
+  L.gammav = q.gammav; L.canliq = s.canliq; L.canice = s.canice; L.latheav = s.latheav; L.sav = s.sav;
+  L.fwet = s.fwet; L.sfcprs = s.sfcprs; L.thair = s.thair; L.czil = P.czil;
+  L.mo = MoState{0.f, 0.f, 0.f, 0.f, 0.1f, 0, 0.f, 0.f};
+  L.tv = s.tv; L.tg = s.tgv; L.tah = s.tah; L.eah = s.eah; L.ch = s.chv; L.cm = cmv;
+  L.r_rhocp = q.r_rhocp; L.r_gammav = q.r_gammav;
+  if (c.O.sfc != 1) { L.r_ur = rc64(ur); L.rlogu = sfcdif2_rlogu(L.z0m, L.zlvl); }
+  const double r_fveg = rc64(fveg);
+  L.vaie = nmp_min(6.f, div_rc(q.vai, r_fveg));
+  L.laisune = nmp_min(6.f, div_rc(q.laisun, r_fveg));
+  L.laishae = nmp_min(6.f, div_rc(q.laisha, r_fveg));
+  float t = tdc(L.tg), destg_unused;
+  esat_sel(t, L.estg, destg_unused);
+  L.hcan = s.htop;
+  L.r_hcan = rc64(L.hcan);
+  float uc = ur * nmp_logf(L.hcan / q.z0m) / nmp_logf(q.zlvl / q.z0m);
+  if ((L.hcan - q.zpd) <= 0.f) raise(s, NOAHMP_ERR_HCAN_LE_ZPD);
+  L.air = -q.emv * (1.f + (1.f - q.emv) * (1.f - q.emg)) * s.lwdn - q.emv * q.emg * SB * powi4(L.tg);
+  L.cir = (2.f - q.emv * (1.f - q.emg)) * q.emv * SB;
+  L.sqrt_dleaf_uc = sqrtf(P.dleaf / uc);
+  L.irc = s.irc; L.shc = s.shc; L.evc = s.evc; L.tr = s.tr;
+  L.done = 0; L.iter = 1;
+  f.parsun = q.parsun; f.parsha = q.parsha; f.foln = s.foln; f.o2air = s.o2air; f.co2air = s.co2air; f.igs = s.igs; f.btran = s.btran;
+}
+template <bool CHK, class Runner>
+NMP_DEV void vege_loop1(Libm<CHK>& lm, const Ctx& c, const Parm& P, Col& s, const VegIn& q, float cmv, float& psnsun, float& psnsha,
+                        const bool canopy, Runner& runner, VegLoop& L, int& bisections) {
+  L = VegLoop{};
+  L.done = 1;
+  bisections = 0;
+  if (canopy) {
+    VegFirst f;
+    vege_setup(c, P, s, q, cmv, L, f);
+    vege_iter<true>(lm, c, L, 1, &f);
+    psnsun = f.psnsun; psnsha = f.psnsha;
+    bisections = f.bisections;
+  }
+  runner.run(lm, c, L, canopy);
+}
 
 template <class Runner>
 NMP_DEV void vege_flux(const Ctx& c, const Parm& P, Col& s, const VegIn& q, float& cmv, float& psnsun,
                        float& psnsha, const bool canopy, Runner& runner) {
-  const noahmp_tables* T = c.T;
   const float MPE = 1E-6f;
-  VegLoop L = {};
-  L.done = 1;
-  if (canopy) {
-    const int v = s.vegtyp - 1;
-    VegFirst f = {};
-    f.P = &P; f.v = v;
-    if (c.O.crs == 1) f.sp = stomata_rows(T, v);
-    const float fveg = s.fveg, ur = q.ur;
-    L.sfctmp = s.sfctmp; L.rhoair = s.rhoair; L.qair = s.qair; L.zlvl = q.zlvl; L.zpd = q.zpd; L.z0m = q.z0m;
-    L.ur = ur; L.z0mg = q.z0mg; L.cwp = q.cwp; L.fveg = fveg; L.rsurf = q.rsurf; L.eair = s.eair;
-    L.gammav = q.gammav; L.canliq = s.canliq; L.canice = s.canice; L.latheav = s.latheav; L.sav = s.sav;
-    L.fwet = s.fwet; L.sfcprs = s.sfcprs; L.thair = s.thair; L.czil = P.czil;
-    L.mo = MoState{0.f, 0.f, 0.f, 0.f, 0.1f, 0, 0.f, 0.f};
-    L.tv = s.tv; L.tg = s.tgv; L.tah = s.tah; L.eah = s.eah; L.ch = s.chv; L.cm = cmv;
-    L.r_rhocp = q.r_rhocp; L.r_gammav = q.r_gammav;
-    if (c.O.sfc != 1) { L.r_ur = rc64(ur); L.rlogu = sfcdif2_rlogu(L.z0m, L.zlvl); }
-    const double r_fveg = rc64(fveg);
-    L.vaie = nmp_min(6.f, div_rc(q.vai, r_fveg));
-    L.laisune = nmp_min(6.f, div_rc(q.laisun, r_fveg));
-    L.laishae = nmp_min(6.f, div_rc(q.laisha, r_fveg));
-    float t = tdc(L.tg), destg_unused;
-    esat_sel(t, L.estg, destg_unused);
-    L.hcan = s.htop;
-    L.r_hcan = rc64(L.hcan);
-    float uc = ur * nmp_logf(L.hcan / q.z0m) / nmp_logf(q.zlvl / q.z0m);
-    if ((L.hcan - q.zpd) <= 0.f) raise(s, NOAHMP_ERR_HCAN_LE_ZPD);
-    L.air = -q.emv * (1.f + (1.f - q.emv) * (1.f - q.emg)) * s.lwdn - q.emv * q.emg * SB * powi4(L.tg);
-    L.cir = (2.f - q.emv * (1.f - q.emg)) * q.emv * SB;
-    L.sqrt_dleaf_uc = sqrtf(P.dleaf / uc);
-    L.irc = s.irc; L.shc = s.shc; L.evc = s.evc; L.tr = s.tr;
-    L.done = 0; L.iter = 1;
-    f.parsun = q.parsun; f.parsha = q.parsha; f.foln = s.foln; f.o2air = s.o2air; f.co2air = s.co2air; f.igs = s.igs; f.btran = s.btran;
-    vege_iter<true>(c, L, 1, &f);
-    psnsun = f.psnsun; psnsha = f.psnsha;
-    record_cost(c, 1, f.bisections);
-  } else {
-    record_cost(c, 1, 0);
-  }
-  runner.run(c, L, canopy);
+  VegLoop L;
+  int bisections;
+#if NMP_OPTIMISTIC_REGIONS
+  Libm<false> u;
+  vege_loop1(u, c, P, s, q, cmv, psnsun, psnsha, canopy, runner, L, bisections);
+  if (__builtin_expect(wave_any(u.suspect != 0 || c.force_checked != 0), 0)) {
+    NMP_REDO(0);
+    Libm<true> lm;
+    vege_loop1(lm, c, P, s, q, cmv, psnsun, psnsha, canopy, runner, L, bisections);
+  }
+#else
+  Libm<true> lm;
+  vege_loop1(lm, c, P, s, q, cmv, psnsun, psnsha, canopy, runner, L, bisections);
+#endif
+  record_cost(c, 1, canopy ? bisections : 0);
   record_cost(c, 0, canopy ? L.iter - 1 : 0);
   NMP_TIC(21);
   if (!canopy) return;
@@ -776,25 +809,26 @@
   s.chuc = 1.f / rahg;
 }
 
-NMP_DEV void bare_flux(const Ctx& c, const Parm& P, Col& s, const VegIn& q, float zpdg, float& cmb) {
+struct BareLoop {
+  double r_ur; float rlogu2;
+  MoState mo; float h, wstar, estg, destg, csh, cev, ehb;
+};
+template <bool CHK>
+NMP_DEV void bare_loop3(Libm<CHK>& lm, const Ctx& c, const Parm& P, Col& s, const VegIn& q, float zpdg, float& cmb, BareLoop& B) {
   const float MPE = 1E-6f;
   const float rhoair = s.rhoair, sfctmp = s.sfctmp, ur = q.ur, z0m = q.z0mg;
-  MoState mo = {0.f, 0.f, 0.f, 0.f, 0.1f, 0, 0.f, 0.f};
-  float h = 0.f, wstar = 0.f;
-  float t, estg = 0.f, destg, csh = 0.f, cev = 0.f, ehb = 0.f;
-  float& tgb = s.tgb; float& ch = s.chb; float& cm = cmb;
-  const float z0h = z0m;
   const float cir = q.emg * SB;
   const float cgh = 2.f * q.df_top / q.dz_top;
-  const float gamma = q.gammag, lathea = s.latheag;
-  t = tdc(tgb);
-  esat_sel(t, estg, destg);
-  const double r_ur = (c.O.sfc != 1) ? rc64(ur) : 0.0;
-  const float rlogu2 = (c.O.sfc != 1) ? sfcdif2_rlogu(z0m, q.zlvl) : 0.f;
+  MoState& mo = B.mo;
+  float& h = B.h; float& wstar = B.wstar; float& estg = B.estg; float& destg = B.destg; float& csh = B.csh; float& cev = B.cev; float& ehb = B.ehb;
+  float& tgb = s.tgb; float& ch = s.chb; float& cm = cmb;
+  const double r_ur = B.r_ur;
+  const float rlogu2 = B.rlogu2;
+  float t;
 #pragma unroll 1
   for (int iter = 1; iter <= 5; iter++) {
     if (c.O.sfc == 1) {
-      sfcdif1(s.err, iter, sfctmp, q.r_rhocp, h, s.qair, q.zlvl, zpdg, z0m, ur, MPE, mo, cm, ch);
+      sfcdif1(lm, s.err, iter, sfctmp, q.r_rhocp, h, s.qair, q.zlvl, zpdg, z0m, ur, MPE, mo, cm, ch);
     } else {
       sfcdif2(iter, z0m, tgb, s.thair, ur, P.czil, q.zlvl, cm, ch, mo.moz, wstar, mo.fv, rlogu2);
       ch = div_rc(ch, r_ur);
@@ -826,6 +860,37 @@
     esat_sel(t, estg, destg);
     if (iter == 5) s.qsfc = 0.622f * (estg * q.rhsur) / (s.psfc - 0.378f * (estg * q.rhsur));
   }
+}
+
+NMP_DEV void bare_flux(const Ctx& c, const Parm& P, Col& s, const VegIn& q, float zpdg, float& cmb) {
+  const float rhoair = s.rhoair, sfctmp = s.sfctmp, ur = q.ur, z0m = q.z0mg;
+  float& tgb = s.tgb; float& ch = s.chb;
+  const float z0h = z0m;
+  const float cir = q.emg * SB;
+  const float lathea = s.latheag;
+  BareLoop B = {};
+  B.mo = MoState{0.f, 0.f, 0.f, 0.f, 0.1f, 0, 0.f, 0.f};
+  esat_sel(tdc(tgb), B.estg, B.destg);
+  B.r_ur = (c.O.sfc != 1) ? rc64(ur) : 0.0;
+  B.rlogu2 = (c.O.sfc != 1) ? sfcdif2_rlogu(z0m, q.zlvl) : 0.f;
+#if NMP_OPTIMISTIC_REGIONS
+  const BareLoop B0 = B;
+  const float tgb0 = s.tgb, chb0 = s.chb, cmb0 = cmb;
+  const int err0 = s.err;
+  Libm<false> u;
+  bare_loop3(u, c, P, s, q, zpdg, cmb, B);
+  if (__builtin_expect(wave_any(u.suspect != 0 || c.force_checked != 0), 0)) {
+    NMP_REDO(1);
+    B = B0; s.tgb = tgb0; s.chb = chb0; cmb = cmb0; s.err = err0;
+    Libm<true> lm;
+    bare_loop3(lm, c, P, s, q, zpdg, cmb, B);
+  }
+#else
+  Libm<true> lm;
+  bare_loop3(lm, c, P, s, q, zpdg, cmb, B);
+#endif
+  const MoState& mo = B.mo;
+  const float estg = B.estg, csh = B.csh, cev = B.cev, ehb = B.ehb;
   if (c.O.stc == 1) {
     if (s.snowh > 0.05f && tgb > TFRZ) {
       tgb = TFRZ;
diff --git a/noahmp_amd/csrc/nmp_dev_water.hpp b/noahmp_amd/csrc/nmp_dev_water.hpp
--- a/noahmp_amd/csrc/nmp_dev_water.hpp
+++ b/noahmp_amd/csrc/nmp_dev_water.hpp
@@ -67,7 +67,7 @@
   if (s.canice <= 1.E-6f) s.canice = 0.f;
   if (s.canice > 0.f) s.fwet = nmp_max(0.f, s.canice) / nmp_max(maxsno, 1.E-06f);
   else s.fwet = nmp_max(0.f, s.canliq) / nmp_max(maxliq, 1.E-06f);
-  s.fwet = nmp_powf(nmp_min(s.fwet, 1.f), 0.667f);
+  s.fwet = nmp_powf_zero_base(nmp_min(s.fwet, 1.f), 0.667f);
   if (s.canice > 1.E-6f && s.tv > TFRZ) {
     float qmeltc = nmp_min(div_rc(s.canice, rdt), div_rc(div_rc((s.tv - TFRZ) * CICE * s.canice, NMP_RCC(DENICE)), c.u.dt_hfus));
     s.canice = nmp_max(0.f, s.canice - qmeltc * dt);
@@ -440,24 +440,25 @@
   wcnd = P.dksat * nmp_powf(factr, 2.0f * P.bexp + 3.0f);
   wcnd = wcnd * (1.0f - fcr);
 }
-NMP_DEV void wdfcnd2(const Parm& P, double r_smcmax, float& wdf, float& wcnd, float smc, float sice) {
+template <class M>
+NMP_DEV void wdfcnd2(M& m, const Parm& P, double r_smcmax, float& wdf, float& wcnd, float smc, float sice) {
   float factr = nmp_max(0.01f, div_rc(smc, r_smcmax));
   float expon = P.bexp + 2.0f;
-  wdf = P.dwsat * nmp_powf(factr, expon);
+  wdf = P.dwsat * m.powf(factr, expon);
   if (sice > 0.0f) {
     float x = 500.f * sice;
-    float vkwgt = 1.f / (1.f + nmp_powf(x, 3.f));
-    wdf = vkwgt * wdf + (1.f - vkwgt) * P.dwsat * nmp_powf(div_rc(0.2f, r_smcmax), expon);
-  }
-  wcnd = P.dksat * nmp_powf(factr, 2.0f * P.bexp + 3.0f);
-}
-
-template <class A>
-NMP_DEV void soilwater(const Ctx& c, const Parm& P, Col& s, const Lay<A>& y, float qinsur, float qseva,
-                       const float* etrani, float& qdrain, float* wcnd, float& fcrmax) {
+    float vkwgt = 1.f / (1.f + m.powf(x, 3.f));
+    wdf = vkwgt * wdf + (1.f - vkwgt) * P.dwsat * m.powf(div_rc(0.2f, r_smcmax), expon);
+  }
+  wcnd = P.dksat * m.powf(factr, 2.0f * P.bexp + 3.0f);
+}
+
+template <bool CHK, class A>
+NMP_DEV void soilwater_impl(Libm<CHK>& m, const Ctx& c, const Parm& P, Col& s, const Lay<A>& y, float qinsur, float qseva,
+                            const float* etrani, float& qdrain, float* wcnd, float& fcrmax, float* sh2o, float* smc) {
   const float dt = c.dt;
   const double r_smcmax = rc64(P.smcmax);
-  float sh2o[NL], smc[NL], sice[NL], dz[NL], fcr[NL];
+  float sice[NL], dz[NL], fcr[NL];
   float pddum = 0.0f, rsat = 0.0f, sicemax = 0.0f;
   s.runsrf = 0.0f;
   fcrmax = 0.0f;
@@ -476,7 +477,7 @@
   float fcr_arg[NSOIL], fcr_exp[NSOIL];
 #pragma unroll
   for (int k = 1; k <= NSOIL; k++) fcr_arg[k - 1] = -4.0f * (1.f - nmp_min(1.0f, div_rc(sice[L(k)], r_smcmax)));
-  nmp_expfN<NSOIL>(fcr_arg, fcr_exp);
+  m.template expfN<NSOIL>(fcr_arg, fcr_exp);
 #pragma unroll
   for (int k = 1; k <= NSOIL; k++) {
     fcr[L(k)] = div_rc(nmp_max(0.0f, fcr_exp[k - 1] - ea4), c.u.one_m_ea4);
@@ -494,17 +495,17 @@
     for (int k = 1; k <= 100; k++) {
       float zfine = (float)k * dzfine;
       float temp = 1.f + (zwt0 - zfine) / P.psisat;
-      wd2 = wd2 + P.smcmax * (1.f - nmp_powf(temp, -1.f / P.bexp)) * dzfine;
+      wd2 = wd2 + P.smcmax * (1.f - m.powf(temp, -1.f / P.bexp)) * dzfine;
       if (fabsf(wd2 - wd1) <= 0.01f) { s.zwt = zfine; break; }
     }
-    s.runsub = (1.0f - fcrmax) * 4.0f * nmp_expf_const(-TIMEAN) * nmp_expf(-2.0f * s.zwt);
+    s.runsub = (1.0f - fcrmax) * 4.0f * nmp_expf_const(-TIMEAN) * m.expf(-2.0f * s.zwt);
   }
   if (s.vegtyp == c.isurban) fcr[L(1)] = 0.95f;
   if (c.O.run == 1 || c.O.run == 2 || c.O.run == 4 || c.O.run == 5) {
     float fsat;
-    if (c.O.run == 1) fsat = FSATMX * nmp_expf(-0.5f * 6.0f * (s.zwt - 2.0f));
-    else if (c.O.run == 5) fsat = FSATMX * nmp_expf(-0.5f * 6.0f * nmp_max(-2.0f - s.zwt, 0.f));
-    else if (c.O.run == 2) fsat = FSATMX * nmp_expf(-0.5f * 2.0f * s.zwt);
+    if (c.O.run == 1) fsat = FSATMX * m.expf(-0.5f * 6.0f * (s.zwt - 2.0f));
+    else if (c.O.run == 5) fsat = FSATMX * m.expf(-0.5f * 6.0f * nmp_max(-2.0f - s.zwt, 0.f));
+    else if (c.O.run == 2) fsat = FSATMX * m.expf(-0.5f * 2.0f * s.zwt);
     else {
       float smctot = 0.f, dztot = 0.f;
       bool done = false;
@@ -517,7 +518,7 @@
         }
       }
       smctot = smctot / dztot;
-      fsat = nmp_powf(nmp_max(0.01f, smctot / P.smcmax), 4.f);
+      fsat = m.powf(nmp_max(0.01f, smctot / P.smcmax), 4.f);
     }
     if (qinsur > 0.f) {
       s.runsrf = qinsur * ((1.0f - fcr[L(1)]) * fsat + fcr[L(1)]);
@@ -540,7 +541,7 @@
         dmax = dmax * (1.0f - (sh2o[L(k)] + sice[L(k)] - P.smcwlt) / smcav);
         dd = dd + dmax;
       }
-      float val = (1.f - nmp_expf(-P.kdt * dt1));
+      float val = (1.f - m.expf(-P.kdt * dt1));
       float ddt = dd * val;
       float px = nmp_max(0.f, qinsur * dt);
       float infmax = (px * (ddt / (px + ddt))) / dt;
@@ -550,11 +551,11 @@
         float sum = 1.f;
         sum = sum + (acrt * acrt) / 2.f;
         sum = sum + acrt / 1.f;
-        fcr_ = 1.f - nmp_expf(-acrt) * sum;
+        fcr_ = 1.f - m.expf(-acrt) * sum;
       }
       infmax = infmax * fcr_;
       float wdf_, wcnd_;
-      wdfcnd2(P, r_smcmax, wdf_, wcnd_, sh2o[L(1)], sicemax);
+      wdfcnd2(m, P, r_smcmax, wdf_, wcnd_, sh2o[L(1)], sicemax);
       infmax = nmp_max(infmax, wcnd_);
       infmax = nmp_min(infmax, px);
       s.runsrf = nmp_max(0.f, qinsur - infmax);
@@ -577,7 +578,7 @@
       float factr[NSOIL], pw1[NSOIL], pw2[NSOIL];
 #pragma unroll
       for (int k = 1; k <= NSOIL; k++) factr[k - 1] = nmp_max(0.01f, div_rc(smc[L(k)], r_smcmax));
-      nmp_powf_pairN<NSOIL>(factr, P.bexp + 2.0f, 2.0f * P.bexp + 3.0f, pw1, pw2);
+      m.template powf_pairN<NSOIL>(factr, P.bexp + 2.0f, 2.0f * P.bexp + 3.0f, pw1, pw2);
 #pragma unroll
       for (int k = 1; k <= NSOIL; k++) {
         wdf[L(k)] = P.dwsat * pw1[k - 1];
@@ -588,7 +589,7 @@
       }
     } else {
 #pragma unroll
-      for (int k = 1; k <= NSOIL; k++) { wdfcnd2(P, r_smcmax, wdf[L(k)], wcnd[L(k)], sh2o[L(k)], sicemax); smx[L(k)] = sh2o[L(k)]; }
+      for (int k = 1; k <= NSOIL; k++) { wdfcnd2(m, P, r_smcmax, wdf[L(k)], wcnd[L(k)], sh2o[L(k)], sicemax); smx[L(k)] = sh2o[L(k)]; }
     }
     if (c.O.run == 5) smxwtd = (c.O.inf == 1) ? s.smcwtd : s.smcwtd * sh2o[L(NSOIL)] / smc[L(NSOIL)];
 #pragma unroll
@@ -722,6 +723,27 @@
 #pragma unroll
     for (int iz = 1; iz <= NSOIL; iz++) sh2o[L(iz)] = div_rc(mliq[L(iz)], c.u.dzmm[L(iz)]);
   }
+}
+
+template <class A>
+NMP_DEV void soilwater(const Ctx& c, const Parm& P, Col& s, const Lay<A>& y, float qinsur, float qseva,
+                       const float* etrani, float& qdrain, float* wcnd, float& fcrmax) {
+  float sh2o[NL], smc[NL];
+#if NMP_OPTIMISTIC_REGIONS
+  const float runsub0 = s.runsub, zwt0 = s.zwt, smcwtd0 = s.smcwtd, deeprech0 = s.deeprech;
+  Libm<false> u;
+  soilwater_impl(u, c, P, s, y, qinsur, qseva, etrani, qdrain, wcnd, fcrmax, sh2o, smc);
+  if (__builtin_expect(wave_any(u.suspect != 0 || c.force_checked != 0), 0)) {
+    NMP_REDO(2);
+    if (c.O.run != 1) s.runsub = runsub0;
+    if (c.O.run == 2 || c.O.run == 5) { s.zwt = zwt0; s.smcwtd = smcwtd0; s.deeprech = deeprech0; }
+    Libm<true> m;
+    soilwater_impl(m, c, P, s, y, qinsur, qseva, etrani, qdrain, wcnd, fcrmax, sh2o, smc);
+  }
+#else
+  Libm<true> m;
+  soilwater_impl(m, c, P, s, y, qinsur, qseva, etrani, qdrain, wcnd, fcrmax, sh2o, smc);
+#endif
 #pragma unroll
   for (int k = 1; k <= NSOIL; k++) { y.sh2o[L(k)] = sh2o[L(k)]; y.smc[L(k)] = smc[L(k)]; }
 }
diff --git a/noahmp_amd/csrc/nmp_engine_fixed.inc b/noahmp_amd/csrc/nmp_engine_fixed.inc
--- a/noahmp_amd/csrc/nmp_engine_fixed.inc
+++ b/noahmp_amd/csrc/nmp_engine_fixed.inc
@@ -14,7 +14,7 @@
   for (int l = 0; l < NL; l++) k.c.zsoil[l] = d.zsoil[l];
   ctx_fill_uniform(k.c);
   k.ni = d.ni; k.nka = d.nka; k.nti = d.nti; k.ntj = d.ntj; k.k1 = d.k1; k.kp_lo = d.kp_lo; k.kp_hi = d.kp_hi; k.yearlen = d.yearlen;
-  k.c.cost = d.cost;
+  k.c.cost = d.cost; k.c.force_checked = d.force_checked;
   k.r_land = d.r_land; k.r_ice = d.r_ice; k.r_skip = d.r_skip;
   k.err = d.err; k.counts = d.counts; k.err_base = d.err_base; k.t_offset = d.t_offset; k.t_first = d.t_first; k.t_count = d.t_count;
 }
diff --git a/noahmp_amd/csrc/nmp_engine_host.hpp b/noahmp_amd/csrc/nmp_engine_host.hpp
--- a/noahmp_amd/csrc/nmp_engine_host.hpp
+++ b/noahmp_amd/csrc/nmp_engine_host.hpp
@@ -84,6 +84,7 @@
   noahmp_step_args resident_args;
   int jit_kernels = 1;
   int jit_compile_only = 0;
+  int force_checked_regions = 0;
   int fixed_kernels = 1;
   long sorted_land = -1, sorted_glacier = -1;
   int block = 256;
@@ -104,6 +105,7 @@
   long t_offset, t_first, t_count;
   unsigned char* cost;
   long r_land, r_ice, r_skip;
+  int force_checked;
 };
 void launch_fixed_d1_r1(const LaunchDesc& d, int mode, hipStream_t s, hipEvent_t ev0, hipEvent_t ev1);
 #ifdef NMP_PHASE_TIMERS
diff --git a/noahmp_amd/csrc/nmp_libm.hpp b/noahmp_amd/csrc/nmp_libm.hpp
--- a/noahmp_amd/csrc/nmp_libm.hpp
+++ b/noahmp_amd/csrc/nmp_libm.hpp
@@ -16,6 +16,13 @@
 #endif
 #ifndef NMP_LIBM_FN_POW
 #define NMP_LIBM_FN_POW NMP_LIBM_FN
+#endif
+#ifdef NMP_LIBM_NO_SPECIAL
+#define NMP_LIBM_RARE(c) (0)
+#define NMP_LIBM_RARE_EXP(c) (1)
+#else
+#define NMP_LIBM_RARE(c) __builtin_expect((c), 0)
+#define NMP_LIBM_RARE_EXP(c) NMP_LIBM_RARE(c)
 #endif
 
 #if defined(__HIP_DEVICE_COMPILE__)
@@ -90,7 +97,7 @@
   y = mad(z, r2, y);
   y = y * s;
   float res = (float)y;
-  if (__builtin_expect(expf_is_special_(x), 0)) res = expf_special_(x, res);
+  if (NMP_LIBM_RARE_EXP(expf_is_special_(x))) res = expf_special_(x, res);
   return res;
 }
 
@@ -128,7 +135,7 @@
 NMP_LIBM_FN float logf_(float x) {
   const uint32_t ix0 = asuint(x);
   uint32_t ix = ix0;
-  if (__builtin_expect(logf_is_special_(ix0), 0)) ix = logf_normalise_(x, ix0);
+  if (NMP_LIBM_RARE(logf_is_special_(ix0))) ix = logf_normalise_(x, ix0);
   const uint32_t tmp = ix - 0x3f330000u;
   const int i = (tmp >> (23 - 4)) % 16;
   const int k = (int32_t)tmp >> 23;
@@ -142,7 +149,7 @@
   y = mad(kLogfPoly[0], r2, y);
   y = mad(y, r2, y0 + r);
   float res = (float)y;
-  if (__builtin_expect(logf_is_special_(ix0), 0)) res = logf_fix_special_(ix0, x, res);
+  if (NMP_LIBM_RARE(logf_is_special_(ix0))) res = logf_fix_special_(ix0, x, res);
   return res;
 }
 
@@ -161,7 +168,7 @@
     ixn[n] = ix0[n];
     special = special || logf_is_special_(ix0[n]);
   }
-  if (__builtin_expect(special, 0)) {
+  if (NMP_LIBM_RARE(special)) {
 #pragma unroll
     for (int n = 0; n < N; n++) ixn[n] = logf_normalise_(x[n], ix0[n]);
   }
@@ -186,7 +193,7 @@
     y = mad(y, r2, y0 + r);
     out[n] = (float)y;
   }
-  if (__builtin_expect(special, 0)) {
+  if (NMP_LIBM_RARE(special)) {
 #pragma unroll
     for (int n = 0; n < N; n++) out[n] = logf_fix_special_(ix0[n], x[n], out[n]);
   }
@@ -217,7 +224,7 @@
     out[n] = (float)y;
     special = special || expf_is_special_(x[n]);
   }
-  if (__builtin_expect(special, 0)) {
+  if (NMP_LIBM_RARE_EXP(special)) {
 #pragma unroll
     for (int n = 0; n < N; n++) out[n] = expf_special_(x[n], out[n]);
   }
@@ -267,6 +274,7 @@
   return 2;
 }
 NMP_LIBM_DEV bool powf_zeroinfnan(uint32_t ix) { return 2 * ix - 1 >= 2u * 0x7f800000u - 1; }
+NMP_LIBM_DEV bool powf_infnan(uint32_t ix) { return 2 * ix >= 2u * 0x7f800000u; }
 
 NMP_LIBM_DEV bool powf_range_special_(double ylogx) { return !(__builtin_fabs(ylogx) < 126.0); }
 NMP_LIBM_DEV bool powf_x_special_(uint32_t ix) { return ix - 0x00800000u >= 0x7f800000u - 0x00800000u; }
@@ -306,11 +314,11 @@
   const uint32_t ix0 = asuint(x), iy = asuint(y);
   const bool special = powf_is_special_(ix0, iy);
   uint32_t ix = ix0;
-  if (__builtin_expect(special, 0)) ix = powf_pre_special_(x, ix0);
+  if (NMP_LIBM_RARE(special)) ix = powf_pre_special_(x, ix0);
   const double logx = powf_log2_inline(ix);
   const double ylogx = (double)y * logx;
   float res = (float)powf_exp2_inline(ylogx, 0);
-  if (__builtin_expect(special || powf_range_special_(ylogx), 0)) res = powf_post_special_(x, y, ylogx, res);
+  if (NMP_LIBM_RARE(special || powf_range_special_(ylogx))) res = powf_post_special_(x, y, ylogx, res);
   return res;
 }
 
@@ -323,7 +331,7 @@
     ix[n] = asuint(x[n]);
     special = special || powf_is_special_(ix[n], asuint(y[n]));
   }
-  if (__builtin_expect(special, 0)) {
+  if (NMP_LIBM_RARE(special)) {
 #pragma unroll
     for (int n = 0; n < N; n++) if (powf_x_special_(ix[n])) ix[n] = powf_pre_special_(x[n], ix[n]);
   }
@@ -368,7 +376,7 @@
     out[n] = (float)yy;
     special = special || powf_range_special_(ylogx[n]);
   }
-  if (__builtin_expect(special, 0)) {
+  if (NMP_LIBM_RARE(special)) {
 #pragma unroll
     for (int n = 0; n < N; n++)
       if (powf_is_special_(asuint(x[n]), asuint(y[n])) || powf_range_special_(ylogx[n])) out[n] = powf_post_special_(x[n], y[n], ylogx[n], out[n]);
@@ -423,10 +431,10 @@
 #pragma unroll
   for (int n = 0; n < N; n++) {
     ylogx[n] = (double)y[n] * log2base[n];
-    special = special || powf_zeroinfnan(asuint(y[n])) || powf_range_special_(ylogx[n]);
+    special = special || powf_infnan(asuint(y[n])) || powf_range_special_(ylogx[n]);
   }
   powf_exp2N_<N>(ylogx, out);
-  if (__builtin_expect(special, 0)) {
+  if (NMP_LIBM_RARE(special)) {
 #pragma unroll
     for (int n = 0; n < N; n++)
       if (powf_zeroinfnan(asuint(y[n])) || powf_range_special_(ylogx[n])) out[n] = powf_post_special_(base[n], y[n], ylogx[n], out[n]);
@@ -441,7 +449,7 @@
     ix[n] = asuint(x[n]);
     special = special || powf_x_special_(ix[n]);
   }
-  if (__builtin_expect(special, 0)) {
+  if (NMP_LIBM_RARE(special)) {
 #pragma unroll
     for (int n = 0; n < N; n++) if (powf_x_special_(ix[n])) ix[n] = powf_pre_special_(x[n], ix[n]);
   }
@@ -475,7 +483,7 @@
   powf_exp2N_<2 * N>(ylogx, o);
 #pragma unroll
   for (int n = 0; n < N; n++) { out1[n] = o[2 * n]; out2[n] = o[2 * n + 1]; }
-  if (__builtin_expect(special, 0)) {
+  if (NMP_LIBM_RARE(special)) {
 #pragma unroll
     for (int n = 0; n < N; n++) {
       const uint32_t ixn = asuint(x[n]);
@@ -483,6 +491,174 @@
       if (powf_is_special_(ixn, asuint(y2)) || powf_range_special_(ylogx[2 * n + 1])) out2[n] = powf_post_special_(x[n], y2, ylogx[2 * n + 1], out2[n]);
     }
   }
+}
+
+NMP_LIBM_DEV float expf_u_(float x, unsigned& suspect) {
+  const double xd = (double)x;
+  double z = kExpfInvLn2Scaled * xd;
+  double kd = z + kExp2fShift;
+  const uint64_t ki = asuint64(kd);
+  kd -= kExp2fShift;
+  const double r = mad(kExpfInvLn2Scaled, xd, -kd);
+  const uint64_t t = exp2_tab_scale_(NMP_T_EXP2F[ki % 32], ki);
+  const double s = asdouble(t);
+  z = mad(kExp2fPolyScaled[0], r, kExp2fPolyScaled[1]);
+  const double r2 = r * r;
+  double y = mad(kExp2fPolyScaled[2], r, 1.0);
+  y = mad(z, r2, y);
+  y = y * s;
+  suspect |= (unsigned)expf_is_special_(x);
+  return (float)y;
+}
+NMP_LIBM_DEV float logf_u_(float x, unsigned& suspect) {
+  const uint32_t ix = asuint(x);
+  const uint32_t tmp = ix - 0x3f330000u;
+  const int i = (tmp >> (23 - 4)) % 16;
+  const int k = (int32_t)tmp >> 23;
+  const uint32_t iz = ix - (tmp & 0xff800000u);
+  const double invc = NMP_T_LOGF[2 * i], logc = NMP_T_LOGF[2 * i + 1];
+  const double z = (double)asfloat(iz);
+  const double r = mad(z, invc, -1.0);
+  const double y0 = mad((double)k, kLogfLn2, logc);
+  const double r2 = r * r;
+  double y = mad(kLogfPoly[1], r, kLogfPoly[2]);
+  y = mad(kLogfPoly[0], r2, y);
+  y = mad(y, r2, y0 + r);
+  suspect |= (unsigned)logf_is_special_(ix);
+  return (float)y;
+}
+template <int N>
+NMP_LIBM_DEV void logfN_u_(const float* x, float* out, unsigned& suspect) {
+  uint32_t iz[N]; int k[N]; double invc[N], logc[N];
+#pragma unroll
+  for (int n = 0; n < N; n++) {
+    const uint32_t ix = asuint(x[n]);
+    suspect |= (unsigned)logf_is_special_(ix);
+    const uint32_t tmp = ix - 0x3f330000u;
+    const int i = (tmp >> (23 - 4)) % 16;
+    k[n] = (int32_t)tmp >> 23;
+    iz[n] = ix - (tmp & 0xff800000u);
+    invc[n] = NMP_T_LOGF[2 * i]; logc[n] = NMP_T_LOGF[2 * i + 1];
+  }
+  NMP_LIBM_PIN();
+#pragma unroll
+  for (int n = 0; n < N; n++) {
+    const double z = (double)asfloat(iz[n]);
+    const double r = mad(z, invc[n], -1.0);
+    const double y0 = mad((double)k[n], kLogfLn2, logc[n]);
+    const double r2 = r * r;
+    double y = mad(kLogfPoly[1], r, kLogfPoly[2]);
+    y = mad(kLogfPoly[0], r2, y);
+    y = mad(y, r2, y0 + r);
+    out[n] = (float)y;
+  }
+}
+template <int N>
+NMP_LIBM_DEV void expfN_u_(const float* x, float* out, unsigned& suspect) {
+  double r[N]; uint64_t t[N];
+#pragma unroll
+  for (int n = 0; n < N; n++) {
+    const double xd = (double)x[n];
+    const double z = kExpfInvLn2Scaled * xd;
+    double kd = z + kExp2fShift;
+    const uint64_t ki = asuint64(kd);
+    kd -= kExp2fShift;
+    r[n] = mad(kExpfInvLn2Scaled, xd, -kd);
+    t[n] = exp2_tab_scale_(NMP_T_EXP2F[ki % 32], ki);
+  }
+  NMP_LIBM_PIN();
+#pragma unroll
+  for (int n = 0; n < N; n++) {
+    const double s = asdouble(t[n]);
+    const double z = mad(kExp2fPolyScaled[0], r[n], kExp2fPolyScaled[1]);
+    const double r2 = r[n] * r[n];
+    double y = mad(kExp2fPolyScaled[2], r[n], 1.0);
+    y = mad(z, r2, y);
+    y = y * s;
+    out[n] = (float)y;
+    suspect |= (unsigned)expf_is_special_(x[n]);
+  }
+}
+NMP_LIBM_DEV float powf_u_(float x, float y, unsigned& suspect) {
+  const uint32_t ix = asuint(x), iy = asuint(y);
+  const double logx = powf_log2_inline(ix);
+  const double ylogx = (double)y * logx;
+  const float res = (float)powf_exp2_inline(ylogx, 0);
+  suspect |= (unsigned)(powf_is_special_(ix, iy) || powf_range_special_(ylogx));
+  return res;
+}
+template <int N>
+NMP_LIBM_DEV void powf_log2N_(const uint32_t* ix, double* log2x) {
+  double invc[N], logc[N];
+#pragma unroll
+  for (int n = 0; n < N; n++) {
+    const int i = ((ix[n] - 0x3f330000u) >> (23 - 4)) % 16;
+    invc[n] = NMP_T_POWLOG2[2 * i]; logc[n] = NMP_T_POWLOG2[2 * i + 1];
+  }
+  NMP_LIBM_PIN();
+#pragma unroll
+  for (int n = 0; n < N; n++) {
+    const uint32_t tmp = ix[n] - 0x3f330000u;
+    const uint32_t top = tmp & 0xff800000u;
+    const int k = (int32_t)top >> 23;
+    const double z = (double)asfloat(ix[n] - top);
+    const double rr = mad(z, invc[n], -1.0);
+    const double y0 = logc[n] + (double)k;
+    const double r2 = rr * rr;
+    double yy = mad(kPowfLog2Poly[0], rr, kPowfLog2Poly[1]);
+    const double p = mad(kPowfLog2Poly[2], rr, kPowfLog2Poly[3]);
+    const double r4 = r2 * r2;
+    double q = mad(kPowfLog2Poly[4], rr, y0);
+    q = mad(p, r2, q);
+    log2x[n] = mad(yy, r4, q);
+  }
+}
+template <int N>
+NMP_LIBM_DEV void powfN_u_(const float* x, const float* y, float* out, unsigned& suspect) {
+  uint32_t ix[N]; double ylogx[N];
+#pragma unroll
+  for (int n = 0; n < N; n++) {
+    ix[n] = asuint(x[n]);
+    suspect |= (unsigned)powf_is_special_(ix[n], asuint(y[n]));
+  }
+  powf_log2N_<N>(ix, ylogx);
+#pragma unroll
+  for (int n = 0; n < N; n++) {
+    ylogx[n] = (double)y[n] * ylogx[n];
+    suspect |= (unsigned)powf_range_special_(ylogx[n]);
+  }
+  powf_exp2N_<N>(ylogx, out);
+}
+template <int N>
+NMP_LIBM_DEV void powf_constbaseN_u_(const double* log2base, const float* y, float* out, unsigned& suspect) {
+  double ylogx[N];
+#pragma unroll
+  for (int n = 0; n < N; n++) {
+    ylogx[n] = (double)y[n] * log2base[n];
+    suspect |= (unsigned)(powf_infnan(asuint(y[n])) || powf_range_special_(ylogx[n]));
+  }
+  powf_exp2N_<N>(ylogx, out);
+}
+template <int N>
+NMP_LIBM_DEV void powf_pairN_u_(const float* x, float y1, float y2, float* out1, float* out2, unsigned& suspect) {
+  uint32_t ix[N]; double log2x[N], ylogx[2 * N];
+  suspect |= (unsigned)(powf_zeroinfnan(asuint(y1)) || powf_zeroinfnan(asuint(y2)));
+#pragma unroll
+  for (int n = 0; n < N; n++) {
+    ix[n] = asuint(x[n]);
+    suspect |= (unsigned)powf_x_special_(ix[n]);
+  }
+  powf_log2N_<N>(ix, log2x);
+#pragma unroll
+  for (int n = 0; n < N; n++) {
+    ylogx[2 * n] = (double)y1 * log2x[n];
+    ylogx[2 * n + 1] = (double)y2 * log2x[n];
+    suspect |= (unsigned)(powf_range_special_(ylogx[2 * n]) || powf_range_special_(ylogx[2 * n + 1]));
+  }
+  float o[2 * N];
+  powf_exp2N_<2 * N>(ylogx, o);
+#pragma unroll
+  for (int n = 0; n < N; n++) { out1[n] = o[2 * n]; out2[n] = o[2 * n + 1]; }
 }
 
 NMP_LIBM_FN float log10f_(float x) {
diff --git a/noahmp_amd/csrc/noahmp_engine.hip b/noahmp_amd/csrc/noahmp_engine.hip
--- a/noahmp_amd/csrc/noahmp_engine.hip
+++ b/noahmp_amd/csrc/noahmp_engine.hip
@@ -186,6 +186,7 @@
   else if (!strcmp(key, "jit_option_kernels")) { prev = g.jit_kernels; if (value == 0 || value == 1) g.jit_kernels = value; }
   else if (!strcmp(key, "jit_compile_only")) { prev = g.jit_compile_only; if (value == 0 || value == 1) g.jit_compile_only = value; }
   else if (!strcmp(key, "fixed_option_kernels")) { prev = g.fixed_kernels; if (value == 0 || value == 1) g.fixed_kernels = value; }
+  else if (!strcmp(key, "force_checked_regions")) { prev = g.force_checked_regions; if (value == 0 || value == 1) g.force_checked_regions = value; }
   else if (!strcmp(key, "sorted_land_columns")) { prev = (int)g.sorted_land; g.sorted_land = value; }
   else if (!strcmp(key, "sorted_glacier_columns")) { prev = (int)g.sorted_glacier; g.sorted_glacier = value; }
   else if (!strcmp(key, "resident_state")) {
@@ -296,7 +297,7 @@
   for (int l = 0; l < NL; l++) d.zsoil[l] = k.c.zsoil[l];
   d.ni = k.ni; d.nka = k.nka; d.nti = k.nti; d.ntj = k.ntj; d.k1 = k.k1; d.kp_lo = k.kp_lo; d.kp_hi = k.kp_hi; d.yearlen = k.yearlen;
   d.err = k.err; d.counts = k.counts; d.err_base = k.err_base; d.t_offset = k.t_offset; d.t_first = k.t_first; d.t_count = k.t_count;
-  d.cost = k.c.cost;
+  d.cost = k.c.cost; d.force_checked = g.force_checked_regions;
   d.r_land = k.r_land; d.r_ice = k.r_ice; d.r_skip = k.r_skip;
   if (level > 0) { kFixed[level - 1].launch(d, mode, s, ev0, ev1); return true; }
   const Opt& o = k.c.O;
diff --git a/noahmp_amd/csrc/noahmp_jit.hip b/noahmp_amd/csrc/noahmp_jit.hip
--- a/noahmp_amd/csrc/noahmp_jit.hip
+++ b/noahmp_amd/csrc/noahmp_jit.hip
@@ -53,6 +53,9 @@
     "#define NOAHMP_NSOIL " NMP_STR(NOAHMP_NSOIL) "\n"
 #ifdef NMP_PHASE_TIMERS
     "#define NMP_PHASE_TIMERS 1\n"
+#endif
+#ifdef NMP_LIBM_NO_SPECIAL
+    "#define NMP_LIBM_NO_SPECIAL 1\n"
 #endif
     ;
 const char* kWrapper =
```

Measured after the change: 2.252 billion (median of 6 runs). +5.1%, better.
